# AILab-CVC/SEED-X

Measured on AMD Instinct MI355X. Metric: end-to-end generations/sec (img-in -> txt + 1024px-img-out), higher is better.
Workload: dtype fp16

## Files before the change

include/seedx_hip.h:

```cpp
#ifndef SEEDX_HIP_H
#define SEEDX_HIP_H
#include <stdint.h>
#ifdef __cplusplus
extern "C" {
#endif

#define SX_OK 0
#define SX_ERR_INVALID 1
#define SX_ERR_HIP 2

#define SX_F16 0
#define SX_BF16 1
#define SX_F32 2
#define SX_BF16X3 3
#define SX_F16X2 4
#define SX_FP8_E4M3 5
#define SX_TILED16 0x100

#define SX_ACT_NONE 0
#define SX_ACT_GELU 1
#define SX_ACT_SILU 2

#define SX_A_LINEAR 0
#define SX_A_CONV3X3 1

const char* sx_last_error(void);
int sx_version(void);

typedef struct sx_gemm_args {
  const void* A;
  const void* W;
  void* C;
  const float* bias;
  const float* bias2d;
  const float* residual;
  int32_t M, N, K;
  int32_t ldc, ldr;
  int32_t n_valid;
  int32_t res_mod;
  int32_t bias2d_rows;
  int32_t dtype;
  int32_t out_dtype;
  int32_t act;
  int32_t glu;
  int32_t a_mode;
  int32_t B, Hin, Win, Cin, Hout, Wout;
  int32_t stride;
  int32_t upsample;
  int32_t ld_bias2d;
  int32_t pad_mode;
  int32_t a_planes;
} sx_gemm_args;
int sx_gemm(const sx_gemm_args* args, void* stream);
int sx_gemm_gn(const sx_gemm_args* args, double* stats, int groups, int rows_per_sample, int* fused_host, void* stream);
typedef struct sx_gemm_ln_args {
  void* x16_out;
  double* row_stats_out;
  const double* row_stats_in;
  const float* colsum;
  int32_t ld_x16;
  int32_t dim;
  float eps;
  int32_t reserved;
} sx_gemm_ln_args;
int sx_gemm_ln(const sx_gemm_args* args, const sx_gemm_ln_args* ln, void* stream);
int sx_gemm_force_tile(int cfg);
int sx_gemm_debug_stamps(void* buf);
int sx_gemm_pick_tile(int M, int N, int K, int glu, int conv);

typedef struct sx_gemv_args {
  const void* x;
  const void* W;
  void* y;
  const float* residual;
  int32_t M, N, K;
  int32_t dtype, out_dtype, act, glu;
  int32_t w_layout;
  int32_t x_layout;
  void* workspace;
  uint64_t workspace_bytes;
  void* x16_out;
  float* row_ssq_out;
  const float* row_ssq_in;
  int32_t ssq_in_parts, ssq_dim;
  float ssq_eps;
  int32_t x_planes;
  int32_t out_planes;
  const float* x16_gamma;
  int32_t w_dtype;
  const float* w_scale;
} sx_gemv_args;
int sx_gemv_ssq_parts(int N, int glu, int w_layout);
int sx_gemv(const sx_gemv_args* args, void* stream);
int sx_gemv_force_valu(int on);
int sx_gemv_tune(int key, int value);

int sx_layernorm(const void* x, int in_dtype, void* y, int out_dtype, const float* gamma, const float* beta,
                 int rows, int cols, float eps, int rms, void* stream);

int sx_softmax_rows(const float* x, int64_t ldx, void* y, int64_t ldy, int rows, int cols, float scale, int out_dtype,
                    void* stream);

int sx_groupnorm(const float* x, void* y, void* raw16, int out_dtype, const float* gamma, const float* beta,
                 double* stats, int B, int HW, int C, int groups, float eps, int silu, void* stream);
int sx_groupnorm2(const float* x, const float* x2, int C1, void* y, void* raw16, int out_dtype, const float* gamma,
                  const float* beta, double* stats, int B, int HW, int C, int groups, float eps, int silu, void* stream);
int sx_norm_tune(int key, int value);
int sx_groupnorm_sp(const float* x, const float* x2, int C1, void* y, void* raw16, int out_dtype, const float* gamma,
                    const float* beta, double* stats, int B, int HW, int hw_total, int C, int groups, float eps, int silu,
                    int phase, void* stream);

typedef struct sx_attn_args {
  const void* Q;
  const void* K;
  const void* V;
  void* O;
  int32_t B, H, Sq, Skv, D, reserved;
  int64_t q_batch_stride, q_row_stride, q_head_stride;
  int64_t k_batch_stride, k_row_stride, k_head_stride;
  int64_t v_batch_stride, v_row_stride, v_head_stride;
  int64_t o_batch_stride, o_row_stride;
  float scale;
  int32_t causal;
  int32_t dtype;
} sx_attn_args;
int sx_attention(const sx_attn_args* args, void* stream);

typedef struct sx_attn_small_args {
  const void* Q;
  const void* K;
  const void* V;
  void* O;
  int32_t B, H, Sq, Skv, D;
  int64_t q_batch_stride, q_row_stride, q_head_stride;
  int64_t k_batch_stride, k_row_stride, k_head_stride;
  int64_t v_batch_stride, v_row_stride, v_head_stride;
  int64_t o_batch_stride, o_row_stride;
  float scale;
  int32_t dtype;
} sx_attn_small_args;
int sx_attention_small(const sx_attn_small_args* args, void* stream);

int sx_attn_decode(const void* q, const void* kcache, const void* vcache, void* out, float* scratch,
                   const int32_t* ctx_len_dev, int H, int D, int Tmax, int nsplit, float scale, int dtype,
                   void* stream);

int sx_rope_kv_append(void* qkv, void* kcache, void* vcache, const float* cos_tab, const float* sin_tab,
                      const int32_t* pos0_dev, int T, int H, int D, int Tmax, int dtype, void* stream);
int sx_embedding(const int32_t* ids, const void* table, float* out, int T, int dim, int dtype, void* stream);
int sx_scatter_rows(const float* src, const int32_t* rows, float* dst, int n, int dim, void* stream);
int sx_greedy_next(float* logits, int vocab, const int32_t* img_ids_dev, int n_img, const int32_t* prev_id_dev,
                   int32_t* next_id_dev, int32_t* out_ids, const int32_t* step_dev, void* stream);

int sx_rope_kv_append_b(void* qkv, void* kcache, void* vcache, const float* cos_tab, const float* sin_tab,
                        const int32_t* pos0_dev, int G, int T, int H, int D, int Tmax, int64_t cache_seq_stride, int dtype,
                        void* stream);
int sx_attn_decode_b(const void* q, const void* kcache, const void* vcache, void* out, float* scratch,
                     const int32_t* ctx_len_dev, int G, int H, int D, int Tmax, int64_t cache_seq_stride, int nsplit,
                     float scale, int dtype, int64_t q_seq_stride, void* stream);
typedef struct sx_attn_decode_args {
  const void* qkv;
  void* kcache;
  void* vcache;
  void* out;
  float* scratch;
  void* counters;
  const float* cos_tab;
  const float* sin_tab;
  const int32_t* pos_dev;
  int32_t G, H, D, Tmax, nsplit, dtype;
  int64_t cache_seq_stride;
  float scale;
  int32_t reserved;
} sx_attn_decode_args;
int sx_attn_decode_fused(const sx_attn_decode_args* args, void* stream);
int sx_greedy_next_b(float* logits, int ld_logits, int vocab, const int32_t* img_ids_dev, int n_img,
                     const int32_t* prev_id_dev, int32_t* next_id_dev, int32_t* out_ids, int ld_out,
                     const int32_t* step_dev, int G, void* stream);
int sx_scatter_rows_step(const float* src, const int32_t* step_dev, float* dst, int G, int dim, int seq_rows, void* stream);
int sx_add_i32_n(int32_t* p, int delta, int n, void* stream);
typedef struct sx_slot_step_args {
  float* logits;
  const int32_t* img_ids_dev;
  int32_t* cur;
  int32_t* live;
  int32_t* n_new;
  const int32_t* max_new;
  const int32_t* force_at;
  int32_t* pos;
  int32_t* ctx;
  int32_t* step;
  int32_t* out_ids;
  int32_t* status;
  int32_t ld_logits, vocab, n_img, ld_out, force_id, eos_id, G, reserved;
} sx_slot_step_args;
int sx_greedy_next_slots(const sx_slot_step_args* args, void* stream);
typedef struct sx_sample_args {
  const int32_t* do_sample;
  const float* temperature;
  const int32_t* top_k;
  const float* top_p;
  const uint32_t* seed;
  const int32_t* token_index;
  int32_t* n_kept;
  float* p_chosen;
} sx_sample_args;
int sx_sample_next_b(float* logits, int ld_logits, int vocab, const int32_t* img_ids_dev, int n_img,
                     const int32_t* prev_id_dev, int32_t* next_id_dev, int32_t* out_ids, int ld_out,
                     const int32_t* step_dev, int G, const sx_sample_args* sample, void* stream);
int sx_sample_next_slots(const sx_slot_step_args* args, const sx_sample_args* sample, void* stream);

int sx_cast(const void* src, int src_dtype, void* dst, int dst_dtype, int64_t n, void* stream);
int sx_split_bf16(const float* x, void* out, int64_t rows, int cols, int role, void* stream);

int sx_split16(const float* x, int64_t ldx, void* out, int rows, int cols, int dtype, void* stream);
int sx_rmsnorm_planes(const float* x, const float* gamma, float* y32, void* out16, int rows, int cols, float eps, int dtype,
                      void* stream);
int sx_rope_kv_append_f32(float* qkv, float* kcache, float* vcache, const float* cos_tab, const float* sin_tab,
                          const int32_t* pos0_dev, int G, int T, int H, int D, int Tmax, int64_t cache_seq_stride,
                          int table_dtype, void* stream);
int sx_rope_kv_append_f32_v16(float* qkv, float* kcache, void* vcache16, const float* cos_tab, const float* sin_tab,
                              const int32_t* pos0_dev, int G, int T, int H, int D, int Tmax, int64_t cache_seq_stride,
                              int table_dtype, void* stream);
int sx_rope_kv_append_f32_q8(float* qkv, void* kcodes, void* vcodes, float* kscale, float* vscale, const float* cos_tab,
                             const float* sin_tab, const int32_t* pos0_dev, int G, int T, int H, int D, int Tmax,
                             int64_t cache_seq_stride, int64_t scale_seq_stride, int table_dtype, int emulate, void* stream);
typedef struct sx_attn_f32_args {
  const float* q;
  const float* kcache;
  const void* vcache;
  void* out;
  const int32_t* pos0_dev;
  int64_t q_row_stride, cache_seq_stride;
  int64_t kv_row_stride;
  int64_t kv_head_stride;
  int32_t G, T, H, D, Tmax, dtype;
  float scale;
  int32_t causal;
  int32_t v16;
  int32_t nsplit;
  float* scratch;
  const float* rope_cos;
  const float* rope_sin;
  const float* k_new;
  const float* v_new;
  int32_t kv_fp8;
  const float* k_scale;
  const float* v_scale;
  int64_t scale_seq_stride;
} sx_attn_f32_args;
int sx_attention_f32(const sx_attn_f32_args* args, void* stream);
int sx_attention_f32_variant(int v);
int sx_copy2d_f32(const float* src, int64_t src_ld, float* dst, int64_t dst_ld, int64_t rows, int cols,
                  void* stream);
int sx_add_f32(const float* a, const float* b, float* y, int64_t n, void* stream);
int sx_patchify(const float* img, void* patches, int B, int S, int P, int Kpad, int dtype, void* stream);
int sx_im2col3x3_small(const float* x, void* out, int B, int H, int W, int Cin, int Kpad, int dtype,
                       void* stream);
int sx_avgpool_tokens(const float* x, float* y, int B, int L, int D, int k, void* stream);
int sx_timestep_embedding(const float* t, const int32_t* idx_dev, void* out, int n, int dim, int dtype, void* stream);
int sx_nchw_to_nhwc(const float* src, float* dst, int ld, int B, int C, int HW, void* stream);
int sx_nhwc_to_nchw(const float* src, int ld, float* dst, int B, int C, int HW, void* stream);
int sx_add_i32(int32_t* p, int delta, void* stream);
int sx_profile_marker(int tag, void* stream);
int sx_silu_cast(const float* x, void* y, int dtype, int64_t n, void* stream);

int sx_cfg_euler_step(const float* eps, float* latents, float* scaled_next, const float* sigmas_dev,
                      const int32_t* step_dev, int nb, int64_t n, int C, int ld_scaled, float gs, float igs, int mode,
                      void* stream);

int sx_resample_u8(const void* src, int Hin, int Win, int C, int64_t src_stride, void* dst, int Hout, int Wout,
                   const int32_t* kk_h, const int32_t* bounds_h, int ksize_h, const int32_t* kk_v,
                   const int32_t* bounds_v, int ksize_v, int y_first, int y_rows, void* tmp, void* stream);
int sx_u8_to_chw_lut(const void* src, int H, int W, int64_t src_stride, int x0, int y0, int Hc, int Wc,
                     const float* lut3x256, float* dst, void* stream);
int sx_chw_to_u8_image(const float* src, int H, int W, void* dst, void* stream);
int sx_marker_mask(const int64_t* ids, int T, int64_t boi, int64_t bop, int64_t eoi, int64_t eop, void* mask,
                   void* stream);
int sx_l2norm_dim1(const float* x, float* y, int B, int T, int D, float eps, void* stream);

int sx_comm_alloc(void** ptr, uint64_t bytes);
int sx_comm_free(void* ptr);
int sx_ipc_export(void* ptr, unsigned char* handle64);
int sx_ipc_open(const unsigned char* handle64, void** ptr);
int sx_ipc_close(void* ptr);
#define SX_ONESHOT_CHUNK 4096
typedef struct sx_oneshot_args {
  void* data;
  void* gather_out;
  const void* stage;
  const void* flags;
  void* epoch;
  void* status;
  int32_t n, cap, rank, world;
  uint32_t max_spin;
  int32_t chunk;
  int32_t mode;
  int32_t reserved;
} sx_oneshot_args;
int sx_allreduce_oneshot(const sx_oneshot_args* args, void* stream);

int sx_halo_pack(const void* x, const void* prev_row, const void* next_row, void* out, int B, int Hl, int W, int C, int left_col,
                 int bottom, void* stream);

#ifdef __cplusplus
}
#endif
#endif
```

seed-x_amd/_lib.py:

```python
import ctypes as C
import os

_HERE = os.path.dirname(os.path.abspath(__file__))
LIB_PATH = os.path.join(_HERE, "lib", "libseedx_hip.so")

SX_F16, SX_BF16, SX_F32 = 0, 1, 2
SX_BF16X3 = 3
SX_F16X2 = 4
SX_FP8_E4M3 = 5
SX_TILED16 = 0x100
SX_ACT_NONE, SX_ACT_GELU, SX_ACT_SILU = 0, 1, 2
SX_A_LINEAR, SX_A_CONV3X3 = 0, 1

c_i32, c_i64, c_f32, c_vp = C.c_int32, C.c_int64, C.c_float, C.c_void_p


class GemmArgs(C.Structure):
    _fields_ = [("A", c_vp), ("W", c_vp), ("C", c_vp), ("bias", c_vp), ("bias2d", c_vp), ("residual", c_vp),
                ("M", c_i32), ("N", c_i32), ("K", c_i32), ("ldc", c_i32), ("ldr", c_i32), ("n_valid", c_i32),
                ("res_mod", c_i32), ("bias2d_rows", c_i32), ("dtype", c_i32), ("out_dtype", c_i32),
                ("act", c_i32), ("glu", c_i32), ("a_mode", c_i32),
                ("B", c_i32), ("Hin", c_i32), ("Win", c_i32), ("Cin", c_i32), ("Hout", c_i32), ("Wout", c_i32),
                ("stride", c_i32), ("upsample", c_i32), ("ld_bias2d", c_i32), ("pad_mode", c_i32), ("a_planes", c_i32)]


class GemmLnArgs(C.Structure):
    _fields_ = [("x16_out", c_vp), ("row_stats_out", c_vp), ("row_stats_in", c_vp), ("colsum", c_vp),
                ("ld_x16", c_i32), ("dim", c_i32), ("eps", c_f32), ("reserved", c_i32)]


class GemvArgs(C.Structure):
    _fields_ = [("x", c_vp), ("W", c_vp), ("y", c_vp), ("residual", c_vp),
                ("M", c_i32), ("N", c_i32), ("K", c_i32),
                ("dtype", c_i32), ("out_dtype", c_i32), ("act", c_i32), ("glu", c_i32),
                ("w_layout", c_i32), ("x_layout", c_i32), ("workspace", c_vp), ("workspace_bytes", C.c_uint64),
                ("x16_out", c_vp), ("row_ssq_out", c_vp), ("row_ssq_in", c_vp), ("ssq_in_parts", c_i32), ("ssq_dim", c_i32),
                ("ssq_eps", c_f32), ("x_planes", c_i32), ("out_planes", c_i32), ("x16_gamma", c_vp),
                ("w_dtype", c_i32), ("w_scale", c_vp)]


class AttnF32Args(C.Structure):
    _fields_ = [("q", c_vp), ("kcache", c_vp), ("vcache", c_vp), ("out", c_vp), ("pos0_dev", c_vp),
                ("q_row_stride", c_i64), ("cache_seq_stride", c_i64), ("kv_row_stride", c_i64), ("kv_head_stride", c_i64),
                ("G", c_i32), ("T", c_i32), ("H", c_i32), ("D", c_i32), ("Tmax", c_i32), ("dtype", c_i32),
                ("scale", c_f32), ("causal", c_i32), ("v16", c_i32), ("nsplit", c_i32), ("scratch", c_vp),
                ("rope_cos", c_vp), ("rope_sin", c_vp), ("k_new", c_vp), ("v_new", c_vp),
                ("kv_fp8", c_i32), ("k_scale", c_vp), ("v_scale", c_vp), ("scale_seq_stride", c_i64)]


class OneshotArgs(C.Structure):
    _fields_ = [("data", c_vp), ("gather_out", c_vp), ("stage", c_vp), ("flags", c_vp), ("epoch", c_vp), ("status", c_vp),
                ("n", c_i32), ("cap", c_i32), ("rank", c_i32), ("world", c_i32), ("max_spin", C.c_uint32), ("chunk", c_i32),
                ("mode", c_i32), ("reserved", c_i32)]


class AttnDecodeArgs(C.Structure):
    _fields_ = [("qkv", c_vp), ("kcache", c_vp), ("vcache", c_vp), ("out", c_vp), ("scratch", c_vp), ("counters", c_vp),
                ("cos_tab", c_vp), ("sin_tab", c_vp), ("pos_dev", c_vp),
                ("G", c_i32), ("H", c_i32), ("D", c_i32), ("Tmax", c_i32), ("nsplit", c_i32), ("dtype", c_i32),
                ("cache_seq_stride", c_i64), ("scale", c_f32), ("reserved", c_i32)]


class SlotStepArgs(C.Structure):
    _fields_ = [("logits", c_vp), ("img_ids_dev", c_vp), ("cur", c_vp), ("live", c_vp), ("n_new", c_vp), ("max_new", c_vp),
                ("force_at", c_vp), ("pos", c_vp), ("ctx", c_vp), ("step", c_vp), ("out_ids", c_vp), ("status", c_vp),
                ("ld_logits", c_i32), ("vocab", c_i32), ("n_img", c_i32), ("ld_out", c_i32), ("force_id", c_i32),
                ("eos_id", c_i32), ("G", c_i32), ("reserved", c_i32)]


class SampleArgs(C.Structure):
    _fields_ = [("do_sample", c_vp), ("temperature", c_vp), ("top_k", c_vp), ("top_p", c_vp), ("seed", c_vp),
                ("token_index", c_vp), ("n_kept", c_vp), ("p_chosen", c_vp)]


class AttnArgs(C.Structure):
    _fields_ = [("Q", c_vp), ("K", c_vp), ("V", c_vp), ("O", c_vp),
                ("B", c_i32), ("H", c_i32), ("Sq", c_i32), ("Skv", c_i32), ("D", c_i32), ("reserved", c_i32),
                ("q_batch_stride", c_i64), ("q_row_stride", c_i64), ("q_head_stride", c_i64),
                ("k_batch_stride", c_i64), ("k_row_stride", c_i64), ("k_head_stride", c_i64),
                ("v_batch_stride", c_i64), ("v_row_stride", c_i64), ("v_head_stride", c_i64),
                ("o_batch_stride", c_i64), ("o_row_stride", c_i64),
                ("scale", c_f32), ("causal", c_i32), ("dtype", c_i32)]


class AttnSmallArgs(C.Structure):
    _fields_ = [("Q", c_vp), ("K", c_vp), ("V", c_vp), ("O", c_vp),
                ("B", c_i32), ("H", c_i32), ("Sq", c_i32), ("Skv", c_i32), ("D", c_i32),
                ("q_batch_stride", c_i64), ("q_row_stride", c_i64), ("q_head_stride", c_i64),
                ("k_batch_stride", c_i64), ("k_row_stride", c_i64), ("k_head_stride", c_i64),
                ("v_batch_stride", c_i64), ("v_row_stride", c_i64), ("v_head_stride", c_i64),
                ("o_batch_stride", c_i64), ("o_row_stride", c_i64),
                ("scale", c_f32), ("dtype", c_i32)]


SIGNATURES = {
    "sx_version": [],
    "sx_gemm": [C.POINTER(GemmArgs), c_vp],
    "sx_gemm_gn": [C.POINTER(GemmArgs), c_vp, c_i32, c_i32, C.POINTER(c_i32), c_vp],
    "sx_gemm_ln": [C.POINTER(GemmArgs), C.POINTER(GemmLnArgs), c_vp],
    "sx_gemm_force_tile": [c_i32],
    "sx_gemm_debug_stamps": [c_vp],
    "sx_gemm_pick_tile": [c_i32, c_i32, c_i32, c_i32, c_i32],
    "sx_gemv": [C.POINTER(GemvArgs), c_vp],
    "sx_gemv_ssq_parts": [c_i32, c_i32, c_i32],
    "sx_gemv_force_valu": [c_i32],
    "sx_layernorm": [c_vp, c_i32, c_vp, c_i32, c_vp, c_vp, c_i32, c_i32, c_f32, c_i32, c_vp],
    "sx_softmax_rows": [c_vp, c_i64, c_vp, c_i64, c_i32, c_i32, c_f32, c_i32, c_vp],
    "sx_groupnorm": [c_vp, c_vp, c_vp, c_i32, c_vp, c_vp, c_vp, c_i32, c_i32, c_i32, c_i32, c_f32, c_i32, c_vp],
    "sx_groupnorm2": [c_vp, c_vp, c_i32, c_vp, c_vp, c_i32, c_vp, c_vp, c_vp, c_i32, c_i32, c_i32, c_i32, c_f32, c_i32, c_vp],
    "sx_groupnorm_sp": [c_vp, c_vp, c_i32, c_vp, c_vp, c_i32, c_vp, c_vp, c_vp, c_i32, c_i32, c_i32, c_i32, c_i32, c_f32, c_i32,
                        c_i32, c_vp],
    "sx_attention": [C.POINTER(AttnArgs), c_vp],
    "sx_norm_tune": [c_i32, c_i32],
    "sx_gemv_tune": [c_i32, c_i32],
    "sx_comm_alloc": [C.POINTER(c_vp), C.c_uint64],
    "sx_comm_free": [c_vp],
    "sx_ipc_export": [c_vp, C.c_char_p],
    "sx_ipc_open": [C.c_char_p, C.POINTER(c_vp)],
    "sx_ipc_close": [c_vp],
    "sx_allreduce_oneshot": [C.POINTER(OneshotArgs), c_vp],
    "sx_halo_pack": [c_vp, c_vp, c_vp, c_vp, c_i32, c_i32, c_i32, c_i32, c_i32, c_i32, c_vp],
    "sx_attention_small": [C.POINTER(AttnSmallArgs), c_vp],
    "sx_attn_decode": [c_vp, c_vp, c_vp, c_vp, c_vp, c_vp, c_i32, c_i32, c_i32, c_i32, c_f32, c_i32, c_vp],
    "sx_rope_kv_append": [c_vp, c_vp, c_vp, c_vp, c_vp, c_vp, c_i32, c_i32, c_i32, c_i32, c_i32, c_vp],
    "sx_rope_kv_append_b": [c_vp, c_vp, c_vp, c_vp, c_vp, c_vp, c_i32, c_i32, c_i32, c_i32, c_i32, c_i64, c_i32, c_vp],
    "sx_attn_decode_fused": [C.POINTER(AttnDecodeArgs), c_vp],
    "sx_attn_decode_b": [c_vp, c_vp, c_vp, c_vp, c_vp, c_vp, c_i32, c_i32, c_i32, c_i32, c_i64, c_i32, c_f32, c_i32, c_i64, c_vp],
    "sx_greedy_next_b": [c_vp, c_i32, c_i32, c_vp, c_i32, c_vp, c_vp, c_vp, c_i32, c_vp, c_i32, c_vp],
    "sx_greedy_next_slots": [C.POINTER(SlotStepArgs), c_vp],
    "sx_sample_next_b": [c_vp, c_i32, c_i32, c_vp, c_i32, c_vp, c_vp, c_vp, c_i32, c_vp, c_i32, C.POINTER(SampleArgs), c_vp],
    "sx_sample_next_slots": [C.POINTER(SlotStepArgs), C.POINTER(SampleArgs), c_vp],
    "sx_scatter_rows_step": [c_vp, c_vp, c_vp, c_i32, c_i32, c_i32, c_vp],
    "sx_add_i32_n": [c_vp, c_i32, c_i32, c_vp],
    "sx_embedding": [c_vp, c_vp, c_vp, c_i32, c_i32, c_i32, c_vp],
    "sx_scatter_rows": [c_vp, c_vp, c_vp, c_i32, c_i32, c_vp],
    "sx_greedy_next": [c_vp, c_i32, c_vp, c_i32, c_vp, c_vp, c_vp, c_vp, c_vp],
    "sx_cast": [c_vp, c_i32, c_vp, c_i32, c_i64, c_vp],
    "sx_split_bf16": [c_vp, c_vp, c_i64, c_i32, c_i32, c_vp],
    "sx_split16": [c_vp, c_i64, c_vp, c_i32, c_i32, c_i32, c_vp],
    "sx_rmsnorm_planes": [c_vp, c_vp, c_vp, c_vp, c_i32, c_i32, c_f32, c_i32, c_vp],
    "sx_rope_kv_append_f32": [c_vp, c_vp, c_vp, c_vp, c_vp, c_vp, c_i32, c_i32, c_i32, c_i32, c_i32, c_i64, c_i32, c_vp],
    "sx_rope_kv_append_f32_v16": [c_vp, c_vp, c_vp, c_vp, c_vp, c_vp, c_i32, c_i32, c_i32, c_i32, c_i32, c_i64, c_i32, c_vp],
    "sx_rope_kv_append_f32_q8": [c_vp, c_vp, c_vp, c_vp, c_vp, c_vp, c_vp, c_vp, c_i32, c_i32, c_i32, c_i32, c_i32, c_i64, c_i64, c_i32,
                                 c_i32, c_vp],
    "sx_attention_f32": [C.POINTER(AttnF32Args), c_vp],
    "sx_attention_f32_variant": [c_i32],
    "sx_copy2d_f32": [c_vp, c_i64, c_vp, c_i64, c_i64, c_i32, c_vp],
    "sx_add_f32": [c_vp, c_vp, c_vp, c_i64, c_vp],
    "sx_patchify": [c_vp, c_vp, c_i32, c_i32, c_i32, c_i32, c_i32, c_vp],
    "sx_im2col3x3_small": [c_vp, c_vp, c_i32, c_i32, c_i32, c_i32, c_i32, c_i32, c_vp],
    "sx_avgpool_tokens": [c_vp, c_vp, c_i32, c_i32, c_i32, c_i32, c_vp],
    "sx_timestep_embedding": [c_vp, c_vp, c_vp, c_i32, c_i32, c_i32, c_vp],
    "sx_nchw_to_nhwc": [c_vp, c_vp, c_i32, c_i32, c_i32, c_i32, c_vp],
    "sx_nhwc_to_nchw": [c_vp, c_i32, c_vp, c_i32, c_i32, c_i32, c_vp],
    "sx_add_i32": [c_vp, c_i32, c_vp],
    "sx_profile_marker": [c_i32, c_vp],
    "sx_silu_cast": [c_vp, c_vp, c_i32, c_i64, c_vp],
    "sx_resample_u8": [c_vp, c_i32, c_i32, c_i32, c_i64, c_vp, c_i32, c_i32, c_vp, c_vp, c_i32, c_vp, c_vp, c_i32, c_i32, c_i32,
                       c_vp, c_vp],
    "sx_u8_to_chw_lut": [c_vp, c_i32, c_i32, c_i64, c_i32, c_i32, c_i32, c_i32, c_vp, c_vp, c_vp],
    "sx_chw_to_u8_image": [c_vp, c_i32, c_i32, c_vp, c_vp],
    "sx_marker_mask": [c_vp, c_i32, c_i64, c_i64, c_i64, c_i64, c_vp, c_vp],
    "sx_l2norm_dim1": [c_vp, c_vp, c_i32, c_i32, c_i32, c_f32, c_vp],
    "sx_cfg_euler_step": [c_vp, c_vp, c_vp, c_vp, c_vp, c_i32, c_i64, c_i32, c_i32, c_f32, c_f32, c_i32, c_vp],
}

_lib = None


def load():
    global _lib
    if _lib is not None:
        return _lib
    if not os.path.exists(LIB_PATH):
        raise RuntimeError(
            f"seedx_amd: {LIB_PATH} not found — build it with `python -c 'import __graft_entry__ as g; g.build()'` "
            "(hipcc --offload-arch=gfx950). There is no CPU fallback for the product path.")
    lib = C.CDLL(LIB_PATH)
    for name, argtypes in SIGNATURES.items():
        fn = getattr(lib, name)
        fn.argtypes = argtypes
        fn.restype = C.c_int
    lib.sx_last_error.argtypes = []
    lib.sx_last_error.restype = C.c_char_p
    _lib = lib
    return lib


def check(status, what):
    if status != 0:
        msg = load().sx_last_error().decode("utf-8", "replace")
        raise RuntimeError(f"{what} failed (status {status}): {msg}")
```

seed-x_amd/csrc/gemm.hip:

```cpp
#include "gemm_common.h"

namespace sxk_gemm {

template <typename TT, int BM, int BN, int WM, int WN, int NSTAGE, int AMODE>
__global__ __launch_bounds__(WM * WN * 64) void gemm_kernel(const GemmP p) {
#if defined(__HIP_DEVICE_COMPILE__)
  typedef typename TT::vec8 vec8;
  constexpr int NW = WM * WN;
  static_assert(NW == 4 || NW == 8, "4 or 8 waves per block");
  constexpr int TM = BM / WM, TN = BN / WN;
  constexpr int FM = TM / 16, FN = TN / 16;
  constexpr bool kGlu = (FN % 2 == 0);
  constexpr int BNP = (BN + 8 * NW - 1) / (8 * NW) * (8 * NW);
  constexpr int A_PER_WAVE = BM / (8 * NW);
  constexpr int B_PER_WAVE = BNP / (8 * NW);
  constexpr int LOADS = A_PER_WAVE + B_PER_WAVE;
  constexpr int A_BYTES = BM * 128, B_BYTES = BNP * 128, STAGE = A_BYTES + B_BYTES;
  static_assert(LOADS * (NSTAGE - 1) <= 63, "vmcnt range");
  extern __shared__ __attribute__((aligned(16))) unsigned char smem[];

  const int tid = threadIdx.x, lane = tid & 63;
  const int wave = __builtin_amdgcn_readfirstlane(tid >> 6);
  const int wm = wave / WN, wn = wave % WN;
  unsigned long long t_start = 0, t_first = 0, t_main = 0;
// ... 43 lines not shown
    int dy = 0, dx = 0, cc = 0;
    if (AMODE == SX_A_CONV3X3) {
      const int tap = kt / cpt;
      cc = kt - tap * cpt;
      dy = tap / 3;
      dx = tap - dy * 3;
    }
#pragma unroll
    for (int i = 0; i < A_PER_WAVE; ++i) {
      unsigned voff;
      if (AMODE == SX_A_LINEAR) {
        voff = a_off[i] + (unsigned)kt * 128u;
      } else {
        int iy = a_y[i] + dy, ix = a_x[i] + dx;
        const bool ok = (a_b[i] >= 0) && iy >= 0 && iy < Hv && ix >= 0 && ix < Wv;
        if (p.upsample) { iy >>= 1; ix >>= 1; }
        voff = ok ? (unsigned)(((a_b[i] + iy) * p.Win + ix) * p.Cin) * 2u + (unsigned)cc * 128u + gchunk
                  : 0x80000000u;
      }
      __builtin_amdgcn_raw_ptr_buffer_load_lds(rA, SX_LDS_PTR(sA + (wave * A_PER_WAVE + i) * 1024), 16, voff, 0, 0,
                                               0);
    }
#pragma unroll
    for (int i = 0; i < B_PER_WAVE; ++i) {
      __builtin_amdgcn_raw_ptr_buffer_load_lds(rW, SX_LDS_PTR(sB + (wave * B_PER_WAVE + i) * 1024), 16,
                                               w_off[i] + (unsigned)(kt >= nkw ? kt - nkw : kt) * 128u, 0, 0, 0);
    }
  };

  f32x4_t acc[FN][FM];
  if (p.res_init) {
#pragma unroll
    for (int j = 0; j < FM; ++j) {
      const int m = m0 + wm * TM + j * 16 + (lane & 15);
      const int mc = m < p.M ? m : p.M - 1;
      const float* rr = p.residual + (size_t)(p.res_mod ? (mc % p.res_mod) : mc) * p.ldr;
#pragma unroll
      for (int i = 0; i < FN; ++i) {
        int c = n0 + wn * TN + i * 16 + (lane >> 4) * 4;
        if (c + 4 > p.ldr) c = 0;
        acc[i][j] = *(const f32x4_t*)(rr + c);
      }
    }
  } else {
#pragma unroll
    for (int i = 0; i < FN; ++i)
#pragma unroll
      for (int j = 0; j < FM; ++j) acc[i][j] = (f32x4_t){0.f, 0.f, 0.f, 0.f};
  }

  const unsigned frag_row = (unsigned)(lane & 15) * 128u;
  unsigned frag_sw[2];
  frag_sw[0] = (unsigned)(((lane >> 4)) ^ (lane & 7)) << 4;
  frag_sw[1] = (unsigned)((4 + (lane >> 4)) ^ (lane & 7)) << 4;

  const int nkt = p.K / 64;
  constexpr int D = NSTAGE - 1;
#pragma unroll
  for (int s = 0; s < D; ++s)
    if (s < nkt) stage(s, s);
  int cur = 0, nxt = D % NSTAGE;
  for (int kt = 0; kt < nkt; ++kt) {
    if (D >= 2 && kt + 1 < nkt) wait_vmcnt<LOADS*(D - 1)>();
    else wait_vmcnt<0>();
    __builtin_amdgcn_s_barrier();
    if (p.dbg && kt == 0) t_first = __builtin_amdgcn_s_memtime();
    if (kt + D < nkt) stage(nxt, kt + D);
    const unsigned char* sA = smem + cur * STAGE + (wm * TM) * 128;
    const unsigned char* sB = smem + cur * STAGE + A_BYTES + (wn * TN) * 128;
#pragma unroll
    for (int ks = 0; ks < 2; ++ks) {
      vec8 af[FM], wf[FN];
#pragma unroll
      for (int j = 0; j < FM; ++j) af[j] = *(const vec8*)(sA + j * 2048 + frag_row + frag_sw[ks]);
#pragma unroll
      for (int i = 0; i < FN; ++i) wf[i] = *(const vec8*)(sB + i * 2048 + frag_row + frag_sw[ks]);
#pragma unroll
      for (int i = 0; i < FN; ++i)
#pragma unroll
        for (int j = 0; j < FM; ++j) acc[i][j] = TT::mfma16(wf[i], af[j], acc[i][j]);
    }
    cur = (cur + 1 == NSTAGE) ? 0 : cur + 1;
    nxt = (nxt + 1 == NSTAGE) ? 0 : nxt + 1;
  }

  if (p.dbg) t_main = __builtin_amdgcn_s_memtime();
  const int lq = (lane >> 4) * 4;
  int ncol[FN], nout[FN];
  bool nok[FN];
  f32x4_t bv[FN];
#pragma unroll
  for (int i = 0; i < FN; ++i) {
    const int nb = n0 + wn * TN + i * 16;
    ncol[i] = nb + lq;
    nout[i] = (kGlu && p.glu) ? (nb >> 1) + lq : ncol[i];
    nok[i] = ncol[i] < p.N && nout[i] < p.n_valid && !((kGlu && p.glu) && (i & 1));
    if (ncol[i] >= p.N) ncol[i] = p.N - 4;
    if (nout[i] + 4 > p.ldc) nout[i] = 0;
    bv[i] = (f32x4_t){0.f, 0.f, 0.f, 0.f};
  }
  if (p.bias) {
#pragma unroll
    for (int i = 0; i < FN; ++i) bv[i] = *(const f32x4_t*)(p.bias + ncol[i]);
  }
  const bool wide = p.out_dtype != SX_F32 && !(kGlu && p.glu) && (p.ldc & 7) == 0 && (((size_t)p.C) & 15) == 0;
  bool pair_ok[(FN + 1) / 2];
#pragma unroll
  for (int i = 0; i < (FN + 1) / 2; ++i) {
    const int lim = p.n_valid < p.N ? p.n_valid : p.N;
    pair_ok[i] = (2 * i + 1 < FN) && (n0 + wn * TN + i * 32 + 32 <= lim);
  }
#pragma unroll
  for (int j = 0; j < FM; ++j) {
    const int m = m0 + wm * TM + j * 16 + (lane & 15);
    const bool mok = m < p.M;
    const int mc = mok ? m : p.M - 1;
    f32x4_t v[FN], rv[FN];
#pragma unroll
    for (int i = 0; i < FN; ++i) {
      v[i] = acc[i][j] + bv[i];
      rv[i] = (f32x4_t){0.f, 0.f, 0.f, 0.f};
    }
    if (p.bias2d) {
      const float* b2 = p.bias2d + (size_t)(mc / p.bias2d_rows) * p.ldb2;
#pragma unroll
      for (int i = 0; i < FN; ++i) v[i] += *(const f32x4_t*)(b2 + ncol[i]);
    }
    if (p.residual && !p.res_init) {
      const float* rr = p.residual + (size_t)(p.res_mod ? (mc % p.res_mod) : mc) * p.ldr;
#pragma unroll
      for (int i = 0; i < FN; ++i) {
        const int c = (nout[i] + 4 <= p.ldr) ? nout[i] : 0;
        rv[i] = *(const f32x4_t*)(rr + c);
      }
    }
    if (wide) {
#pragma unroll
      for (int i = 0; i + 1 < FN; i += 2) {
        if (!pair_ok[i >> 1]) continue;
        u32x2_t o[2];
#pragma unroll
        for (int h = 0; h < 2; ++h) {
          f32x4_t x = v[i + h];
          if (p.act == SX_ACT_GELU) {
            const f32x2_t g0 = gelu_erf2((f32x2_t){x[0], x[1]}), g1 = gelu_erf2((f32x2_t){x[2], x[3]});
            x = (f32x4_t){g0[0], g0[1], g1[0], g1[1]};
          } else if (p.act != SX_ACT_NONE) {
#pragma unroll
            for (int r = 0; r < 4; ++r) x[r] = apply_act(x[r], p.act);
          }
          x += rv[i + h];
          if (p.out_dtype == SX_BF16) {
            o[h][0] = pack2<BF16>(x[0], x[1]);
            o[h][1] = pack2<BF16>(x[2], x[3]);
          } else {
            o[h][0] = pack2<F16>(x[0], x[1]);
            o[h][1] = pack2<F16>(x[2], x[3]);
          }
        }
        const auto s0 = __builtin_amdgcn_permlane16_swap(o[0][0], o[1][0], false, false);
        const auto s1 = __builtin_amdgcn_permlane16_swap(o[0][1], o[1][1], false, false);
        if (!mok) continue;
        const u32x4_t w4 = {s0[0], s1[0], s0[1], s1[1]};
        const int q = lane >> 4;
        const int col = n0 + wn * TN + i * 16 + (q & 1) * 16 + (q >> 1) * 8;
        *(u32x4_t*)((unsigned short*)p.C + (size_t)m * p.ldc + col) = w4;
      }
    }
#pragma unroll
    for (int i = 0; i < FN; ++i) {
      if (wide && pair_ok[i >> 1]) continue;
      if ((kGlu && p.glu)) {
        if (i & 1) continue;
        const f32x4_t g = v[(i + 1) < FN ? (i + 1) : i];
        if (p.act == SX_ACT_GELU) {
          const f32x2_t g0 = gelu_erf2((f32x2_t){g[0], g[1]}), g1 = gelu_erf2((f32x2_t){g[2], g[3]});
          v[i][0] *= g0[0]; v[i][1] *= g0[1]; v[i][2] *= g1[0]; v[i][3] *= g1[1];
        } else {
#pragma unroll
          for (int r = 0; r < 4; ++r) v[i][r] = v[i][r] * apply_act(g[r], p.act);
        }
      } else if (p.act == SX_ACT_GELU) {
        const f32x2_t g0 = gelu_erf2((f32x2_t){v[i][0], v[i][1]}), g1 = gelu_erf2((f32x2_t){v[i][2], v[i][3]});
        v[i] = (f32x4_t){g0[0], g0[1], g1[0], g1[1]};
      } else if (p.act != SX_ACT_NONE) {
#pragma unroll
        for (int r = 0; r < 4; ++r) v[i][r] = apply_act(v[i][r], p.act);
      }
      const f32x4_t o4 = v[i] + rv[i];
      if (!(mok && nok[i])) continue;
      if (p.out_dtype == SX_F32) {
        *(f32x4_t*)((float*)p.C + (size_t)m * p.ldc + nout[i]) = o4;
      } else {
        u32x2_t o;
        if (p.out_dtype == SX_BF16) {
          o[0] = pack2<BF16>(o4[0], o4[1]);
          o[1] = pack2<BF16>(o4[2], o4[3]);
        } else {
          o[0] = pack2<F16>(o4[0], o4[1]);
          o[1] = pack2<F16>(o4[2], o4[3]);
        }
        *(u32x2_t*)((unsigned short*)p.C + (size_t)m * p.ldc + nout[i]) = o;
      }
    }
  }
  if (p.dbg) {
    asm volatile("s_waitcnt vmcnt(0)" ::: "memory");
    const unsigned long long t_end = __builtin_amdgcn_s_memtime();
    if (tid == 0) {
      unsigned long long* d = p.dbg + (size_t)blockIdx.x * 4;
      d[0] = t_start; d[1] = t_first; d[2] = t_main; d[3] = t_end;
    }
  }
#endif
}

unsigned long long* g_dbg = nullptr;
int g_gm = 0;
int g_xcd_2d = 1;

template <typename TT, int BM, int BN, int WM, int WN, int NSTAGE>
int launch_cfg(const GemmP& p0, int a_mode, hipStream_t st) {
  GemmP p = p0;
  p.dbg = g_dbg;
  const int grid = plan_grid(p, BM, BN, g_xcd_2d, g_gm);
  constexpr int NW = WM * WN;
  const size_t lds = (size_t)NSTAGE * (BM + (BN + 8 * NW - 1) / (8 * NW) * (8 * NW)) * 128;
  auto reserve = [&](const void* k, hipError_t* attr, bool* done) -> hipError_t {
    int dev = 0;
    (void)hipGetDevice(&dev);
    dev &= 15;
    if (!done[dev]) {
      attr[dev] = lds > 65536 ? hipFuncSetAttribute(k, hipFuncAttributeMaxDynamicSharedMemorySize, (int)lds) : hipSuccess;
      done[dev] = true;
    }
    return attr[dev];
  };
  if (a_mode == SX_A_LINEAR) {
    auto k = gemm_kernel<TT, BM, BN, WM, WN, NSTAGE, SX_A_LINEAR>;
    static hipError_t attr[16];
    static bool done[16];
    const hipError_t e = reserve((const void*)k, attr, done);
    SX_CHECK(e == hipSuccess, "sx_gemm: cannot reserve %zu B of LDS for the %dx%d tile: %s", lds, BM, BN, hipGetErrorString(e));
    hipLaunchKernelGGL(k, dim3(grid), dim3(NW * 64), lds, st, p);
  } else {
    auto k = gemm_kernel<TT, BM, BN, WM, WN, NSTAGE, SX_A_CONV3X3>;
    static hipError_t attr[16];
    static bool done[16];
    const hipError_t e = reserve((const void*)k, attr, done);
    SX_CHECK(e == hipSuccess, "sx_gemm: cannot reserve %zu B of LDS for the %dx%d tile: %s", lds, BM, BN, hipGetErrorString(e));
    hipLaunchKernelGGL(k, dim3(grid), dim3(NW * 64), lds, st, p);
  }
  SX_HIP_LAUNCH_CHECK();
  return SX_OK;
}

struct TileCfg { int bm, bn; bool glu_ok; int slots; float a_lin, b_lin, a_conv, b_conv; };
static const int kNumTiles = 9;
static const TileCfg kTiles[kNumTiles] = {
    {128, 128, true, 512, 7.85f, 0.01202f, 15.26f, 0.01513f},  {128, 80, false, 256, 3.45f, 0.00766f, 3.59f, 0.01135f},
    {64, 128, true, 256, 1.37f, 0.00479f, 1.63f, 0.00546f},    {64, 64, true, 256, 0.33f, 0.00301f, 0.82f, 0.00313f},
    {256, 256, true, 256, 11.34f, 0.02161f, 13.19f, 0.02365f}, {256, 320, false, 256, 17.95f, 0.02566f, 18.01f, 0.02985f},
    {256, 160, false, 256, 8.13f, 0.01579f, 9.06f, 0.01897f},  {256, 256, true, 256, 10.56f, 0.01592f, 12.81f, 0.01840f},
    {256, 320, false, 256, 13.32f, 0.01928f, 15.12f, 0.02173f}};

inline int pick_tile(int M, int N, int K, bool glu, bool conv, int force, unsigned allow = 0x7f) {
  if (force >= 0 && force < kNumTiles && (!glu || kTiles[force].glu_ok)) return force;
  int best = 2;
  float best_t = 1e30f;
  for (int c = 0; c < kNumTiles; ++c) {
    const TileCfg& t = kTiles[c];
    if (!((allow >> c) & 1u)) continue;
    if (glu && !t.glu_ok) continue;
    const long tiles = (long)((M + t.bm - 1) / t.bm) * ((N + t.bn - 1) / t.bn);
    const long rounds = (tiles + t.slots - 1) / t.slots;
    const float us = (float)rounds * (conv ? t.a_conv + t.b_conv * (float)K : t.a_lin + t.b_lin * (float)K);
    if (us < best_t) { best_t = us; best = c; }
  }
  return best;
}

}
using namespace sxk_gemm;

static int g_force_tile = -1;
extern "C" int sx_gemm_pick_tile(int M, int N, int K, int glu, int conv) {
  return sxk_gemm::pick_tile(M, N, K, glu != 0, conv != 0, -1, 0x1ff);
}

extern "C" int sx_gemm_debug_stamps(void* buf) {
  sxk_gemm::g_dbg = (unsigned long long*)buf;
  return SX_OK;
}

extern "C" int sx_gemm_force_tile(int cfg) {
  if (cfg == 100 || cfg == 101) { sxk_gemm::g_xcd_2d = cfg - 100; return SX_OK; }
  if (cfg >= 300 && cfg <= 364) { sxk_gemm::g_gm = cfg - 300; return SX_OK; }
  SX_CHECK(cfg >= -1 && cfg < kNumTiles, "sx_gemm_force_tile: %d is not -1, a tile config 0..%d, 100/101 or 300..364", cfg,
           kNumTiles - 1);
  g_force_tile = cfg;
  return SX_OK;
}

static int gemm_impl(const sx_gemm_args* a, double* gn_stats, int gn_groups, int gn_rows, int* gn_fused, const sx_gemm_ln_args* ln,
                     void* stream);

extern "C" int sx_gemm(const sx_gemm_args* a, void* stream) { return gemm_impl(a, nullptr, 0, 0, nullptr, nullptr, stream); }

extern "C" int sx_gemm_ln(const sx_gemm_args* a, const sx_gemm_ln_args* ln, void* stream) {
  SX_CHECK(ln && (ln->row_stats_in || ln->row_stats_out), "sx_gemm_ln: neither a producer nor a consumer role");
  return gemm_impl(a, nullptr, 0, 0, nullptr, ln, stream);
}

extern "C" int sx_gemm_gn(const sx_gemm_args* a, double* stats, int groups, int rows_per_sample, int* fused, void* stream) {
  SX_CHECK(stats && fused && groups > 0 && rows_per_sample > 0, "sx_gemm_gn: bad statistics arguments");
  return gemm_impl(a, stats, groups, rows_per_sample, fused, nullptr, stream);
}

static int gemm_impl(const sx_gemm_args* a, double* gn_stats, int gn_groups, int gn_rows, int* gn_fused, const sx_gemm_ln_args* ln,
                     void* stream) {
  SX_CHECK(a && a->A && a->W && a->C, "sx_gemm: null pointer");
  if (gn_fused) *gn_fused = 0;
  SX_CHECK(a->dtype == SX_F16 || a->dtype == SX_BF16, "sx_gemm: dtype must be f16/bf16");
  SX_CHECK(a->out_dtype >= SX_F16 && a->out_dtype <= SX_F32, "sx_gemm: bad out_dtype");
  SX_CHECK(a->M > 0 && a->N > 0 && a->K > 0, "sx_gemm: empty problem M=%d N=%d K=%d", a->M, a->N, a->K);
  SX_CHECK(a->K % 64 == 0, "sx_gemm: K=%d must be a multiple of 64 (pad the operand)", a->K);
  SX_CHECK(a->N % 16 == 0, "sx_gemm: N=%d must be a multiple of 16 (pad the weight)", a->N);
  SX_CHECK(!a->glu || a->N % 32 == 0, "sx_gemm: glu needs N %% 32 == 0");
  const int n_out = a->glu ? a->N / 2 : a->N;
  SX_CHECK(a->n_valid >= 0 && a->n_valid % 4 == 0 && a->n_valid <= n_out, "sx_gemm: n_valid=%d", a->n_valid);
  SX_CHECK(a->ldc >= (a->n_valid > 0 ? a->n_valid : n_out) && a->ldc % 4 == 0, "sx_gemm: ldc=%d invalid for n_out=%d",
           a->ldc, n_out);
  SX_CHECK(!a->residual || (a->ldr >= (a->n_valid > 0 ? a->n_valid : n_out) && a->ldr % 4 == 0), "sx_gemm: ldr=%d invalid", a->ldr);
  SX_CHECK(!a->bias2d || a->bias2d_rows > 0, "sx_gemm: bias2d_rows must be > 0");
  GemmP p;
  memset(&p, 0, sizeof(p));
  p.A = a->A; p.W = a->W; p.C = a->C; p.bias = a->bias; p.bias2d = a->bias2d; p.residual = a->residual;
  SX_CHECK(a->a_planes >= 0 && a->a_planes <= 2, "sx_gemm: a_planes=%d", a->a_planes);
  const int planes = a->a_planes == 2 ? 2 : 1;
  SX_CHECK(planes == 1 || (a->a_mode == SX_A_LINEAR && !ln), "sx_gemm: a_planes = 2 is for plain linear GEMMs");
  const int Kk = a->K * planes;
  p.M = a->M; p.N = a->N; p.K = Kk; p.Kw = a->K; p.ldc = a->ldc; p.ldr = a->ldr; p.res_mod = a->res_mod;
  p.n_valid = a->n_valid > 0 ? a->n_valid : n_out;
  p.bias2d_rows = a->bias2d_rows; p.out_dtype = a->out_dtype; p.act = a->act; p.glu = a->glu;
  p.ldb2 = a->ld_bias2d > 0 ? a->ld_bias2d : a->N;
  p.pad = 1;
  uint64_t a_bytes;
  if (a->a_mode == SX_A_CONV3X3) {
    SX_CHECK(a->Cin % 64 == 0 && a->K == 9 * a->Cin, "sx_gemm conv: Cin=%d K=%d", a->Cin, a->K);
    SX_CHECK(a->stride == 1 || a->stride == 2, "sx_gemm conv: stride");
    SX_CHECK(a->M == a->B * a->Hout * a->Wout, "sx_gemm conv: M != B*Hout*Wout");
    const int hv = a->upsample ? 2 * a->Hin : a->Hin, wv = a->upsample ? 2 * a->Win : a->Win;
    SX_CHECK(a->pad_mode == 0 || a->pad_mode == 1, "sx_gemm conv: pad_mode");
    const int padsum = a->pad_mode ? 1 : 2;
    SX_CHECK(a->Hout == (hv + padsum - 3) / a->stride + 1 && a->Wout == (wv + padsum - 3) / a->stride + 1,
             "sx_gemm conv: output geometry mismatch");
    p.pad = a->pad_mode ? 0 : 1;
    p.Hin = a->Hin; p.Win = a->Win; p.Cin = a->Cin; p.Hout = a->Hout; p.Wout = a->Wout;
    p.stride = a->stride; p.upsample = a->upsample;
    a_bytes = (uint64_t)a->B * a->Hin * a->Win * a->Cin * 2;
  } else {
    SX_CHECK(a->a_mode == SX_A_LINEAR, "sx_gemm: bad a_mode");
    a_bytes = (uint64_t)a->M * Kk * 2;
  }
  const uint64_t w_bytes = (uint64_t)a->N * a->K * 2;
  SX_CHECK(a_bytes < 0x7fffffffull && w_bytes < 0x7fffffffull, "sx_gemm: operand exceeds 2 GiB descriptor range");
  p.a_bytes = (unsigned)a_bytes;
  p.w_bytes = (unsigned)w_bytes;
  hipStream_t st = (hipStream_t)stream;
  p.res_init = (p.residual && p.act == SX_ACT_NONE && !p.glu) ? 1 : 0;
  if (ln) {
    SX_CHECK(a->a_mode == SX_A_LINEAR && !gn_stats, "sx_gemm_ln: linear GEMMs only");
    SX_CHECK(!(ln->row_stats_in && ln->row_stats_out), "sx_gemm_ln: a launch is a producer or a consumer, not both");
    if (ln->row_stats_out) {
      SX_CHECK(ln->x16_out && a->out_dtype == SX_F32 && !a->glu && a->act == SX_ACT_NONE && p.n_valid == a->N,
               "sx_gemm_ln producer: needs x16_out and a plain fp32 output of all N columns");
      SX_CHECK(ln->ld_x16 >= a->N && ln->ld_x16 % 4 == 0 && (((size_t)ln->x16_out) & 7) == 0, "sx_gemm_ln producer: ld_x16=%d", ln->ld_x16);
      p.ln_x16 = ln->x16_out; p.ln_ldx = ln->ld_x16; p.ln_out = ln->row_stats_out;
    } else {
      SX_CHECK(ln->colsum && ln->dim == a->K && ln->eps > 0.f, "sx_gemm_ln consumer: colsum / dim (= K) / eps");
      SX_CHECK(a->out_dtype == a->dtype && !a->residual && !a->bias2d, "sx_gemm_ln consumer: 16-bit output, no residual / bias2d");
      p.ln_in = ln->row_stats_in; p.ln_cs = ln->colsum; p.ln_eps = ln->eps; p.ln_inv_dim = 1.0f / (float)ln->dim;
    }
  }
  unsigned allow = 0x7f;
  if (ln) allow = 0;
  allow |= pp_supported(p, a->dtype, 256, a->a_mode) ? 0x80u : 0u;
  allow |= pp_supported(p, a->dtype, 320, a->a_mode) ? 0x100u : 0u;
  SX_CHECK(!(g_force_tile == 7 || g_force_tile == 8) || ((allow >> g_force_tile) & 1u),
           "sx_gemm: forced ping-pong tile has no kernel for this epilogue");
  if (ln) {
    const int plain = pick_tile(a->M, a->N, Kk, a->glu != 0, false, g_force_tile, 0x1ff);
    SX_CHECK((plain == 7 || plain == 8) && ((allow >> plain) & 1u),
             "sx_gemm_ln: M=%d N=%d K=%d does not run on a ping-pong tile with this epilogue (tile %d): keep sx_layernorm for it", a->M,
             a->N, a->K, plain);
    allow = 1u << plain;
  }
  const int cfg = pick_tile(a->M, a->N, Kk, a->glu != 0, a->a_mode == SX_A_CONV3X3, g_force_tile, allow);
  if (cfg == 7 || cfg == 8) {
    if (gn_stats && a->out_dtype == SX_F32 && !a->glu && a->act == SX_ACT_NONE && p.n_valid == a->N && a->N % gn_groups == 0 &&
        (a->N / gn_groups) % 2 == 0 && gn_rows % 256 == 0 && a->M % gn_rows == 0) {
      p.gn_stats = gn_stats; p.gn_groups = gn_groups; p.gn_cpg = a->N / gn_groups; p.gn_rows = gn_rows;
      *gn_fused = 1;
    }
    return launch_pp(p, a->dtype, cfg == 7 ? 256 : 320, a->a_mode, st);
  }
#define SX_GEMM_DISPATCH(TT)                                                  \
  switch (cfg) {                                                              \
    case 0: return launch_cfg<TT, 128, 128, 2, 2, 2>(p, a->a_mode, st);       \
    case 1: return launch_cfg<TT, 128, 80, 4, 1, 3>(p, a->a_mode, st);        \
    case 2: return launch_cfg<TT, 64, 128, 2, 2, 3>(p, a->a_mode, st);        \
    case 3: return launch_cfg<TT, 64, 64, 2, 2, 3>(p, a->a_mode, st);         \
    case 4: return launch_cfg<TT, 256, 256, 2, 4, 2>(p, a->a_mode, st);       \
    case 5: return launch_cfg<TT, 256, 320, 2, 4, 2>(p, a->a_mode, st);       \
    default: return launch_cfg<TT, 256, 160, 4, 2, 2>(p, a->a_mode, st);      \
  }
  if (a->dtype == SX_BF16) { SX_GEMM_DISPATCH(BF16) } else { SX_GEMM_DISPATCH(F16) }
#undef SX_GEMM_DISPATCH
}
```

seed-x_amd/csrc/gemm_common.h:

```cpp
#pragma once
#include "sx_common.h"

namespace sxk_gemm {

struct GemmP {
  const void* A;
  const void* W;
  void* C;
  const float* bias;
  const float* bias2d;
  const float* residual;
  int M, N, K, ldc, ldr, n_valid, res_mod, bias2d_rows, out_dtype, act, glu;
  int Kw;
  int Hin, Win, Cin, Hout, Wout, stride, upsample, ldb2, pad;
  int tiles_m, tiles_n, xm, xn;
  int gm;
  int res_init;
  unsigned a_bytes, w_bytes;
  unsigned long long* dbg;
  double* gn_stats;
  int gn_cpg, gn_groups, gn_rows;
  void* ln_x16;
  double* ln_out;
  const double* ln_in;
  const float* ln_cs;
  int ln_ldx;
  float ln_eps, ln_inv_dim;
};

template <int N>
__device__ __forceinline__ void wait_vmcnt() {
  asm volatile("s_waitcnt vmcnt(%0)" ::"n"(N) : "memory");
}

__device__ __forceinline__ bool tile_coords(const GemmP& p, int bid, int nblk, int& tile_m, int& tile_n) {
  if (p.xm == 0) {
    const int t = xcd_remap(bid, nblk);
    tile_m = t % p.tiles_m;
    tile_n = t / p.tiles_m;
    return true;
  }
  const int xcd = bid & 7, idx = bid >> 3;
  const int xr = xcd / p.xn, xc = xcd - xr * p.xn;
  const int ms = xr * p.tiles_m / p.xm, me = (xr + 1) * p.tiles_m / p.xm;
  const int ns = xc * p.tiles_n / p.xn, ne = (xc + 1) * p.tiles_n / p.xn;
  const int rm = me - ms, rn = ne - ns;
  if (idx >= rm * rn) return false;
  const int per_group = p.gm * rn;
  const int g = idx / per_group, first = g * p.gm;
  const int gsz = (rm - first) < p.gm ? (rm - first) : p.gm;
  const int r = idx - g * per_group;
  tile_m = ms + first + r % gsz;
  tile_n = ns + r / gsz;
  return true;
}

inline int plan_grid(GemmP& p, int BM, int BN, int xcd_2d, int gm_force) {
  p.tiles_m = (p.M + BM - 1) / BM;
  p.tiles_n = (p.N + BN - 1) / BN;
  int grid = p.tiles_m * p.tiles_n;
  p.xm = p.xn = 0;
  p.gm = 1;
  if (grid >= 16 && xcd_2d) {
    const double ab = (double)p.M * p.K, wb = (double)p.N * p.K;
    double best = 1e300;
    for (int xm = 1; xm <= 8; xm *= 2) {
      const int xn = 8 / xm;
      if (xm > p.tiles_m || xn > p.tiles_n) continue;
      const long padded = 8L * ((p.tiles_m + xm - 1) / xm) * ((p.tiles_n + xn - 1) / xn);
      const double cost = (ab * xn + wb * xm) * (1.0 + 4.0 * (double)(padded - grid) / grid);
      if (cost < best) { best = cost; p.xm = xm; p.xn = xn; }
    }
    if (p.xm) grid = 8 * ((p.tiles_m + p.xm - 1) / p.xm) * ((p.tiles_n + p.xn - 1) / p.xn);
    p.gm = gm_force > 0 ? gm_force : 8;
  }
  return grid;
}

int launch_pp(const GemmP& p, int dtype, int bn, int a_mode, hipStream_t st);
bool pp_supported(const GemmP& p, int dtype, int bn, int a_mode);

extern unsigned long long* g_dbg;
extern int g_gm;
extern int g_xcd_2d;

}
```

seed-x_amd/csrc/gemm_pp.hip:

```cpp
#include "gemm_common.h"
#include <type_traits>

namespace sxk_gemm {

#define SX_A_CONV3X3_UP 2

#define PP_SYNC()                            \
  do {                                       \
    __builtin_amdgcn_sched_barrier(0);       \
    __builtin_amdgcn_s_barrier();            \
    __builtin_amdgcn_sched_barrier(0);       \
  } while (0)

template <typename TT, int BN, int AMODE, bool OUT32, int ACT, bool GLU, int LN = 0>
__global__ __launch_bounds__(512) void gemm_pp_kernel(const GemmP p) {
#if defined(__HIP_DEVICE_COMPILE__)
  typedef typename TT::vec8 vec8;
  static_assert(LN != 2 || (OUT32 && !GLU && ACT == SX_ACT_NONE), "the LayerNorm producer is the plain fp32-output epilogue");
  constexpr int BM = 256, TN = BN / 4, FN = TN / 16, FM = 8, FH = 4;
  constexpr int NB = BN / 64;
  constexpr int C1 = NB - 3, C2 = 3;
  constexpr int WAITN = 4 + NB;
  constexpr int A_BYTES = BM * 128, STAGE = A_BYTES + BN * 128;
  static_assert(!GLU || FN % 2 == 0, "GLU pairs n-fragments");
  static_assert(BN == 256 || BN == 320, "ping-pong tiles are 256x256 and 256x320");
  extern __shared__ __attribute__((aligned(16))) unsigned char smem[];

  const int tid = threadIdx.x, lane = tid & 63;
  const int wave = __builtin_amdgcn_readfirstlane(tid >> 6);
  const int g = wave >> 2, wc = wave & 3;
  unsigned long long t_start = 0, t_first = 0, t_main = 0;
  if (p.dbg) t_start = __builtin_amdgcn_s_memtime();

  int tile_m, tile_n;
  if (!tile_coords(p, blockIdx.x, gridDim.x, tile_m, tile_n)) return;
  const int m0 = tile_m * BM, n0 = tile_n * BN;

  double ln_s1 = 0.0, ln_s2 = 0.0;
  if constexpr (LN == 1) {
    if (tid < BM) {
      const int m = m0 + tid < p.M ? m0 + tid : p.M - 1;
      ln_s1 = p.ln_in[2 * (size_t)m];
      ln_s2 = p.ln_in[2 * (size_t)m + 1];
    }
  }
  __amdgpu_buffer_rsrc_t rA = __builtin_amdgcn_make_buffer_rsrc((void*)p.A, 0, (int)p.a_bytes, 0x00020000);
  __amdgpu_buffer_rsrc_t rW = __builtin_amdgcn_make_buffer_rsrc((void*)p.W, 0, (int)p.w_bytes, 0x00020000);

  const int rl = lane >> 3;
  const unsigned gchunk = ((lane & 7) ^ rl) << 4;
  unsigned a_off[4], a_msk[4];
  int a_lrow[4];
#pragma unroll
  for (int s = 0; s < 4; ++s) {
    a_lrow[s] = g * 128 + (s >> 1) * 64 + ((2 * wave + (s & 1)) & 7) * 8;
    const int row = m0 + a_lrow[s] + rl;
    if (AMODE == SX_A_LINEAR) {
      a_off[s] = (row < p.M) ? (unsigned)row * (unsigned)p.K * 2u + gchunk : 0xC0000000u;
      a_msk[s] = 0;
    } else {
      const int hw = p.Hout * p.Wout;
      const int b = row / hw, rem = row - b * hw;
      const int oy = rem / p.Wout, ox = rem - oy * p.Wout;
      const int Hv = p.upsample ? 2 * p.Hin : p.Hin, Wv = p.upsample ? 2 * p.Win : p.Win;
      const int vy = oy * p.stride - p.pad, vx = ox * p.stride - p.pad;
      unsigned msk = 0;
#pragma unroll
      for (int t = 0; t < 9; ++t) {
        const int iy = vy + t / 3, ix = vx + t % 3;
        if (row < p.M && iy >= 0 && iy < Hv && ix >= 0 && ix < Wv) msk |= 1u << t;
      }
      int sy = vy, sx = vx;
      if (AMODE == SX_A_CONV3X3_UP) {
        sy = oy >> 1; sx = ox >> 1;
        msk |= (unsigned)(oy & 1) << 9 | (unsigned)(ox & 1) << 10;
      }
      a_off[s] = (unsigned)(((b * p.Hin + sy) * p.Win + sx) * p.Cin) * 2u + gchunk;
      a_msk[s] = msk;
    }
  }
  unsigned w_off[NB];
#pragma unroll
  for (int i = 0; i < NB; ++i) {
    const int row = n0 + (wave * NB + i) * 8 + rl;
    w_off[i] = (row < p.N) ? (unsigned)row * (unsigned)p.Kw * 2u + gchunk : 0xC0000000u;
  }
  const int cpt = (AMODE != SX_A_LINEAR) ? p.Cin / 64 : 1;
  const int nkt = p.K / 64;
  const int nkw = p.Kw / 64;

  struct Tap { int cc, dy, dx; };
  auto tap_next = [&](Tap& t) {
    if (++t.cc == cpt) { t.cc = 0; if (++t.dx == 3) { t.dx = 0; ++t.dy; } }
  };

  auto koff_of = [&](int kt) -> unsigned { return (kt < nkt) ? (unsigned)kt * 128u : 0x80000000u; };
  auto koff_w = [&](int kt) -> unsigned { return (kt < nkt) ? (unsigned)(kt >= nkw ? kt - nkw : kt) * 128u : 0x80000000u; };
  auto dma_a = [&](int s, int buf, int kt, const Tap& t) {
    unsigned voff;
    if (AMODE == SX_A_LINEAR) {
      voff = a_off[s] + koff_of(kt);
    } else {
      const int tap = t.dy * 3 + t.dx;
      const bool ok = ((a_msk[s] >> tap) & 1u) != 0 && kt < nkt;
      unsigned o;
      if (AMODE == SX_A_CONV3X3_UP) {
        const int ry = ((int)((a_msk[s] >> 9) & 1u) + t.dy - 1) >> 1, rx = ((int)((a_msk[s] >> 10) & 1u) + t.dx - 1) >> 1;
        o = a_off[s] + (unsigned)((ry * p.Win + rx) * p.Cin) * 2u + (unsigned)t.cc * 128u;
      } else {
        o = a_off[s] + (unsigned)(((t.dy * p.Win + t.dx) * p.Cin + t.cc * 64) * 2);
      }
      voff = ok ? o : 0x80000000u;
    }
    __builtin_amdgcn_raw_ptr_buffer_load_lds(rA, SX_LDS_PTR(smem + buf * STAGE + a_lrow[s] * 128), 16, voff, 0, 0, 0);
  };
  auto dma_w = [&](int i, int buf, int kt) {
    __builtin_amdgcn_raw_ptr_buffer_load_lds(rW, SX_LDS_PTR(smem + buf * STAGE + A_BYTES + (wave * NB + i) * 1024), 16,
                                             w_off[i] + koff_w(kt), 0, 0, 0);
  };
  auto issue_x = [&](int buf, int kt, const Tap& t) {
    dma_a(0, buf, kt, t);
    dma_a(1, buf, kt, t);
#pragma unroll
    for (int i = 0; i < C1; ++i) dma_w(i, buf, kt);
  };
  auto issue_y = [&](int buf, int kt) {
#pragma unroll
    for (int i = C1; i < NB; ++i) dma_w(i, buf, kt);
  };

  f32x4_t acc[FN][FM];
  const int lq = (lane >> 4) * 4;
  if (p.res_init) {
#pragma unroll
    for (int j = 0; j < FM; ++j) {
      const int m = m0 + g * 128 + j * 16 + (lane & 15);
      const int mc = m < p.M ? m : p.M - 1;
      const float* rr = p.residual + (size_t)(p.res_mod ? (mc % p.res_mod) : mc) * p.ldr;
#pragma unroll
      for (int i = 0; i < FN; ++i) {
        int c = n0 + wc * TN + i * 16 + lq;
        if (c + 4 > p.ldr) c = 0;
        acc[i][j] = *(const f32x4_t*)(rr + c);
      }
    }
  } else {
#pragma unroll
    for (int i = 0; i < FN; ++i)
#pragma unroll
      for (int j = 0; j < FM; ++j) acc[i][j] = (f32x4_t){0.f, 0.f, 0.f, 0.f};
  }

  const unsigned frag_row = (unsigned)(lane & 15) * 128u;
  unsigned frag_sw[2];
  frag_sw[0] = (unsigned)(((lane >> 4)) ^ (lane & 7)) << 4;
  frag_sw[1] = (unsigned)((4 + (lane >> 4)) ^ (lane & 7)) << 4;
  const unsigned a_frag = (unsigned)(g * 128) * 128u + frag_row;
  const unsigned w_frag = (unsigned)A_BYTES + (unsigned)(wc * TN) * 128u + frag_row;

  Tap kx = {0, 0, 0}, kz = {0, 0, 0};
  issue_x(0, 0, kx);
  issue_y(0, 0);
  dma_a(2, 0, 0, kz);
  dma_a(3, 0, 0, kz);
  tap_next(kz);
  tap_next(kx);
  issue_x(1, 1, kx);
  issue_y(1, 1);
  tap_next(kx);
  float* ln_lds = (float*)(smem + 2 * STAGE);
  if constexpr (LN == 1) {
    if (tid < BM) {
      const double mu = ln_s1 * (double)p.ln_inv_dim;
      const double var = ln_s2 * (double)p.ln_inv_dim - mu * mu;
      const float rstd = __builtin_amdgcn_rsqf((float)(var > 0.0 ? var : 0.0) + p.ln_eps);
      *(f32x2_t*)(ln_lds + 2 * tid) = (f32x2_t){rstd, -rstd * (float)mu};
    }
  }
  wait_vmcnt<WAITN>();
  PP_SYNC();
  if (p.dbg) t_first = __builtin_amdgcn_s_memtime();
  if (g == 1) PP_SYNC();

  vec8 af[FH], wf0[FN], wf1[FN];

  auto mma = [&](const vec8* wf, int h) {
    __builtin_amdgcn_s_setprio(1);
#pragma unroll
    for (int i = 0; i < FN; ++i)
#pragma unroll
      for (int j = 0; j < FH; ++j) acc[i][h * FH + j] = TT::mfma16(wf[i], af[j], acc[i][h * FH + j]);
    __builtin_amdgcn_s_setprio(0);
  };
  auto lgkm0 = [&]() { asm volatile("s_waitcnt lgkmcnt(0)" ::: "memory"); };

  auto ktile = [&](auto BUFC, int u) {
    constexpr int BUF = decltype(BUFC)::value;
    const unsigned char* sbuf = smem + BUF * STAGE;
#pragma unroll
    for (int j = 0; j < FH; ++j) af[j] = *(const vec8*)(sbuf + a_frag + j * 2048 + frag_sw[0]);
#pragma unroll
    for (int i = 0; i < FN; ++i) wf0[i] = *(const vec8*)(sbuf + w_frag + i * 2048 + frag_sw[0]);
    dma_a(2, BUF ^ 1, u + 1, kz);
    lgkm0();
    PP_SYNC();
    mma(wf0, 0);
    PP_SYNC();
#pragma unroll
    for (int j = 0; j < FH; ++j) af[j] = *(const vec8*)(sbuf + a_frag + j * 2048 + frag_sw[1]);
#pragma unroll
    for (int i = 0; i < FN; ++i) wf1[i] = *(const vec8*)(sbuf + w_frag + i * 2048 + frag_sw[1]);
    dma_a(3, BUF ^ 1, u + 1, kz);
    tap_next(kz);
    wait_vmcnt<WAITN>();
    lgkm0();
    PP_SYNC();
    mma(wf1, 0);
    PP_SYNC();
#pragma unroll
    for (int j = 0; j < FH; ++j) af[j] = *(const vec8*)(sbuf + a_frag + 8192 + j * 2048 + frag_sw[0]);
    issue_x(BUF, u + 2, kx);
    lgkm0();
    PP_SYNC();
    mma(wf0, 1);
    PP_SYNC();
#pragma unroll
    for (int j = 0; j < FH; ++j) af[j] = *(const vec8*)(sbuf + a_frag + 8192 + j * 2048 + frag_sw[1]);
    issue_y(BUF, u + 2);
    tap_next(kx);
    wait_vmcnt<WAITN>();
    lgkm0();
    PP_SYNC();
    mma(wf1, 1);
    PP_SYNC();
  };

  for (int kt = 0; kt < nkt; kt += 2) {
    ktile(std::integral_constant<int, 0>{}, kt);
    if (kt + 1 < nkt) ktile(std::integral_constant<int, 1>{}, kt + 1);
  }
  if (g == 0) PP_SYNC();
  wait_vmcnt<0>();

  if (p.dbg) t_main = __builtin_amdgcn_s_memtime();
  int ncol[FN], nout[FN];
  bool nok[FN];
  f32x4_t bv[FN];
#pragma unroll
  for (int i = 0; i < FN; ++i) {
    const int nb = n0 + wc * TN + i * 16;
    ncol[i] = nb + lq;
    nout[i] = GLU ? (nb >> 1) + lq : ncol[i];
    nok[i] = ncol[i] < p.N && nout[i] < p.n_valid && !(GLU && (i & 1));
    if (ncol[i] >= p.N) ncol[i] = p.N - 4;
    if (nout[i] + 4 > p.ldc) nout[i] = 0;
    bv[i] = (f32x4_t){0.f, 0.f, 0.f, 0.f};
  }
  if (p.bias) {
#pragma unroll
    for (int i = 0; i < FN; ++i) bv[i] = *(const f32x4_t*)(p.bias + ncol[i]);
  }
  const bool b2_uniform = p.bias2d && (m0 / p.bias2d_rows) == ((m0 + BM - 1 < p.M ? m0 + BM - 1 : p.M - 1) / p.bias2d_rows);
  if (b2_uniform) {
    const float* b2 = p.bias2d + (size_t)(m0 / p.bias2d_rows) * p.ldb2;
#pragma unroll
    for (int i = 0; i < FN; ++i) bv[i] += *(const f32x4_t*)(b2 + ncol[i]);
  }
  const bool b2_rows = p.bias2d && !b2_uniform;
  const bool res_late = p.residual && !p.res_init;
  const bool wide = !OUT32 && !GLU && (p.ldc & 7) == 0 && (((size_t)p.C) & 15) == 0;
  bool pair_ok[(FN + 1) / 2];
#pragma unroll
  for (int i = 0; i < (FN + 1) / 2; ++i) {
    const int lim = p.n_valid < p.N ? p.n_valid : p.N;
    pair_ok[i] = (2 * i + 1 < FN) && (n0 + wc * TN + i * 32 + 32 <= lim);
  }
  const bool glu_wide = GLU && !OUT32 && (p.ldc & 7) == 0 && (((size_t)p.C) & 15) == 0 &&
                        ((n0 + wc * TN) >> 1) + 32 <= (p.n_valid < (p.N >> 1) ? p.n_valid : (p.N >> 1));
  auto act1 = [&](f32x4_t x) -> f32x4_t {
    if (ACT == SX_ACT_GELU) {
      const f32x2_t g0 = gelu_erf2((f32x2_t){x[0], x[1]}), g1 = gelu_erf2((f32x2_t){x[2], x[3]});
      return (f32x4_t){g0[0], g0[1], g1[0], g1[1]};
    } else if (ACT == SX_ACT_SILU) {
      return (f32x4_t){silu_f(x[0]), silu_f(x[1]), silu_f(x[2]), silu_f(x[3])};
    }
    return x;
  };
  auto pack4 = [&](f32x4_t x) -> u32x2_t {
    u32x2_t o;
    o[0] = pack2<TT>(x[0], x[1]);
    o[1] = pack2<TT>(x[2], x[3]);
    return o;
  };
  f32x4_t lcs[LN == 1 ? FN : 1];
  if constexpr (LN == 1) {
#pragma unroll
    for (int i = 0; i < FN; ++i) lcs[i] = *(const f32x4_t*)(p.ln_cs + ncol[i]);
  }
  float lsum[LN == 2 ? FM : 1], lsq[LN == 2 ? FM : 1];
  const bool gn = OUT32 && p.gn_stats != nullptr;
  float gsl[FN], gql[FN], gsh[FN], gqh[FN];
#pragma unroll
  for (int i = 0; i < FN; ++i) gsl[i] = gql[i] = gsh[i] = gqh[i] = 0.f;
#pragma unroll
  for (int j = 0; j < FM; ++j) {
    const int m = m0 + g * 128 + j * 16 + (lane & 15);
    const bool mok = m < p.M;
    const int mc = mok ? m : p.M - 1;
    f32x4_t v[FN];
    if constexpr (LN == 1) {
      const f32x2_t ab = *(const f32x2_t*)(ln_lds + 2 * (g * 128 + j * 16 + (lane & 15)));
#pragma unroll
      for (int i = 0; i < FN; ++i) v[i] = acc[i][j] * ab[0] + (lcs[i] * ab[1] + bv[i]);
    } else {
#pragma unroll
      for (int i = 0; i < FN; ++i) v[i] = acc[i][j] + bv[i];
    }
    if (b2_rows) {
      const float* b2 = p.bias2d + (size_t)(mc / p.bias2d_rows) * p.ldb2;
#pragma unroll
      for (int i = 0; i < FN; ++i) v[i] += *(const f32x4_t*)(b2 + ncol[i]);
    }
    if (GLU) {
#pragma unroll
      for (int i = 0; i + 1 < FN; i += 2) {
        const f32x4_t gt = act1(v[i + 1]);
        v[i] = v[i] * gt;
      }
    } else if (ACT != SX_ACT_NONE) {
#pragma unroll
      for (int i = 0; i < FN; ++i) v[i] = act1(v[i]);
    }
    if (res_late) {
      const float* rr = p.residual + (size_t)(p.res_mod ? (mc % p.res_mod) : mc) * p.ldr;
#pragma unroll
      for (int i = 0; i < FN; ++i) {
        if (GLU && (i & 1)) continue;
        const int c = (nout[i] + 4 <= p.ldr) ? nout[i] : 0;
        v[i] += *(const f32x4_t*)(rr + c);
      }
    }
    if (OUT32) {
#pragma unroll
      for (int i = 0; i < FN; ++i)
        if (mok && nok[i]) *(f32x4_t*)((float*)p.C + (size_t)m * p.ldc + nout[i]) = v[i];
      if constexpr (LN == 2) {
        float s1 = 0.f, s2 = 0.f;
#pragma unroll
        for (int i = 0; i < FN; ++i) {
          if (mok && nok[i]) {
            s1 += (v[i][0] + v[i][1]) + (v[i][2] + v[i][3]);
            s2 += (v[i][0] * v[i][0] + v[i][1] * v[i][1]) + (v[i][2] * v[i][2] + v[i][3] * v[i][3]);
          }
        }
        lsum[j] = s1;
        lsq[j] = s2;
        const bool xwide = (p.ln_ldx & 7) == 0 && (((size_t)p.ln_x16) & 15) == 0;
#pragma unroll
        for (int i = 0; i < FN; ++i) {
          if ((i & 1) == 0 && i + 1 < FN && xwide && pair_ok[i >> 1]) {
            const u32x2_t o0 = pack4(v[i]), o1 = pack4(v[i + 1]);
            const auto w0 = __builtin_amdgcn_permlane16_swap(o0[0], o1[0], false, false);
            const auto w1 = __builtin_amdgcn_permlane16_swap(o0[1], o1[1], false, false);
            if (mok) {
              const u32x4_t w4 = {w0[0], w1[0], w0[1], w1[1]};
              const int q = lane >> 4;
              const int col = n0 + wc * TN + i * 16 + (q & 1) * 16 + (q >> 1) * 8;
              *(u32x4_t*)((unsigned short*)p.ln_x16 + (size_t)m * p.ln_ldx + col) = w4;
            }
            continue;
          }
          if ((i & 1) && xwide && pair_ok[i >> 1]) continue;
          if (mok && nok[i]) *(u32x2_t*)((unsigned short*)p.ln_x16 + (size_t)m * p.ln_ldx + nout[i]) = pack4(v[i]);
        }
      }
      if (gn && mok) {
#pragma unroll
        for (int i = 0; i < FN; ++i) {
          gsl[i] += v[i][0] + v[i][1];
          gql[i] += v[i][0] * v[i][0] + v[i][1] * v[i][1];
          gsh[i] += v[i][2] + v[i][3];
          gqh[i] += v[i][2] * v[i][2] + v[i][3] * v[i][3];
        }
      }
    } else {
      if constexpr (GLU && FN == 4) {
        if (glu_wide) {
          const u32x2_t o0 = pack4(v[0]), o1 = pack4(v[2]);
          const auto s0 = __builtin_amdgcn_permlane16_swap(o0[0], o1[0], false, false);
          const auto s1 = __builtin_amdgcn_permlane16_swap(o0[1], o1[1], false, false);
          if (mok) {
            const u32x4_t w4 = {s0[0], s1[0], s0[1], s1[1]};
            const int q = lane >> 4;
            const int col = ((n0 + wc * TN) >> 1) + (q & 1) * 16 + (q >> 1) * 8;
            *(u32x4_t*)((unsigned short*)p.C + (size_t)m * p.ldc + col) = w4;
          }
          continue;
        }
      }
#pragma unroll
      for (int i = 0; i < FN; ++i) {
        if (GLU && (i & 1)) continue;
        if (!GLU && wide && (i & 1) == 0 && i + 1 < FN && pair_ok[i >> 1]) {
          const u32x2_t o0 = pack4(v[i]), o1 = pack4(v[i + 1]);
          const auto s0 = __builtin_amdgcn_permlane16_swap(o0[0], o1[0], false, false);
          const auto s1 = __builtin_amdgcn_permlane16_swap(o0[1], o1[1], false, false);
          if (mok) {
            const u32x4_t w4 = {s0[0], s1[0], s0[1], s1[1]};
            const int q = lane >> 4;
            const int col = n0 + wc * TN + i * 16 + (q & 1) * 16 + (q >> 1) * 8;
            *(u32x4_t*)((unsigned short*)p.C + (size_t)m * p.ldc + col) = w4;
          }
          continue;
        }
        if (!GLU && wide && (i & 1) && pair_ok[i >> 1]) continue;
        if (mok && nok[i]) *(u32x2_t*)((unsigned short*)p.C + (size_t)m * p.ldc + nout[i]) = pack4(v[i]);
      }
    }
  }
  if constexpr (LN == 2) {
    float* racc = (float*)smem;
    __syncthreads();
#pragma unroll
    for (int j = 0; j < FM; ++j) {
      float s1 = lsum[j], s2 = lsq[j];
      s1 += __shfl_xor(s1, 16, 64); s2 += __shfl_xor(s2, 16, 64);
      s1 += __shfl_xor(s1, 32, 64); s2 += __shfl_xor(s2, 32, 64);
      if (lane < 16) *(f32x2_t*)(racc + ((size_t)(wc * BM + g * 128 + j * 16 + lane)) * 2) = (f32x2_t){s1, s2};
    }
    __syncthreads();
    if (tid < BM && m0 + tid < p.M) {
      float s1 = 0.f, s2 = 0.f;
#pragma unroll
      for (int w = 0; w < 4; ++w) { s1 += racc[(w * BM + tid) * 2]; s2 += racc[(w * BM + tid) * 2 + 1]; }
      atomicAdd(&p.ln_out[2 * (size_t)(m0 + tid)], (double)s1);
      atomicAdd(&p.ln_out[2 * (size_t)(m0 + tid) + 1], (double)s2);
    }
  }
  if (OUT32 && gn) {
    auto row16_sum = [](float x) -> float {
      x += __builtin_bit_cast(float, __builtin_amdgcn_update_dpp(0, __builtin_bit_cast(int, x), 0xB1, 0xF, 0xF, true));
      x += __builtin_bit_cast(float, __builtin_amdgcn_update_dpp(0, __builtin_bit_cast(int, x), 0x4E, 0xF, 0xF, true));
      x += __builtin_bit_cast(float, __builtin_amdgcn_update_dpp(0, __builtin_bit_cast(int, x), 0x141, 0xF, 0xF, true));
      x += __builtin_bit_cast(float, __builtin_amdgcn_update_dpp(0, __builtin_bit_cast(int, x), 0x140, 0xF, 0xF, true));
      return x;
    };
#pragma unroll
    for (int i = 0; i < FN; ++i) {
      gsl[i] = row16_sum(gsl[i]);
      gql[i] = row16_sum(gql[i]);
      gsh[i] = row16_sum(gsh[i]);
      gqh[i] = row16_sum(gqh[i]);
    }
    float* gslot = (float*)smem;
    const int gbase = n0 / p.gn_cpg;
    const int nlast = (n0 + BN < p.N ? n0 + BN : p.N) - 1;
    const int ngr = nlast / p.gn_cpg - gbase + 1;
    __syncthreads();
    if ((lane & 15) == 0) {
#pragma unroll
      for (int i = 0; i < FN; ++i) {
        const int cp = (wc * TN + i * 16 + lq) >> 1;
        *(f32x4_t*)(gslot + ((size_t)g * (BN / 2) + cp) * 2) = (f32x4_t){gsl[i], gql[i], gsh[i], gqh[i]};
      }
    }
    __syncthreads();
    const int smp = m0 / p.gn_rows;
    for (int t = tid; t < 2 * ngr; t += 512) {
      const int G = gbase + (t >> 1), which = t & 1;
      int c_lo = G * p.gn_cpg - n0, c_hi = (G + 1) * p.gn_cpg - n0;
      c_lo = c_lo < 0 ? 0 : c_lo;
      const int c_end = (p.N - n0 < BN ? p.N - n0 : BN);
      c_hi = c_hi > c_end ? c_end : c_hi;
      float acc = 0.f;
      for (int cp = c_lo >> 1; cp < (c_hi >> 1); ++cp) acc += gslot[(size_t)cp * 2 + which];
      for (int cp = c_lo >> 1; cp < (c_hi >> 1); ++cp) acc += gslot[((size_t)(BN / 2) + cp) * 2 + which];
      atomicAdd(&p.gn_stats[((size_t)smp * p.gn_groups + G) * 2 + which], (double)acc);
    }
  }
  if (p.dbg) {
    asm volatile("s_waitcnt vmcnt(0)" ::: "memory");
    const unsigned long long t_end = __builtin_amdgcn_s_memtime();
    if (tid == 0) {
      unsigned long long* d = p.dbg + (size_t)blockIdx.x * 4;
      d[0] = t_start; d[1] = t_first; d[2] = t_main; d[3] = t_end;
    }
  }
#endif
}

template <typename TT, int BN, int AMODE, bool OUT32, int ACT, bool GLU, int LN = 0>
static int launch_one(const GemmP& p0, hipStream_t st) {
  GemmP p = p0;
  p.dbg = g_dbg;
  const int grid = plan_grid(p, 256, BN, g_xcd_2d, g_gm);
  constexpr size_t lds = 2 * (size_t)(256 + BN) * 128 + (LN == 1 ? 2048 : 0);
  auto k = gemm_pp_kernel<TT, BN, AMODE, OUT32, ACT, GLU, LN>;
  static hipError_t attr[16];
  static bool done[16];
  int dev = 0;
  (void)hipGetDevice(&dev);
  dev &= 15;
  if (!done[dev]) {
    attr[dev] = hipFuncSetAttribute((const void*)k, hipFuncAttributeMaxDynamicSharedMemorySize, (int)lds);
    done[dev] = true;
  }
  SX_CHECK(attr[dev] == hipSuccess, "sx_gemm: cannot reserve %zu B of LDS for the 256x%d ping-pong tile: %s", lds, BN,
           hipGetErrorString(attr[dev]));
  hipLaunchKernelGGL(k, dim3(grid), dim3(512), lds, st, p);
  SX_HIP_LAUNCH_CHECK();
  return SX_OK;
}

static int epi_code(const GemmP& p, int dtype) {
  const bool out32 = p.out_dtype == SX_F32;
  if (!out32 && p.out_dtype != dtype) return -1;
  if (p.glu) {
    if (out32) return -1;
    if (p.act == SX_ACT_GELU) return 2;
    if (p.act == SX_ACT_SILU) return 3;
    return -1;
  }
  if (p.act == SX_ACT_NONE) return out32 ? 4 : 0;
  if (p.act == SX_ACT_GELU && !out32) return 1;
  return -1;
}

bool pp_supported(const GemmP& p, int dtype, int bn, int a_mode) {
  const int e = epi_code(p, dtype);
  if (e < 0) return false;
  if (p.ln_in && !(a_mode == SX_A_LINEAR && (e == 0 || e == 2) && !p.ln_out)) return false;
  if (p.ln_out && !(a_mode == SX_A_LINEAR && e == 4 && !p.gn_stats)) return false;
  if (bn == 320 && (e == 2 || e == 3)) return false;
  if (a_mode == SX_A_CONV3X3 && !(e == 0 || e == 4)) return false;
  if (a_mode == SX_A_CONV3X3 && p.upsample && !(p.stride == 1 && p.pad == 1)) return false;
  return bn == 256 || bn == 320;
}

template <typename TT>
static int launch_t(const GemmP& p, int dtype, int bn, int a_mode, hipStream_t st) {
  const int e = epi_code(p, dtype);
#define PP_CASE(BNV, AM, O32, ACTV, GLUV) return launch_one<TT, BNV, AM, O32, ACTV, GLUV>(p, st)
  if (p.ln_in) {
    if (e == 2) return launch_one<TT, 256, SX_A_LINEAR, false, SX_ACT_GELU, true, 1>(p, st);
    if (bn == 256) return launch_one<TT, 256, SX_A_LINEAR, false, SX_ACT_NONE, false, 1>(p, st);
    return launch_one<TT, 320, SX_A_LINEAR, false, SX_ACT_NONE, false, 1>(p, st);
  }
  if (p.ln_out) {
    if (bn == 256) return launch_one<TT, 256, SX_A_LINEAR, true, SX_ACT_NONE, false, 2>(p, st);
    return launch_one<TT, 320, SX_A_LINEAR, true, SX_ACT_NONE, false, 2>(p, st);
  }
  if (a_mode == SX_A_LINEAR) {
    if (bn == 256) {
      switch (e) {
        case 0: PP_CASE(256, SX_A_LINEAR, false, SX_ACT_NONE, false);
        case 1: PP_CASE(256, SX_A_LINEAR, false, SX_ACT_GELU, false);
        case 2: PP_CASE(256, SX_A_LINEAR, false, SX_ACT_GELU, true);
        case 3: PP_CASE(256, SX_A_LINEAR, false, SX_ACT_SILU, true);
        case 4: PP_CASE(256, SX_A_LINEAR, true, SX_ACT_NONE, false);
      }
    } else {
      switch (e) {
        case 0: PP_CASE(320, SX_A_LINEAR, false, SX_ACT_NONE, false);
        case 1: PP_CASE(320, SX_A_LINEAR, false, SX_ACT_GELU, false);
        case 4: PP_CASE(320, SX_A_LINEAR, true, SX_ACT_NONE, false);
      }
    }
  } else if (!p.upsample) {
    if (bn == 256) {
      switch (e) {
        case 0: PP_CASE(256, SX_A_CONV3X3, false, SX_ACT_NONE, false);
        case 4: PP_CASE(256, SX_A_CONV3X3, true, SX_ACT_NONE, false);
      }
    } else {
      switch (e) {
        case 0: PP_CASE(320, SX_A_CONV3X3, false, SX_ACT_NONE, false);
        case 4: PP_CASE(320, SX_A_CONV3X3, true, SX_ACT_NONE, false);
      }
    }
  } else {
    if (bn == 256) {
      switch (e) {
        case 0: PP_CASE(256, SX_A_CONV3X3_UP, false, SX_ACT_NONE, false);
        case 4: PP_CASE(256, SX_A_CONV3X3_UP, true, SX_ACT_NONE, false);
      }
    } else {
      switch (e) {
        case 0: PP_CASE(320, SX_A_CONV3X3_UP, false, SX_ACT_NONE, false);
        case 4: PP_CASE(320, SX_A_CONV3X3_UP, true, SX_ACT_NONE, false);
      }
    }
  }
#undef PP_CASE
  return -1;
}

int launch_pp(const GemmP& p, int dtype, int bn, int a_mode, hipStream_t st) {
  if (!pp_supported(p, dtype, bn, a_mode)) return -1;
  return dtype == SX_BF16 ? launch_t<BF16>(p, dtype, bn, a_mode, st) : launch_t<F16>(p, dtype, bn, a_mode, st);
}

}
```

seed-x_amd/csrc/norm.hip:

```cpp
#include "sx_common.h"

namespace sxk_norm {

template <int IN_DT>
__device__ __forceinline__ f32x4_t load4(const void* base, size_t idx4) {
  if (IN_DT == SX_F32) {
    return ((const f32x4_t*)base)[idx4];
  } else {
    const u32x2_t u = ((const u32x2_t*)base)[idx4];
    f32x4_t v;
    if (IN_DT == SX_BF16) {
      v[0] = BF16::to_f32(u[0] & 0xffff); v[1] = BF16::to_f32(u[0] >> 16);
      v[2] = BF16::to_f32(u[1] & 0xffff); v[3] = BF16::to_f32(u[1] >> 16);
    } else {
      v[0] = F16::to_f32(u[0] & 0xffff); v[1] = F16::to_f32(u[0] >> 16);
      v[2] = F16::to_f32(u[1] & 0xffff); v[3] = F16::to_f32(u[1] >> 16);
    }
    return v;
  }
}
__device__ __forceinline__ void store4(void* base, int dt, size_t idx4, f32x4_t v) {
  if (dt == SX_F32) {
    ((f32x4_t*)base)[idx4] = v;
  } else {
    u32x2_t o;
    if (dt == SX_BF16) { o[0] = pack2<BF16>(v[0], v[1]); o[1] = pack2<BF16>(v[2], v[3]); }
    else { o[0] = pack2<F16>(v[0], v[1]); o[1] = pack2<F16>(v[2], v[3]); }
    ((u32x2_t*)base)[idx4] = o;
  }
}

template <int IN_DT, int NV>
__global__ __launch_bounds__(256) void layernorm_kernel(const void* x, void* y, int out_dt, const float* gamma,
                                                        const float* beta, int rows, int cols, float eps, int rms) {
  const int lane = threadIdx.x & 63;
  const int row = blockIdx.x * 4 + (threadIdx.x >> 6);
  if (row >= rows) return;
  const int n4 = cols >> 2;
  const size_t base4 = (size_t)row * n4;
  f32x4_t v[NV];
#pragma unroll
  for (int k = 0; k < NV; ++k) {
    const int i = lane + 64 * k;
    v[k] = (i < n4) ? load4<IN_DT>(x, base4 + i) : (f32x4_t){0.f, 0.f, 0.f, 0.f};
  }
  float mean = 0.f;
  if (!rms) {
    float s = 0.f;
#pragma unroll
    for (int k = 0; k < NV; ++k) s += (v[k][0] + v[k][1]) + (v[k][2] + v[k][3]);
    mean = wave_sum(s) / (float)cols;
  }
  float q = 0.f;
#pragma unroll
  for (int k = 0; k < NV; ++k) {
    const int i = lane + 64 * k;
    if (i < n4) {
      const f32x4_t d = v[k] - mean;
      q += (d[0] * d[0] + d[1] * d[1]) + (d[2] * d[2] + d[3] * d[3]);
    }
  }
  const float rstd = rsqrtf(wave_sum(q) / (float)cols + eps);
#pragma unroll
  for (int k = 0; k < NV; ++k) {
    const int i = lane + 64 * k;
    if (i < n4) {
      f32x4_t o = (v[k] - mean) * rstd * ((const f32x4_t*)gamma)[i];
      if (beta) o += ((const f32x4_t*)beta)[i];
      store4(y, out_dt, base4 + i, o);
    }
  }
}

template <int IN_DT>
__global__ __launch_bounds__(256) void layernorm_block_kernel(const void* x, void* y, int out_dt, const float* gamma,
                                                              const float* beta, int rows, int cols, float eps, int rms) {
  __shared__ float red[8];
  const int row = blockIdx.x, tid = threadIdx.x, lane = tid & 63, w = tid >> 6;
  const int n4 = cols >> 2;
  const size_t base4 = (size_t)row * n4;
  constexpr int NV = 6;
  f32x4_t v[NV], g[NV], b[NV];
#pragma unroll
  for (int k = 0; k < NV; ++k) {
    const int i = tid + 256 * k;
    const bool ok = i < n4;
    v[k] = ok ? load4<IN_DT>(x, base4 + i) : (f32x4_t){0.f, 0.f, 0.f, 0.f};
    g[k] = ok ? ((const f32x4_t*)gamma)[i] : (f32x4_t){0.f, 0.f, 0.f, 0.f};
    b[k] = (ok && beta) ? ((const f32x4_t*)beta)[i] : (f32x4_t){0.f, 0.f, 0.f, 0.f};
  }
  float mean = 0.f;
  if (!rms) {
    float s = 0.f;
#pragma unroll
    for (int k = 0; k < NV; ++k) s += (v[k][0] + v[k][1]) + (v[k][2] + v[k][3]);
    s = wave_sum(s);
    if (lane == 0) red[w] = s;
    __syncthreads();
    mean = (red[0] + red[1] + red[2] + red[3]) / (float)cols;
  }
  float q = 0.f;
#pragma unroll
  for (int k = 0; k < NV; ++k) {
    if (tid + 256 * k < n4) {
      const f32x4_t d = v[k] - mean;
      q += (d[0] * d[0] + d[1] * d[1]) + (d[2] * d[2] + d[3] * d[3]);
    }
  }
  q = wave_sum(q);
  if (lane == 0) red[4 + w] = q;
  __syncthreads();
  const float rstd = rsqrtf((red[4] + red[5] + red[6] + red[7]) / (float)cols + eps);
#pragma unroll
  for (int k = 0; k < NV; ++k) {
    const int i = tid + 256 * k;
    if (i < n4) {
      const size_t o4 = (out_dt & SX_TILED16) ? ((size_t)(row >> 4) * (size_t)cols * 16 + (size_t)(i >> 3) * 512 + (size_t)(row & 15) * 32 + (size_t)(i & 7) * 4) >> 2 : base4 + i;
      store4(y, out_dt & 0xff, o4, (v[k] - mean) * rstd * g[k] + b[k]);
    }
  }
}

static int g_gn_stat_blocks = 0;

constexpr int GN_MAX_SLOTS2 = 6;
constexpr int GN_MAX_SLOTS4 = 3;

__global__ void gn_zero_kernel(double* p, int n) {
  const int i = blockIdx.x * blockDim.x + threadIdx.x;
  if (i < n) p[i] = 0.0;
}

template <bool TWO>
__global__ __launch_bounds__(320) void gn_stats_kernel(const float* x, const float* x2, int C1, double* stats, int HW, int C,
                                                       int groups, int rows_per_block) {
  __shared__ __attribute__((aligned(16))) float part[GN_MAX_SLOTS4 * 320 * 4];
  const int T = blockDim.x;
  const int b = blockIdx.y;
  const int r0 = blockIdx.x * rows_per_block;
  const int r1 = min(HW, r0 + rows_per_block);
  const int nq = C >> 2, cpg = C / groups;
  float sl[GN_MAX_SLOTS4], ql[GN_MAX_SLOTS4], sh[GN_MAX_SLOTS4], qh[GN_MAX_SLOTS4];
  const f32x4_t* src[GN_MAX_SLOTS4];
  int ld[GN_MAX_SLOTS4];
  const int nq1 = TWO ? (C1 >> 2) : nq, nq2 = nq - nq1;
  const f32x4_t* xb = (const f32x4_t*)(x + (size_t)b * HW * (TWO ? C1 : C));
  const f32x4_t* xb2 = TWO ? (const f32x4_t*)(x2 + (size_t)b * HW * (C - C1)) : nullptr;
#pragma unroll
  for (int k = 0; k < GN_MAX_SLOTS4; ++k) {
    sl[k] = ql[k] = sh[k] = qh[k] = 0.f;
    const int qd = threadIdx.x + k * T;
    const bool second = TWO && qd >= nq1;
    src[k] = second ? xb2 + (qd - nq1) : xb + qd;
    ld[k] = second ? nq2 : nq1;
  }
  auto add = [&](int k, const f32x4_t v) {
    sl[k] += v[0] + v[1];
    ql[k] += v[0] * v[0] + v[1] * v[1];
    sh[k] += v[2] + v[3];
    qh[k] += v[2] * v[2] + v[3] * v[3];
  };
  int r = r0;
  for (; r + 3 < r1; r += 4) {
#pragma unroll
    for (int k = 0; k < GN_MAX_SLOTS4; ++k) {
      if (threadIdx.x + k * T < nq) {
        const f32x4_t v0 = src[k][(size_t)r * ld[k]], v1 = src[k][(size_t)(r + 1) * ld[k]];
        const f32x4_t v2 = src[k][(size_t)(r + 2) * ld[k]], v3 = src[k][(size_t)(r + 3) * ld[k]];
        add(k, v0); add(k, v1); add(k, v2); add(k, v3);
      }
    }
  }
  for (; r < r1; ++r) {
#pragma unroll
    for (int k = 0; k < GN_MAX_SLOTS4; ++k)
      if (threadIdx.x + k * T < nq) add(k, src[k][(size_t)r * ld[k]]);
  }
#pragma unroll
  for (int k = 0; k < GN_MAX_SLOTS4; ++k) {
    const int qd = threadIdx.x + k * T;
    if (qd < nq) *(f32x4_t*)(part + 4 * qd) = (f32x4_t){sl[k], ql[k], sh[k], qh[k]};
  }
  __syncthreads();
  for (int i = threadIdx.x; i < 2 * groups; i += T) {
    const int gi = i >> 1, which = i & 1;
    const int p0 = gi * (cpg >> 1), p1 = p0 + (cpg >> 1);
    float a = 0.f;
    for (int pr = p0; pr < p1; ++pr) a += part[2 * pr + which];
    atomicAdd(&stats[(size_t)b * groups * 2 + i], (double)a);
  }
}

constexpr int GN_MAX_C = 3072;
template <bool TWO>
__global__ __launch_bounds__(256) void gn_apply_kernel(const float* x, const float* x2, int C1, void* y, void* raw16, int out_dt,
                                                       const float* gamma, const float* beta, const double* stats,
                                                       int HW, int C, int groups, float eps, int silu,
                                                       int rows_per_block, int hw_total) {
  __shared__ __attribute__((aligned(16))) float s_sc[GN_MAX_C], s_sh[GN_MAX_C];
  const int b = blockIdx.y;
  const int r0 = blockIdx.x * rows_per_block;
  const int r1 = min(HW, r0 + rows_per_block);
  const int n4 = C >> 2, cpg = C / groups;
  const double cnt = (double)hw_total * cpg;
  for (int c = threadIdx.x; c < C; c += 256) {
    const int g = c / cpg;
    const double su = stats[((size_t)b * groups + g) * 2], sq = stats[((size_t)b * groups + g) * 2 + 1];
    const double mean = su / cnt;
    double var = sq / cnt - mean * mean;
    if (var < 0) var = 0;
    const float rstd = (float)(1.0 / sqrt(var + (double)eps));
    const float ga = gamma[c] * rstd;
    s_sc[c] = ga;
    s_sh[c] = beta[c] - (float)mean * ga;
  }
  __syncthreads();
  const size_t base4 = ((size_t)b * HW + r0) * n4;
  const int total = (r1 - r0) * n4;
  const f32x4_t* x4 = (const f32x4_t*)x + (TWO ? 0 : base4);
  const f32x4_t* x4b = (const f32x4_t*)x2;
  const int n4a = C1 >> 2, n4b = n4 - n4a;
  const size_t row_base = (size_t)b * HW + r0;
  auto fetch = [&](int i, int row, int q) -> f32x4_t {
    if (!TWO) return x4[i];
    return q < n4a ? x4[(row_base + row) * n4a + q] : x4b[(row_base + row) * n4b + (q - n4a)];
  };
  auto store_planes = [&](void* dst, int row, int qi, const f32x4_t v) {
    unsigned short h[4], l[4];
#pragma unroll
    for (int e = 0; e < 4; ++e) {
      h[e] = BF16::from_f32(v[e]);
      l[e] = BF16::from_f32(v[e] - BF16::to_f32(h[e]));
    }
    u32x2_t oh, ol;
    oh[0] = h[0] | ((unsigned)h[1] << 16); oh[1] = h[2] | ((unsigned)h[3] << 16);
    ol[0] = l[0] | ((unsigned)l[1] << 16); ol[1] = l[2] | ((unsigned)l[3] << 16);
    u32x2_t* o = (u32x2_t*)dst + (row_base + row) * 3 * n4 + qi;
    o[0] = oh;
    o[n4] = oh;
    o[2 * n4] = ol;
  };
  auto store_planes2 = [&](void* dst, int row, int qi, const f32x4_t v) {
    unsigned short h[4], l[4];
#pragma unroll
    for (int e = 0; e < 4; ++e) {
      h[e] = F16::from_f32(__builtin_amdgcn_fmed3f(v[e], -65504.f, 65504.f));
      l[e] = F16::from_f32(v[e] - F16::to_f32(h[e]));
    }
    u32x2_t oh, ol;
    oh[0] = h[0] | ((unsigned)h[1] << 16); oh[1] = h[2] | ((unsigned)h[3] << 16);
    ol[0] = l[0] | ((unsigned)l[1] << 16); ol[1] = l[2] | ((unsigned)l[3] << 16);
    u32x2_t* o = (u32x2_t*)dst + (row_base + row) * 2 * n4 + qi;
    o[0] = oh;
    o[n4] = ol;
  };
  auto one = [&](int i, int row, int qi, const f32x4_t v) {
    f32x4_t o = v * *(const f32x4_t*)(s_sc + 4 * qi) + *(const f32x4_t*)(s_sh + 4 * qi);
    if (silu) {
#pragma unroll
      for (int e = 0; e < 4; ++e) o[e] = silu_f(o[e]);
    }
    if (out_dt == SX_BF16X3) {
      store_planes(y, row, qi, o);
      if (raw16) store_planes(raw16, row, qi, v);
      return;
    }
    if (out_dt == SX_F16X2) {
      store_planes2(y, row, qi, o);
      if (raw16) store_planes2(raw16, row, qi, v);
      return;
    }
    store4(y, out_dt, base4 + i, o);
    if (raw16) store4(raw16, out_dt, base4 + i, v);
  };
  const int step = 256 % n4, dstep = 256 / n4;
  int qi = threadIdx.x % n4, ri = threadIdx.x / n4;
  int i = threadIdx.x;
  auto adv = [&](int& r_, int& q_) { q_ += step; r_ += dstep; if (q_ >= n4) { q_ -= n4; ++r_; } };
  for (; i + 768 < total; i += 1024) {
    int q1 = qi, r1_ = ri; adv(r1_, q1);
    int q2 = q1, r2_ = r1_; adv(r2_, q2);
    int q3 = q2, r3_ = r2_; adv(r3_, q3);
    const f32x4_t v0 = fetch(i, ri, qi), v1 = fetch(i + 256, r1_, q1), v2 = fetch(i + 512, r2_, q2), v3 = fetch(i + 768, r3_, q3);
    one(i, ri, qi, v0);
    one(i + 256, r1_, q1, v1);
    one(i + 512, r2_, q2, v2);
    one(i + 768, r3_, q3, v3);
    qi = q3; ri = r3_; adv(ri, qi);
  }
  for (; i < total; i += 256) {
    one(i, ri, qi, fetch(i, ri, qi));
    adv(ri, qi);
  }
}

template <typename TT, bool F32OUT = false>
__global__ __launch_bounds__(256) void softmax_rows_kernel(const float* x, long ldx, unsigned short* y, long ldy, int C,
                                                           float scale) {
  __shared__ float red[4];
  const int tid = threadIdx.x, lane = tid & 63, wave = tid >> 6;
  const float4* xr = (const float4*)(x + (size_t)blockIdx.x * ldx);
  unsigned short* yr = y + (size_t)blockIdx.x * ldy;
  const int n4 = C >> 2;
  const float sl2 = scale * 1.4426950408889634f;
  float m = -INFINITY;
  for (int i = tid; i < n4; i += 256) {
    const float4 v = xr[i];
    m = fmaxf(fmaxf(m, fmaxf(v.x, v.y)), fmaxf(v.z, v.w));
  }
  m = wave_max(m);
  if (lane == 0) red[wave] = m;
  __syncthreads();
  m = fmaxf(fmaxf(red[0], red[1]), fmaxf(red[2], red[3])) * sl2;
  __syncthreads();
  float sum = 0.f;
  for (int i = tid; i < n4; i += 256) {
    const float4 v = xr[i];
    sum += exp2f(v.x * sl2 - m) + exp2f(v.y * sl2 - m) + exp2f(v.z * sl2 - m) + exp2f(v.w * sl2 - m);
  }
  sum = wave_sum(sum);
  if (lane == 0) red[wave] = sum;
  __syncthreads();
  const float inv = 1.f / (red[0] + red[1] + red[2] + red[3]);
  for (int i = tid; i < n4; i += 256) {
    const float4 v = xr[i];
    if (F32OUT) {
      ((float4*)((float*)y + (size_t)blockIdx.x * ldy))[i] =
          make_float4(exp2f(v.x * sl2 - m) * inv, exp2f(v.y * sl2 - m) * inv, exp2f(v.z * sl2 - m) * inv, exp2f(v.w * sl2 - m) * inv);
      continue;
    }
    u32x2_t o;
    o[0] = pack2<TT>(exp2f(v.x * sl2 - m) * inv, exp2f(v.y * sl2 - m) * inv);
    o[1] = pack2<TT>(exp2f(v.z * sl2 - m) * inv, exp2f(v.w * sl2 - m) * inv);
    *(u32x2_t*)(yr + 4 * i) = o;
  }
}

}
using namespace sxk_norm;

extern "C" int sx_layernorm(const void* x, int in_dtype, void* y, int out_dtype, const float* gamma,
                            const float* beta, int rows, int cols, float eps, int rms, void* stream) {
  SX_CHECK(x && y && gamma, "sx_layernorm: null pointer");
  SX_CHECK(rows > 0 && cols > 0 && cols % 4 == 0, "sx_layernorm: rows=%d cols=%d (cols %% 4 must be 0)", rows, cols);
  const bool tiled = (out_dtype & SX_TILED16) != 0;
  SX_CHECK(!tiled || (rows <= 32 && cols % 32 == 0 && ((out_dtype & 0xff) == SX_F16 || (out_dtype & 0xff) == SX_BF16)),
           "sx_layernorm: SX_TILED16 needs rows <= 32, cols %% 32 == 0 and a 16-bit output (rows=%d cols=%d)", rows, cols);
  SX_CHECK((out_dtype & 0xff) >= SX_F16 && (out_dtype & 0xff) <= SX_F32 && (out_dtype & ~0x1ff) == 0, "sx_layernorm: bad out dtype");
  hipStream_t st = (hipStream_t)stream;
  const dim3 grid((rows + 3) / 4), block(256);
  const int n4 = cols / 4;
  SX_CHECK(n4 <= 64 * 24, "sx_layernorm: cols=%d exceeds the register-resident limit (6144)", cols);
#define SX_LN_GO(DT, NV) \
  hipLaunchKernelGGL((layernorm_kernel<DT, NV>), grid, block, 0, st, x, y, out_dtype, gamma, beta, rows, cols, eps, rms)
#define SX_LN_NV(DT)                        \
  if (n4 <= 64 * 3) { SX_LN_GO(DT, 3); }    \
  else if (n4 <= 64 * 5) { SX_LN_GO(DT, 5); }  \
  else if (n4 <= 64 * 8) { SX_LN_GO(DT, 8); }  \
  else if (n4 <= 64 * 16) { SX_LN_GO(DT, 16); } \
  else { SX_LN_GO(DT, 24); }
  if (rows <= 32) {
    const dim3 g1(rows);
    switch (in_dtype) {
      case SX_F32: hipLaunchKernelGGL(layernorm_block_kernel<SX_F32>, g1, block, 0, st, x, y, out_dtype, gamma, beta, rows, cols, eps, rms); break;
      case SX_F16: hipLaunchKernelGGL(layernorm_block_kernel<SX_F16>, g1, block, 0, st, x, y, out_dtype, gamma, beta, rows, cols, eps, rms); break;
      case SX_BF16: hipLaunchKernelGGL(layernorm_block_kernel<SX_BF16>, g1, block, 0, st, x, y, out_dtype, gamma, beta, rows, cols, eps, rms); break;
      default: SX_FAIL("sx_layernorm: bad in dtype %d", in_dtype);
    }
    SX_HIP_LAUNCH_CHECK();
    return SX_OK;
  }
  switch (in_dtype) {
    case SX_F32: SX_LN_NV(SX_F32) break;
    case SX_F16: SX_LN_NV(SX_F16) break;
    case SX_BF16: SX_LN_NV(SX_BF16) break;
    default:
      SX_FAIL("sx_layernorm: bad in dtype %d", in_dtype);
  }
#undef SX_LN_NV
#undef SX_LN_GO
  SX_HIP_LAUNCH_CHECK();
  return SX_OK;
}

static int groupnorm_impl(const float* x, const float* x2, int C1, void* y, void* raw16, int out_dtype, const float* gamma,
                          const float* beta, double* stats, int B, int HW, int hw_total, int C, int groups, float eps,
                          int silu, int phase, void* stream) {
  SX_CHECK(x && stats, "sx_groupnorm: null pointer");
  SX_CHECK(phase == 1 || (y && gamma && beta), "sx_groupnorm: null pointer");
  SX_CHECK(!x2 || (C1 > 0 && C1 < C && C1 % 4 == 0 && (C - C1) % 4 == 0), "sx_groupnorm2: C1=%d of C=%d", C1, C);
  SX_CHECK(phase == 1 || out_dtype == SX_F16 || out_dtype == SX_BF16 || out_dtype == SX_BF16X3 || out_dtype == SX_F16X2 ||
               (out_dtype == SX_F32 && !raw16),
           "sx_groupnorm: output must be 16-bit, SX_BF16X3, SX_F16X2, or fp32 without a raw copy");
  SX_CHECK(groups > 0 && groups <= 64 && C % groups == 0, "sx_groupnorm: C=%d groups=%d", C, groups);
  SX_CHECK(C % 4 == 0 && (C / groups) % 2 == 0, "sx_groupnorm: C %% 4 and (C/groups) %% 2 must be 0 (C=%d)", C);
  SX_CHECK(C / 2 <= 256 * GN_MAX_SLOTS2 && C <= GN_MAX_C, "sx_groupnorm: C=%d too large", C);
  SX_CHECK(hw_total >= HW && HW > 0, "sx_groupnorm: hw_total=%d < HW=%d", hw_total, HW);
  hipStream_t st = (hipStream_t)stream;
  int rows_per_block = (HW * B + 2047) / 2048;
  if (rows_per_block < 4) rows_per_block = 4;
  const dim3 grid((HW + rows_per_block - 1) / rows_per_block, B), block(256);
  const int nq = C / 4;
  const int T = (nq % 320 == 0) ? 320 : ((nq % 160 == 0) ? 160 : ((nq <= 128) ? 128 : 256));
  SX_CHECK((nq + T - 1) / T <= GN_MAX_SLOTS4, "sx_groupnorm: C=%d too large", C);
  if (phase != 2) {
    hipLaunchKernelGGL(gn_zero_kernel, dim3((2 * B * groups + 255) / 256), dim3(256), 0, st, stats, 2 * B * groups);
    SX_HIP_LAUNCH_CHECK();
    long nblk = g_gn_stat_blocks;
    if (nblk <= 0) {
      nblk = ((long)B * HW * C * 4) >> 18;
      nblk = nblk < 512 ? 512 : (nblk > 2048 ? 2048 : nblk);
    }
    int rows_stats = (int)(((long)HW * B + nblk - 1) / nblk);
    if (rows_stats < 8) rows_stats = 8;
    const dim3 grid_s((HW + rows_stats - 1) / rows_stats, B);
    if (x2)
      hipLaunchKernelGGL(gn_stats_kernel<true>, grid_s, dim3(T), 0, st, x, x2, C1, stats, HW, C, groups, rows_stats);
    else
      hipLaunchKernelGGL(gn_stats_kernel<false>, grid_s, dim3(T), 0, st, x, x2, C, stats, HW, C, groups, rows_stats);
    SX_HIP_LAUNCH_CHECK();
  }
  if (phase != 1) {
    if (x2)
      hipLaunchKernelGGL(gn_apply_kernel<true>, grid, block, 0, st, x, x2, C1, y, raw16, out_dtype, gamma, beta, stats, HW, C,
                         groups, eps, silu, rows_per_block, hw_total);
    else
      hipLaunchKernelGGL(gn_apply_kernel<false>, grid, block, 0, st, x, x2, C, y, raw16, out_dtype, gamma, beta, stats, HW, C,
                         groups, eps, silu, rows_per_block, hw_total);
    SX_HIP_LAUNCH_CHECK();
  }
  return SX_OK;
}

extern "C" int sx_norm_tune(int key, int value) {
  if (key == 0 && (value == 0 || (value >= 64 && value <= 65536))) { g_gn_stat_blocks = value; return SX_OK; }
  SX_FAIL("sx_norm_tune: unknown key %d / value %d", key, value);
}

extern "C" int sx_groupnorm2(const float* x, const float* x2, int C1, void* y, void* raw16, int out_dtype, const float* gamma,
                             const float* beta, double* stats, int B, int HW, int C, int groups, float eps, int silu,
                             void* stream) {
  return groupnorm_impl(x, x2, C1, y, raw16, out_dtype, gamma, beta, stats, B, HW, HW, C, groups, eps, silu, 0, stream);
}

extern "C" int sx_groupnorm_sp(const float* x, const float* x2, int C1, void* y, void* raw16, int out_dtype, const float* gamma,
                               const float* beta, double* stats, int B, int HW, int hw_total, int C, int groups, float eps,
                               int silu, int phase, void* stream) {
  SX_CHECK(phase == 1 || phase == 2, "sx_groupnorm_sp: phase must be 1 (statistics) or 2 (apply)");
  return groupnorm_impl(x, x2, C1, y, raw16, out_dtype, gamma, beta, stats, B, HW, hw_total, C, groups, eps, silu, phase, stream);
}

extern "C" int sx_groupnorm(const float* x, void* y, void* raw16, int out_dtype, const float* gamma,
                            const float* beta, double* stats, int B, int HW, int C, int groups, float eps, int silu,
                            void* stream) {
  return sx_groupnorm2(x, nullptr, 0, y, raw16, out_dtype, gamma, beta, stats, B, HW, C, groups, eps, silu, stream);
}

extern "C" int sx_softmax_rows(const float* x, int64_t ldx, void* y, int64_t ldy, int rows, int cols, float scale,
                               int out_dtype, void* stream) {
  SX_CHECK(x && y, "sx_softmax_rows: null pointer");
  SX_CHECK(rows > 0 && cols > 0 && cols % 4 == 0 && ldx % 4 == 0 && ldy % 4 == 0, "sx_softmax_rows: rows=%d cols=%d", rows, cols);
  SX_CHECK(scale > 0.f, "sx_softmax_rows: scale must be positive");
  SX_CHECK(out_dtype >= SX_F16 && out_dtype <= SX_F32, "sx_softmax_rows: bad output dtype");
  hipStream_t st = (hipStream_t)stream;
  if (out_dtype == SX_F32)
    hipLaunchKernelGGL((softmax_rows_kernel<BF16, true>), dim3(rows), dim3(256), 0, st, x, (long)ldx, (unsigned short*)y, (long)ldy, cols, scale);
  else if (out_dtype == SX_BF16)
    hipLaunchKernelGGL(softmax_rows_kernel<BF16>, dim3(rows), dim3(256), 0, st, x, (long)ldx, (unsigned short*)y, (long)ldy, cols, scale);
  else
    hipLaunchKernelGGL(softmax_rows_kernel<F16>, dim3(rows), dim3(256), 0, st, x, (long)ldx, (unsigned short*)y, (long)ldy, cols, scale);
  SX_HIP_LAUNCH_CHECK();
  return SX_OK;
}
```

seed-x_amd/ops.py:

```python
import ctypes as C
import math

import os

import torch

from . import _lib
from ._lib import (SX_A_CONV3X3, SX_A_LINEAR, SX_ACT_GELU, SX_ACT_NONE, SX_ACT_SILU, SX_BF16, SX_F16, SX_F32,
                   AttnArgs, AttnSmallArgs, GemmArgs, GemvArgs, check)

_DT = {torch.float16: SX_F16, torch.bfloat16: SX_BF16, torch.float32: SX_F32}
_TD = {v: k for k, v in _DT.items()}
ACT = {None: SX_ACT_NONE, "none": SX_ACT_NONE, "gelu": SX_ACT_GELU, "silu": SX_ACT_SILU}


def dt_code(dtype):
    return _DT[dtype]


def _stream():
    return C.c_void_p(torch.cuda.current_stream().cuda_stream)


def _p(t):
    if t is None:
        return None
    if not t.is_cuda:
        raise RuntimeError("seedx_amd.ops: tensors must live on the GPU (no CPU fallback)")
    return C.c_void_p(t.data_ptr())


def _f32c(t):
    if t is None:
        return None
    assert t.dtype == torch.float32 and t.is_contiguous(), "expected contiguous fp32 tensor"
    return t


class GnStats:
    __slots__ = ("buf", "groups", "rows", "ready")

    def __init__(self, buf, groups, rows):
        self.buf, self.groups, self.rows, self.ready = buf, int(groups), int(rows), False

    @staticmethod
    def arena(n, B, groups, device):
        return torch.zeros((n, B, groups, 2), dtype=torch.float64, device=device)


class LnRows:
    __slots__ = ("x16", "stats")

    def __init__(self, M, C, dtype, device, stats=None):
        self.x16 = torch.empty((M, C), dtype=dtype, device=device)
        self.stats = stats if stats is not None else torch.zeros((M, 2), dtype=torch.float64, device=device)
        assert self.stats.shape == (M, 2) and self.stats.dtype == torch.float64 and self.stats.is_contiguous()


def gemm_tile(M, N, K, glu=False, conv=False):
    return int(_lib.load().sx_gemm_pick_tile(int(M), int(N), int(K), 1 if glu else 0, 1 if conv else 0))


def ln_fold_ok(M, C, consumers, producers):
    return all(gemm_tile(M, n, C, glu) >= 7 for n, glu in consumers) and all(gemm_tile(M, C, k) >= 7 for k in producers)


def fold_layernorm(w, bias, gamma, beta):
    wf = (w.float() * gamma.float()[None, :]).to(w.dtype).contiguous()
    cs = wf.float().sum(dim=1).contiguous()
    b = w.float() @ beta.float()
    if bias is not None:
        b = b + bias.float()
    return wf, cs, b.contiguous()


GN_FUSE = os.environ.get("SX_GN_FUSE", "1") != "0"


def _launch_gemm(lib, args, gn, what):
    if gn is None or not GN_FUSE:
        check(lib.sx_gemm(C.byref(args), _stream()), what)
        return
    assert gn.buf.dtype == torch.float64 and gn.buf.is_contiguous() and args.M % gn.rows == 0 \
        and gn.buf.numel() == (args.M // gn.rows) * gn.groups * 2, "GnStats does not describe this output"
    fused = C.c_int32(0)
    check(lib.sx_gemm_gn(C.byref(args), gn.buf.data_ptr(), gn.groups, gn.rows, C.byref(fused), _stream()), what)
    gn.ready = bool(fused.value)


def gemm(a, w, bias=None, bias2d=None, bias2d_rows=0, residual=None, res_mod=0, act=None, glu=False,
         out_dtype=None, out=None, n_valid=0, ld_bias2d=0, gn=None, ln_emit=None, ln_apply=None, a_planes=1):
    lib = _lib.load()
    assert a.dim() == 2 and w.dim() == 2 and a.is_contiguous() and w.is_contiguous()
    assert a.dtype == w.dtype and a.dtype in (torch.float16, torch.bfloat16)
    M, K = a.shape
    N = w.shape[0]
    assert a_planes in (1, 2) and K % a_planes == 0
    K //= a_planes
    assert w.shape[1] == K, f"K mismatch {a.shape} vs {w.shape} (a_planes {a_planes})"
    n_out = N // 2 if glu else N
    n_store = n_valid if n_valid else n_out
    out_dtype = out_dtype or a.dtype
    if out is None:
        out = torch.empty((M, n_store), dtype=out_dtype, device=a.device)
    assert out.dtype == out_dtype and out.stride(-1) == 1 and out.shape[0] == M
    args = GemmArgs()
    args.A, args.W, args.C = a.data_ptr(), w.data_ptr(), out.data_ptr()
    args.bias = _f32c(bias).data_ptr() if bias is not None else None
    if bias2d is not None:
        assert bias2d.dtype == torch.float32 and bias2d.stride(-1) == 1
        args.bias2d = bias2d.data_ptr()
        args.ld_bias2d = ld_bias2d or bias2d.stride(0)
    if residual is not None:
        assert residual.dtype == torch.float32 and residual.stride(-1) == 1
        args.residual = residual.data_ptr()
        args.ldr = residual.stride(0)
    args.M, args.N, args.K = M, N, K
    args.ldc = out.stride(0)
    args.n_valid = n_valid
    args.res_mod = res_mod
    args.bias2d_rows = bias2d_rows
    args.dtype = _DT[a.dtype]
    args.out_dtype = _DT[out_dtype]
    args.act = ACT[act]
    args.glu = 1 if glu else 0
    args.a_mode = SX_A_LINEAR
    args.a_planes = a_planes
    if ln_emit is not None or ln_apply is not None:
        assert gn is None and not (ln_emit is not None and ln_apply is not None)
        la = _lib.GemmLnArgs()
        if ln_emit is not None:
            assert ln_emit.x16.shape == (M, N) and ln_emit.x16.dtype == a.dtype and ln_emit.stats.shape[0] == M
            la.x16_out, la.ld_x16, la.row_stats_out = ln_emit.x16.data_ptr(), ln_emit.x16.stride(0), ln_emit.stats.data_ptr()
        else:
            rows, colsum, eps = ln_apply
            assert rows.stats.shape[0] == M and colsum.dtype == torch.float32 and colsum.numel() == N and colsum.is_contiguous()
            la.row_stats_in, la.colsum, la.dim, la.eps = rows.stats.data_ptr(), colsum.data_ptr(), K, float(eps)
        check(lib.sx_gemm_ln(C.byref(args), C.byref(la), _stream()), "sx_gemm_ln")
        return out
    _launch_gemm(lib, args, gn, "sx_gemm")
    return out


def conv3x3(x, w, bias=None, bias2d=None, residual=None, stride=1, upsample=False, out_dtype=None, act=None,
            n_valid=0, pad_mode=0, gn=None):
    lib = _lib.load()
    assert x.dim() == 4 and x.is_contiguous() and w.is_contiguous()
    B, H, W, Cin = x.shape
    Cout, K = w.shape
    assert K == 9 * Cin
    hv, wv = (2 * H, 2 * W) if upsample else (H, W)
    padsum = 1 if pad_mode else 2
    Hout, Wout = (hv + padsum - 3) // stride + 1, (wv + padsum - 3) // stride + 1
    M = B * Hout * Wout
    out_dtype = out_dtype or x.dtype
    n_store = n_valid if n_valid else Cout
    out = torch.empty((M, n_store), dtype=out_dtype, device=x.device)
    args = GemmArgs()
    args.A, args.W, args.C = x.data_ptr(), w.data_ptr(), out.data_ptr()
    args.bias = _f32c(bias).data_ptr() if bias is not None else None
    args.n_valid = n_valid
    if bias2d is not None:
        assert bias2d.dtype == torch.float32 and bias2d.stride(-1) == 1 and bias2d.shape == (B, Cout)
        args.bias2d = bias2d.data_ptr()
        args.bias2d_rows = Hout * Wout
        args.ld_bias2d = bias2d.stride(0)
    if residual is not None:
        assert residual.dtype == torch.float32 and residual.stride(-1) == 1
        args.residual = residual.data_ptr()
        args.ldr = residual.stride(0)
    args.M, args.N, args.K = M, Cout, K
    args.ldc = n_store
    args.dtype = _DT[x.dtype]
    args.out_dtype = _DT[out_dtype]
    args.act = ACT[act]
    args.a_mode = SX_A_CONV3X3
    args.B, args.Hin, args.Win, args.Cin, args.Hout, args.Wout = B, H, W, Cin, Hout, Wout
    args.stride = stride
    args.upsample = 1 if upsample else 0
    args.pad_mode = pad_mode
    _launch_gemm(lib, args, gn, "sx_gemm(conv3x3)")
    return out.view(B, Hout * Wout, n_store)


def pack_decode_tiles(w):
    N, K = w.shape
    assert N % 16 == 0 and K % 32 == 0
    return w.view(N // 16, 16, K // 32, 32).permute(0, 2, 1, 3).contiguous().view(N, K)


def pack_decode_tiles20(w):
    N, K = w.shape
    assert N % 20 == 0 and K % 32 == 0
    return w.view(N // 20, 20, K // 32, 32).permute(0, 2, 1, 3).contiguous().view(N, K)


def _fp8_row_order(codes):
    K = codes.shape[-1]
    return codes.reshape(*codes.shape[:-1], K // 64, 2, 4, 8).transpose(-3, -2).reshape(*codes.shape[:-1], K // 64, 64)


def pack_decode_tiles_fp8(codes):
    N, K = codes.shape
    assert codes.dtype == torch.uint8 and N % 16 == 0 and K % 64 == 0
    return _fp8_row_order(codes).view(N // 16, 16, K // 64, 64).permute(0, 2, 1, 3).contiguous()


def pack_decode_tiles20_fp8(codes):
    N, K = codes.shape
    assert codes.dtype == torch.uint8 and N % 20 == 0 and K % 64 == 0
    return _fp8_row_order(codes).view(N // 20, 20, K // 64, 64).permute(0, 2, 1, 3).contiguous()


class Tiled16:
    __slots__ = ("t", "rows", "cols", "planes")

    def __init__(self, rows, cols, dtype, device, planes=1):
        assert rows <= 32 and cols % 32 == 0 and planes in (1, 2)
        nb = planes * ((rows + 15) // 16)
        self.t, self.rows, self.cols, self.planes = torch.empty((nb, cols // 32, 16, 32), dtype=dtype, device=device), rows, cols, planes

    @property
    def dtype(self):
        return self.t.dtype

    def dense(self):
        nb = self.t.shape[0]
        d = self.t.permute(0, 2, 1, 3).reshape(nb * 16, self.cols)
        if self.planes == 2:
            half = (nb // 2) * 16
            return d[:self.rows].float() + d[half:half + self.rows].float()
        return d[:self.rows].contiguous()


def gemv(x, w, residual=None, act=None, glu=False, out_dtype=None, w_tiles=None, y_tiled=False, workspace=None,
         emit_norm=False, ssq_in=None, w_tiles20=None, planes_out=False, norm_gamma=None, w_fp8=None):
    lib = _lib.load()
    xt = isinstance(x, Tiled16)
    if xt:
        M, K = x.rows, x.cols
        assert x.dtype == w.dtype and (x.planes == 2 or w_tiles is not None or w_tiles20 is not None or w_fp8 is not None)
    else:
        assert x.dim() == 2 and x.is_contiguous() and w.is_contiguous() and x.dtype == w.dtype
        M, K = x.shape
    N = w.shape[0]
    n_out = N // 2 if glu else N
    out_dtype = out_dtype or x.dtype
    dev = x.t.device if xt else x.device
    if y_tiled:
        yt = Tiled16(M, n_out, out_dtype, dev, planes=2 if planes_out else 1)
        y = yt.t
    else:
        y = torch.empty((M, n_out), dtype=out_dtype, device=dev)
    args = GemvArgs()
    args.x, args.W, args.y = (x.t if xt else x).data_ptr(), w.data_ptr(), y.data_ptr()
    args.x_layout = 1 if xt else 0
    args.x_planes = x.planes if xt else 1
    if workspace is not None:
        args.workspace, args.workspace_bytes = workspace.data_ptr(), workspace.numel() * workspace.element_size()
    if residual is not None:
        assert residual.dtype == torch.float32 and residual.is_contiguous() and residual.shape == (M, n_out)
        args.residual = residual.data_ptr()
    args.M, args.N, args.K = M, N, K
    args.dtype, args.out_dtype, args.act, args.glu = _DT[x.dtype], _DT[out_dtype], ACT[act], 1 if glu else 0
    if y_tiled:
        args.out_dtype |= _lib.SX_TILED16
    if planes_out:
        assert y_tiled or emit_norm
        args.out_planes = 1
    if w_tiles is not None and (xt or y_tiled or M >= 5) and K % 64 == 0 and K >= 256 and N % 32 == 0:
        assert w_tiles.shape == w.shape and w_tiles.dtype == w.dtype and w_tiles.is_contiguous()
        args.W, args.w_layout = w_tiles.data_ptr(), 1
    if w_tiles20 is not None and not glu and (xt or y_tiled or M >= 5) and K % 64 == 0 and K >= 256 and N % 32 == 0 and N % 20 == 0:
        assert w_tiles20.shape == w.shape and w_tiles20.dtype == w.dtype and w_tiles20.is_contiguous()
        args.W, args.w_layout = w_tiles20.data_ptr(), 2
    if w_fp8 is not None:
        t8, sc = w_fp8
        assert t8.dtype == torch.uint8 and t8.is_contiguous() and t8.dim() == 4 and t8.shape[2] in (16, 20) and t8.shape[3] == 64
        assert t8.shape[0] * t8.shape[2] == N and t8.shape[1] * 64 == K and t8.device == dev, "FP8 tiles do not match the weight's shape"
        assert sc.dtype == torch.float32 and sc.is_contiguous() and sc.shape == (N,) and sc.device == dev
        args.W, args.w_layout = t8.data_ptr(), 1 if t8.shape[2] == 16 else 2
        args.w_dtype, args.w_scale = _lib.SX_FP8_E4M3, sc.data_ptr()
    x16 = ssq = None
    if emit_norm:
        assert args.w_layout in (1, 2) and out_dtype == torch.float32 and not glu and not y_tiled
        x16 = Tiled16(M, n_out, w.dtype, dev, planes=2 if planes_out else 1)
        if norm_gamma is not None:
            assert norm_gamma.dtype == torch.float32 and norm_gamma.is_contiguous() and norm_gamma.numel() == n_out
            args.x16_gamma = norm_gamma.data_ptr()
        ssq = torch.empty((16 * ((M + 15) // 16), lib.sx_gemv_ssq_parts(N, 0, args.w_layout)), dtype=torch.float32, device=dev)
        args.x16_out, args.row_ssq_out = x16.t.data_ptr(), ssq.data_ptr()
    if ssq_in is not None:
        t, dim, eps = ssq_in
        assert args.w_layout == 1 and t.dtype == torch.float32 and t.is_contiguous() and t.shape[0] == 16 * ((M + 15) // 16)
        args.row_ssq_in, args.ssq_in_parts, args.ssq_dim, args.ssq_eps = t.data_ptr(), t.shape[1], int(dim), float(eps)
    check(lib.sx_gemv(C.byref(args), _stream()), "sx_gemv")
    out = yt if y_tiled else y
    return (out, x16, ssq) if emit_norm else out


def linear(x, w, **kw):
    M, K, N = x.shape[0], x.shape[1], w.shape[0]
    skinny_ok = M <= 8 or (K % 64 == 0 and K >= 256 and N % 32 == 0)
    if M <= 16 and skinny_ok and kw.get("bias") is None and kw.get("bias2d") is None and not kw.get("res_mod") \
            and kw.get("out") is None and not kw.get("n_valid"):
        res = kw.get("residual")
        if res is None or res.is_contiguous():
            return gemv(x, w, residual=res, act=kw.get("act"), glu=kw.get("glu", False), out_dtype=kw.get("out_dtype"),
                        w_tiles=kw.get("w_tiles"))
    kw.pop("w_tiles", None)
    return gemm(x, w, **kw)


def layernorm(x, gamma, beta, eps, out_dtype, rms=False, tiled=False):
    lib = _lib.load()
    assert x.is_contiguous()
    cols = x.shape[-1]
    rows = x.numel() // cols
    if tiled:
        yt = Tiled16(rows, cols, out_dtype, x.device)
        y, code = yt.t, _DT[out_dtype] | _lib.SX_TILED16
    else:
        y, code = torch.empty(x.shape, dtype=out_dtype, device=x.device), _DT[out_dtype]
    check(lib.sx_layernorm(_p(x), _DT[x.dtype], _p(y), code, _p(_f32c(gamma)), _p(_f32c(beta)), rows, cols,
                           float(eps), 1 if rms else 0, _stream()), "sx_layernorm")
    return yt if tiled else y


def rmsnorm(x, gamma, eps, out_dtype, tiled=False):
    return layernorm(x, gamma, None, eps, out_dtype, rms=True, tiled=tiled)


def groupnorm(x, gamma, beta, groups, eps, silu, out_dtype, want_raw=False, x2=None, comm=None, hw_total=None, planes=False,
              stats=None):
    lib = _lib.load()
    assert x.dtype == torch.float32 and x.is_contiguous() and x.dim() == 3
    B, HW, C1 = x.shape
    Cc = C1
    if x2 is not None:
        assert x2.dtype == torch.float32 and x2.is_contiguous() and x2.shape[:2] == (B, HW)
        Cc = C1 + x2.shape[2]
    if planes == 2:
        out_dtype, code, cols = torch.float16, _lib.SX_F16X2, 2 * Cc
    elif planes:
        out_dtype, code, cols = torch.bfloat16, _lib.SX_BF16X3, 3 * Cc
    else:
        code, cols = _DT[out_dtype], Cc
    y = torch.empty((B, HW, cols), dtype=out_dtype, device=x.device)
    raw = torch.empty((B, HW, cols), dtype=out_dtype, device=x.device) if want_raw else None
    if stats is not None and stats.ready and x2 is None and (comm is None or comm.world == 1):
        assert stats.groups == groups and stats.rows == HW and stats.buf.numel() == B * groups * 2
        check(lib.sx_groupnorm_sp(_p(x), None, C1, _p(y), _p(raw), code, _p(_f32c(gamma)), _p(_f32c(beta)), _p(stats.buf), B, HW, HW,
                                  Cc, groups, float(eps), 1 if silu else 0, 2, _stream()), "sx_groupnorm_sp(apply, fused statistics)")
        return (y, raw) if want_raw else y
    stats = torch.empty((B, groups, 2), dtype=torch.float64, device=x.device)
    if comm is None or comm.world == 1:
        check(lib.sx_groupnorm2(_p(x), _p(x2), C1, _p(y), _p(raw), code, _p(_f32c(gamma)), _p(_f32c(beta)), _p(stats),
                                B, HW, Cc, groups, float(eps), 1 if silu else 0, _stream()), "sx_groupnorm")
    else:
        args = (_p(x), _p(x2), C1, _p(y), _p(raw), code, _p(_f32c(gamma)), _p(_f32c(beta)), _p(stats), B, HW,
                int(hw_total), Cc, groups, float(eps), 1 if silu else 0)
        check(lib.sx_groupnorm_sp(*args, 1, _stream()), "sx_groupnorm_sp(stats)")
        comm.all_reduce(stats)
        check(lib.sx_groupnorm_sp(*args, 2, _stream()), "sx_groupnorm_sp(apply)")
    return (y, raw) if want_raw else y


def softmax_rows(x, scale, out_dtype):
    lib = _lib.load()
    assert x.dtype == torch.float32 and x.dim() == 2 and x.stride(1) == 1
    R, Cc = x.shape
    y = torch.empty((R, Cc), dtype=out_dtype, device=x.device)
    check(lib.sx_softmax_rows(_p(x), x.stride(0), _p(y), y.stride(0), R, Cc, float(scale), _DT[out_dtype], _stream()),
          "sx_softmax_rows")
    return y


def _bshd_strides(t):
    assert t.dim() == 4 and t.stride(3) == 1, "expected a [B, S, H, D] view with unit stride on D"
    return t.stride(0), t.stride(1), t.stride(2)


def attention(q, k, v, scale, causal=False, out=None):
    lib = _lib.load()
    B, Sq, H, D = q.shape
    Skv = k.shape[1]
    assert k.shape == (B, Skv, H, D) and v.shape == (B, Skv, H, D) and q.dtype == k.dtype == v.dtype
    if out is None:
        out = torch.empty((B, Sq, H * D), dtype=q.dtype, device=q.device)
    a = AttnArgs()
    a.Q, a.K, a.V, a.O = q.data_ptr(), k.data_ptr(), v.data_ptr(), out.data_ptr()
    a.B, a.H, a.Sq, a.Skv, a.D = B, H, Sq, Skv, D
    a.q_batch_stride, a.q_row_stride, a.q_head_stride = _bshd_strides(q)
    a.k_batch_stride, a.k_row_stride, a.k_head_stride = _bshd_strides(k)
    a.v_batch_stride, a.v_row_stride, a.v_head_stride = _bshd_strides(v)
    a.o_batch_stride, a.o_row_stride = out.stride(0), out.stride(1)
    a.scale = float(scale)
    a.causal = 1 if causal else 0
    a.dtype = _DT[q.dtype]
    check(lib.sx_attention(C.byref(a), _stream()), "sx_attention")
    return out


def attention_small(q, k, v, scale):
    lib = _lib.load()
    B, Sq, H, D = q.shape
    Skv = k.shape[1]
    out = torch.empty((B, Sq, H * D), dtype=q.dtype, device=q.device)
    a = AttnSmallArgs()
    a.Q, a.K, a.V, a.O = q.data_ptr(), k.data_ptr(), v.data_ptr(), out.data_ptr()
    a.B, a.H, a.Sq, a.Skv, a.D = B, H, Sq, Skv, D
    a.q_batch_stride, a.q_row_stride, a.q_head_stride = _bshd_strides(q)
    a.k_batch_stride, a.k_row_stride, a.k_head_stride = _bshd_strides(k)
    a.v_batch_stride, a.v_row_stride, a.v_head_stride = _bshd_strides(v)
    a.o_batch_stride, a.o_row_stride = out.stride(0), out.stride(1)
    a.scale = float(scale)
    a.dtype = _DT[q.dtype]
    check(lib.sx_attention_small(C.byref(a), _stream()), "sx_attention_small")
    return out


def attn_decode(q, kcache, vcache, ctx_len_dev, scale, nsplit=8):
    lib = _lib.load()
    H, D = q.shape
    Tmax = kcache.shape[1]
    out = torch.empty((1, H * D), dtype=q.dtype, device=q.device)
    scratch = torch.empty((H, nsplit, D + 2), dtype=torch.float32, device=q.device)
    check(lib.sx_attn_decode(_p(q), _p(kcache), _p(vcache), _p(out), _p(scratch), _p(ctx_len_dev), H, D, Tmax, nsplit,
                             float(scale), _DT[q.dtype], _stream()), "sx_attn_decode")
    return out


def _planes_out(rows, cols, dtype, device, tiled):
    if tiled:
        t = Tiled16(rows, cols, dtype, device, planes=2)
        return t, t.t, _DT[dtype] | _lib.SX_TILED16
    y = torch.empty((rows, 2 * cols), dtype=dtype, device=device)
    return y, y, _DT[dtype]


def split16(x, dtype, tiled=False):
    assert x.dtype == torch.float32 and x.dim() == 2 and x.stride(1) == 1
    rows, cols = x.shape
    ret, buf, code = _planes_out(rows, cols, dtype, x.device, tiled)
    check(_lib.load().sx_split16(_p(x), x.stride(0), _p(buf), rows, cols, code, _stream()), "sx_split16")
    return ret


def rmsnorm_planes(x, gamma, eps, dtype, tiled=False, want_f32=False, want_planes=True):
    assert x.dtype == torch.float32 and x.dim() == 2 and x.is_contiguous()
    rows, cols = x.shape
    ret = buf = None
    code = _DT[dtype]
    if want_planes:
        ret, buf, code = _planes_out(rows, cols, dtype, x.device, tiled)
    y32 = torch.empty_like(x) if want_f32 else None
    check(_lib.load().sx_rmsnorm_planes(_p(x), _p(_f32c(gamma)), _p(y32), _p(buf), rows, cols, float(eps), code, _stream()),
          "sx_rmsnorm_planes")
    return ret, y32


def _kv_scales_ok(kv_scales, kcache, vcache):
    ks, vs = kv_scales
    assert kcache.dtype == torch.uint8 and vcache.dtype == torch.uint8 and kcache.shape[3] == 128
    assert ks.dtype == torch.float32 and vs.dtype == torch.float32 and ks.shape == kcache.shape[:3] and vs.shape == ks.shape \
        and ks[0].is_contiguous() and vs.stride() == ks.stride()
    return ks, vs


def rope_kv_append_f32(qkv, kcache, vcache, cos_tab, sin_tab, pos_dev, G, T, H, D, table_dtype, kv_scales=None, kv_emulate=False):
    assert qkv.dtype == torch.float32 and qkv.is_contiguous() and qkv.shape == (G * T, 3 * H * D)
    assert kcache.dim() == 4 and kcache.shape[0] == G and kcache[0].is_contiguous() and vcache.stride() == kcache.stride()
    if kv_scales is not None or kv_emulate:
        assert not (kv_scales is not None and kv_emulate)
        if kv_emulate:
            assert kcache.dtype == torch.float32 and vcache.dtype == torch.float32
            ks = vs = None
        else:
            ks, vs = _kv_scales_ok(kv_scales, kcache, vcache)
        check(_lib.load().sx_rope_kv_append_f32_q8(_p(qkv), _p(kcache), _p(vcache), _p(ks), _p(vs), _p(cos_tab), _p(sin_tab), _p(pos_dev),
                                                   G, T, H, D, kcache.shape[2], kcache.stride(0), 0 if ks is None else ks.stride(0),
                                                   _DT[table_dtype], 1 if kv_emulate else 0, _stream()), "sx_rope_kv_append_f32_q8")
        return
    assert kcache.dtype == torch.float32 and vcache.dtype in (torch.float32, table_dtype)
    fn = "sx_rope_kv_append_f32" if vcache.dtype == torch.float32 else "sx_rope_kv_append_f32_v16"
    check(getattr(_lib.load(), fn)(_p(qkv), _p(kcache), _p(vcache), _p(cos_tab), _p(sin_tab), _p(pos_dev), G, T, H, D,
                                   kcache.shape[2], kcache.stride(0), _DT[table_dtype], _stream()), fn)


def attention_f32(qkv, kcache, vcache, pos_dev, G, T, H, D, scale, dtype, tiled=False, nsplit=1, scratch=None, rope=None, kv_scales=None,
                  kv_emulate=False):
    assert qkv.dtype == torch.float32 and qkv.is_contiguous() and qkv.shape[0] == G * T and qkv.shape[1] >= H * D
    assert kcache.shape[0] == G and kcache.shape[1] == H and kcache.shape[3] == D and vcache.stride() == kcache.stride()
    ret, buf, code = _planes_out(G * T, H * D, dtype, qkv.device, tiled)
    a = _lib.AttnF32Args()
    if kv_scales is not None:
        assert not kv_emulate
        ks, vs = _kv_scales_ok(kv_scales, kcache, vcache)
        a.kv_fp8, a.k_scale, a.v_scale, a.scale_seq_stride = 1, _p(ks), _p(vs), ks.stride(0)
    else:
        assert kcache.dtype == torch.float32 and vcache.dtype in ((torch.float32,) if kv_emulate else (torch.float32, dtype))
        a.kv_fp8 = 2 if kv_emulate else 0
    a.q, a.kcache, a.vcache, a.out, a.pos0_dev = _p(qkv), _p(kcache), _p(vcache), _p(buf), _p(pos_dev)
    a.q_row_stride, a.cache_seq_stride = qkv.stride(0), kcache.stride(0)
    a.G, a.T, a.H, a.D, a.Tmax, a.dtype, a.scale, a.causal = G, T, H, D, kcache.shape[2], code, float(scale), 1
    a.v16 = 0 if vcache.dtype in (torch.float32, torch.uint8) else 1
    if nsplit > 1 and T == 1:
        if scratch is None:
            scratch = torch.empty((G, H, nsplit, D + 2), dtype=torch.float32, device=qkv.device)
        assert scratch.dtype == torch.float32 and scratch.numel() >= G * H * nsplit * (D + 2)
        a.nsplit, a.scratch = nsplit, _p(scratch)
    if rope is not None:
        assert T == 1 and D == 128 and qkv.shape[1] == 3 * H * D
        cos, sin = rope
        a.rope_cos, a.rope_sin = _p(cos), _p(sin)
        a.k_new, a.v_new = qkv.data_ptr() + 4 * H * D, qkv.data_ptr() + 8 * H * D
    check(_lib.load().sx_attention_f32(C.byref(a), _stream()), "sx_attention_f32")
    return ret


def attention_f32_full(q, k, v, scale, dtype):
    B, Sq, H, D = q.shape
    Skv = k.shape[1]
    assert q.dtype == k.dtype == v.dtype == torch.float32 and k.shape == (B, Skv, H, D) and v.shape == k.shape
    assert q.stride(3) == 1 and q.stride(2) == D and q.stride(0) == Sq * q.stride(1), "q rows must be [B*Sq] rows of H*D heads"
    assert k.stride(3) == 1 and v.stride() == k.stride()
    ret, buf, code = _planes_out(B * Sq, H * D, dtype, q.device, False)
    a = _lib.AttnF32Args()
    a.q, a.kcache, a.vcache, a.out, a.pos0_dev = _p(q), _p(k), _p(v), _p(buf), None
    a.q_row_stride, a.cache_seq_stride, a.kv_row_stride, a.kv_head_stride = q.stride(1), k.stride(0), k.stride(1), k.stride(2)
    a.G, a.T, a.H, a.D, a.Tmax, a.dtype, a.scale, a.causal = B, Sq, H, D, Skv, code, float(scale), 0
    check(_lib.load().sx_attention_f32(C.byref(a), _stream()), "sx_attention_f32")
    return ret


def linear_planes(x32, w, w_tiles=None, **kw):
    M, K = x32.shape
    N = w.shape[0]
    if M <= 32 and K % 64 == 0 and K >= 256 and N % 32 == 0:
        return gemv(split16(x32, w.dtype, tiled=True), w, w_tiles=w_tiles, **kw)
    return gemm(split16(x32, w.dtype), w, a_planes=2, **kw)


def rope_kv_append(qkv, kcache, vcache, cos_tab, sin_tab, pos0_dev, H, D):
    lib = _lib.load()
    T = qkv.shape[0]
    assert qkv.is_contiguous() and qkv.shape[1] == 3 * H * D
    check(lib.sx_rope_kv_append(_p(qkv), _p(kcache), _p(vcache), _p(cos_tab), _p(sin_tab), _p(pos0_dev), T, H, D,
                                kcache.shape[1], _DT[qkv.dtype], _stream()), "sx_rope_kv_append")


def embedding(ids_i32, table):
    lib = _lib.load()
    T = ids_i32.numel()
    out = torch.empty((T, table.shape[1]), dtype=torch.float32, device=table.device)
    check(lib.sx_embedding(_p(ids_i32), _p(table), _p(out), T, table.shape[1], _DT[table.dtype], _stream()),
          "sx_embedding")
    return out


def scatter_rows(src, rows_i32, dst):
    lib = _lib.load()
    assert src.dtype == torch.float32 and dst.dtype == torch.float32 and src.is_contiguous() and dst.is_contiguous()
    check(lib.sx_scatter_rows(_p(src), _p(rows_i32), _p(dst), src.shape[0], src.shape[1], _stream()),
          "sx_scatter_rows")


def greedy_next(logits, vocab, img_ids_dev, prev_id_dev, next_id_dev, out_ids=None, step_dev=None):
    lib = _lib.load()
    assert logits.dtype == torch.float32
    cap = out_ids.numel() if out_ids is not None else 0
    check(lib.sx_greedy_next_b(_p(logits), 0, vocab, _p(img_ids_dev), img_ids_dev.numel(), _p(prev_id_dev),
                               _p(next_id_dev), _p(out_ids), cap, _p(step_dev), 1, _stream()), "sx_greedy_next")


def cast(x, dtype):
    lib = _lib.load()
    assert x.is_contiguous()
    y = torch.empty(x.shape, dtype=dtype, device=x.device)
    check(lib.sx_cast(_p(x), _DT[x.dtype], _p(y), _DT[dtype], x.numel(), _stream()), "sx_cast")
    return y


OPERAND_PLANES = 1


def split_bf16(x, role="a"):
    lib = _lib.load()
    assert x.dtype == torch.float32 and x.is_contiguous() and x.shape[-1] % 4 == 0
    Cc = x.shape[-1]
    out = torch.empty(x.shape[:-1] + (3 * Cc,), dtype=torch.bfloat16, device=x.device)
    check(lib.sx_split_bf16(_p(x), _p(out), x.numel() // Cc, Cc, {"a": 0, "w": 1}[role], _stream()), "sx_split_bf16")
    return out


def copy2d(src, dst, dst_col_off=0):
    lib = _lib.load()
    assert src.dtype == torch.float32 and dst.dtype == torch.float32 and src.dim() == 2 and dst.dim() == 2
    assert src.stride(1) == 1 and dst.stride(1) == 1
    d = dst[:, dst_col_off:dst_col_off + src.shape[1]]
    check(lib.sx_copy2d_f32(_p(src), src.stride(0), C.c_void_p(d.data_ptr()), dst.stride(0), src.shape[0],
                            src.shape[1], _stream()), "sx_copy2d_f32")


def add(a, b):
    lib = _lib.load()
    assert a.dtype == torch.float32 and b.dtype == torch.float32 and a.is_contiguous() and b.is_contiguous()
    y = torch.empty_like(a)
    check(lib.sx_add_f32(_p(a), _p(b), _p(y), a.numel(), _stream()), "sx_add_f32")
    return y


def patchify(img, patch, kpad, dtype):
    lib = _lib.load()
    assert img.dtype == torch.float32 and img.is_contiguous() and img.shape[1] == 3 and img.shape[2] == img.shape[3]
    B, _, S, _ = img.shape
    g = S // patch
    out = torch.empty((B * g * g, kpad), dtype=dtype, device=img.device)
    check(lib.sx_patchify(_p(img), _p(out), B, S, patch, kpad, _DT[dtype], _stream()), "sx_patchify")
    return out


def im2col3x3_small(x, kpad, dtype):
    lib = _lib.load()
    assert x.dtype == torch.float32 and x.is_contiguous() and x.dim() == 4
    B, H, W, Cin = x.shape
    out = torch.empty((B * H * W, kpad), dtype=dtype, device=x.device)
    check(lib.sx_im2col3x3_small(_p(x), _p(out), B, H, W, Cin, kpad, _DT[dtype], _stream()), "sx_im2col3x3_small")
    return out


def avgpool_tokens(x, k):
    lib = _lib.load()
    assert x.dtype == torch.float32 and x.is_contiguous()
    B, L, D = x.shape
    y = torch.empty((B, L // k, D), dtype=torch.float32, device=x.device)
    check(lib.sx_avgpool_tokens(_p(x), _p(y), B, L, D, k, _stream()), "sx_avgpool_tokens")
    return y


def timestep_embedding(t, dim, dtype, idx_dev=None, n=None):
    lib = _lib.load()
    assert t.dtype == torch.float32
    n = n if n is not None else t.numel()
    out = torch.empty((n, dim), dtype=dtype, device=t.device)
    check(lib.sx_timestep_embedding(_p(t), _p(idx_dev), _p(out), n, dim, _DT[dtype], _stream()),
          "sx_timestep_embedding")
    return out


def nchw_to_nhwc(src, ld=None, dst=None):
    lib = _lib.load()
    B, Cc, H, W = src.shape
# ... 152 lines not shown
```

seed-x_amd/unet.py:

```python
import math
import os
import types

import torch

from . import ops
from .llama import glu_pack_rows

LN_FOLD = os.environ.get("SX_LN_FOLD", "1") != "0"

SDXL_BASE_CONFIG = dict(in_channels=4, out_channels=4, block_out_channels=(320, 640, 1280), layers_per_block=2,
                        down_attn=(False, True, True), up_attn=(True, True, False), transformer_layers=(1, 2, 10),
                        heads=(5, 10, 20), cross_attention_dim=2048, addition_time_embed_dim=256, pooled_dim=1280,
                        norm_groups=32, sample_size=128)


class UNetOutput:
    def __init__(self, sample):
        self.sample = sample


class UNet2DConditionModel:
    def __init__(self, comm=None, **cfg):
        from .parallel import Comm
        self.comm = comm or Comm()
        c = dict(SDXL_BASE_CONFIG)
        c.update(cfg)
        self.cfg = c
        self.config = types.SimpleNamespace(sample_size=c.get("sample_size", 128),
                                            addition_time_embed_dim=c["addition_time_embed_dim"],
                                            in_channels=c["in_channels"], out_channels=c["out_channels"])
        ted = c["block_out_channels"][0] * 4
        self.time_embed_dim = ted
        self.add_embedding = types.SimpleNamespace(
            linear_1=types.SimpleNamespace(in_features=6 * c["addition_time_embed_dim"] + c["pooled_dim"]))
        self.device, self.dtype = None, torch.float16
        self._sd, self._P = None, None
        self._ctx_key, self._ctx = None, None
        self._gn_arena, self._gn_next, self._n_gn_slots = None, 0, 64
        self._on_mark, self._mark_i, self._trace = None, 0, None
        self._ln_ok = {}

    @classmethod
    def from_pretrained(cls, path, subfolder=None, **kw):
        import json
        import os
        d = os.path.join(path, subfolder) if subfolder else path
        j = json.load(open(os.path.join(d, "config.json")))
        cfg = dict(in_channels=j["in_channels"], out_channels=j["out_channels"],
                   block_out_channels=tuple(j["block_out_channels"]), layers_per_block=j["layers_per_block"],
                   transformer_layers=tuple(j["transformer_layers_per_block"]), heads=tuple(j["attention_head_dim"]),
                   cross_attention_dim=j["cross_attention_dim"], addition_time_embed_dim=j["addition_time_embed_dim"],
                   pooled_dim=j["projection_class_embeddings_input_dim"] - 6 * j["addition_time_embed_dim"],
                   norm_groups=j["norm_num_groups"], sample_size=j["sample_size"],
                   down_attn=tuple("CrossAttn" in t for t in j["down_block_types"]),
                   up_attn=tuple("CrossAttn" in t for t in j["up_block_types"]))
        m = cls(**cfg)
        from safetensors.torch import load_file
        f = os.path.join(d, "diffusion_pytorch_model.safetensors")
        m.load_state_dict(load_file(f))
        return m

    def expand_conv_in(self, in_channels):
        if self.cfg["in_channels"] == in_channels:
            return
        if self._sd is None and self._P is not None:
            raise RuntimeError("UNet2DConditionModel: weights already packed; expand conv_in before the first forward")
        if self._sd is not None:
            w = self._sd["conv_in.weight"]
            new = torch.zeros((w.shape[0], in_channels, w.shape[2], w.shape[3]), dtype=w.dtype)
            new[:, :w.shape[1]] = w
            self._sd = dict(self._sd)
            self._sd["conv_in.weight"] = new
        self.cfg["in_channels"] = self.config.in_channels = in_channels
        self._P = None

    def load_state_dict(self, sd, strict=True, prefix="", merge=False):
        if prefix:
            sd = {k[len(prefix):]: v for k, v in sd.items() if k.startswith(prefix)}
        if merge and self._sd is not None:
            full = dict(self._sd)
            full.update(sd)
            sd = full
        need = ["conv_in.weight", "conv_out.weight", "time_embedding.linear_1.weight", "add_embedding.linear_2.bias",
                "mid_block.resnets.1.conv2.weight", "conv_norm_out.weight"]
        missing = [k for k in need if k not in sd]
        if missing and strict:
            raise KeyError(f"UNet2DConditionModel: missing keys {missing}")
        if "conv_in.weight" in sd and sd["conv_in.weight"].shape[1] != self.cfg["in_channels"]:
            self.cfg["in_channels"] = int(sd["conv_in.weight"].shape[1])
            self.config.in_channels = self.cfg["in_channels"]
        self._sd = sd
        self._P = None
        self._ctx_key = None
        return missing, []

    def to(self, device=None, dtype=None):
        old = (self.device, self.dtype)
        if device is not None:
            self.device = torch.device(device)
        if dtype is not None:
            assert dtype in (torch.float16, torch.bfloat16)
            self.dtype = dtype
        if (self.device, self.dtype) != old:
            if self._P is not None and self._sd is None:
                raise RuntimeError("weights were already packed for %s/%s; reload the state dict to move them" % old)
            self._P = None
            self._ctx_key = None
        return self

    def eval(self):
        return self

    def requires_grad_(self, flag=False):
        return self

    def _pack(self):
        if self._P is not None:
            return self._P
        if self._sd is None:
            raise RuntimeError("UNet2DConditionModel: load_state_dict() first")
        if self.device is None or self.device.type != "cuda":
            raise RuntimeError("UNet2DConditionModel runs on the GPU only")
        sd, dev, dt, c = self._sd, self.device, self.dtype, self.cfg

        def f32(k):
            return sd[k].detach().to(dev, torch.float32).contiguous()

        def lin16(k):
            return sd[k].detach().to(dev, dt).contiguous()

        def conv16(k):
            w = sd[k].detach().to(dev, dt)
            return w.permute(0, 2, 3, 1).reshape(w.shape[0], -1).contiguous()

        def resnet(n):
            r = dict(n1=(f32(n + ".norm1.weight"), f32(n + ".norm1.bias")), w1=conv16(n + ".conv1.weight"),
                     b1=f32(n + ".conv1.bias"), n2=(f32(n + ".norm2.weight"), f32(n + ".norm2.bias")),
                     w2=conv16(n + ".conv2.weight"), b2=f32(n + ".conv2.bias"), name=n)
            if n + ".conv_shortcut.weight" in sd:
                w = sd[n + ".conv_shortcut.weight"].detach().to(dev, dt)
                r["ws"] = w.reshape(w.shape[0], w.shape[1]).contiguous()
                r["bs"] = f32(n + ".conv_shortcut.bias")
            self._temb_names.append(n)
            return r

        def transformer(n, layers, heads):
            t = dict(norm=(f32(n + ".norm.weight"), f32(n + ".norm.bias")), pin_w=lin16(n + ".proj_in.weight"),
                     pin_b=f32(n + ".proj_in.bias"), pout_w=lin16(n + ".proj_out.weight"),
                     pout_b=f32(n + ".proj_out.bias"), heads=heads, blocks=[])
            for k in range(layers):
                b = f"{n}.transformer_blocks.{k}"
                ffw = sd[b + ".ff.net.0.proj.weight"].detach().to(dev, dt)
                ffb = sd[b + ".ff.net.0.proj.bias"].detach().to(dev, torch.float32)
                half = ffw.shape[0] // 2
                t["blocks"].append(dict(
                    n1=(f32(b + ".norm1.weight"), f32(b + ".norm1.bias")),
                    wqkv=torch.cat([lin16(b + f".attn1.{q}.weight") for q in ("to_q", "to_k", "to_v")], 0).contiguous(),
                    wo1=lin16(b + ".attn1.to_out.0.weight"), bo1=f32(b + ".attn1.to_out.0.bias"),
                    n2=(f32(b + ".norm2.weight"), f32(b + ".norm2.bias")),
                    wq2=lin16(b + ".attn2.to_q.weight"),
                    wkv2=torch.cat([lin16(b + ".attn2.to_k.weight"), lin16(b + ".attn2.to_v.weight")], 0).contiguous(),
                    wo2=lin16(b + ".attn2.to_out.0.weight"), bo2=f32(b + ".attn2.to_out.0.bias"),
                    n3=(f32(b + ".norm3.weight"), f32(b + ".norm3.bias")),
                    wff1=glu_pack_rows(ffw[:half].contiguous(), ffw[half:].contiguous()),
                    bff1=glu_pack_rows(ffb[:half].reshape(-1, 1).contiguous(), ffb[half:].reshape(-1, 1).contiguous()).reshape(-1).contiguous(),
                    wff2=lin16(b + ".ff.net.2.weight"), bff2=f32(b + ".ff.net.2.bias")))
            if LN_FOLD:
                for blk in t["blocks"]:
                    blk["f1"] = ops.fold_layernorm(blk["wqkv"], None, *blk["n1"])
                    blk["f2"] = ops.fold_layernorm(blk["wq2"], None, *blk["n2"])
                    blk["f3"] = ops.fold_layernorm(blk["wff1"], blk["bff1"], *blk["n3"])
            self._xattn.append(t)
            return t

        self._temb_names, self._xattn = [], []
        boc = c["block_out_channels"]
        P = {}
        cin = c["in_channels"]
        self.cin_kpad = (9 * cin + 63) // 64 * 64
        w = sd["conv_in.weight"].detach().to(dev, dt).permute(0, 2, 3, 1).reshape(boc[0], -1)
        wp = torch.zeros(boc[0], self.cin_kpad, dtype=dt, device=dev)
        wp[:, :w.shape[1]] = w
        P["conv_in_w"], P["conv_in_b"] = wp, f32("conv_in.bias")
        P["te1"] = (lin16("time_embedding.linear_1.weight"), f32("time_embedding.linear_1.bias"))
        P["te2"] = (lin16("time_embedding.linear_2.weight"), f32("time_embedding.linear_2.bias"))
        P["ae1"] = (lin16("add_embedding.linear_1.weight"), f32("add_embedding.linear_1.bias"))
        P["ae2"] = (lin16("add_embedding.linear_2.weight"), f32("add_embedding.linear_2.bias"))
        P["down"] = []
        for i, co in enumerate(boc):
            blk = dict(res=[], attn=[], down=None)
            for j in range(c["layers_per_block"]):
                blk["res"].append(resnet(f"down_blocks.{i}.resnets.{j}"))
                if c["down_attn"][i]:
                    blk["attn"].append(transformer(f"down_blocks.{i}.attentions.{j}", c["transformer_layers"][i], c["heads"][i]))
            if i != len(boc) - 1:
                n = f"down_blocks.{i}.downsamplers.0.conv"
                blk["down"] = (conv16(n + ".weight"), f32(n + ".bias"))
            P["down"].append(blk)
        P["mid"] = dict(res=[resnet("mid_block.resnets.0")], attn=[transformer("mid_block.attentions.0", c["transformer_layers"][-1], c["heads"][-1])])
        P["mid"]["res"].append(resnet("mid_block.resnets.1"))
        P["up"] = []
        rh, rl = list(reversed(c["heads"])), list(reversed(c["transformer_layers"]))
        for i in range(len(boc)):
            blk = dict(res=[], attn=[], up=None)
            for j in range(c["layers_per_block"] + 1):
                blk["res"].append(resnet(f"up_blocks.{i}.resnets.{j}"))
                if c["up_attn"][i]:
                    blk["attn"].append(transformer(f"up_blocks.{i}.attentions.{j}", rl[i], rh[i]))
            if i != len(boc) - 1:
                n = f"up_blocks.{i}.upsamplers.0.conv"
                blk["up"] = (conv16(n + ".weight"), f32(n + ".bias"))
            P["up"].append(blk)
        P["norm_out"] = (f32("conv_norm_out.weight"), f32("conv_norm_out.bias"))
        wo = conv16("conv_out.weight")
        wop = torch.zeros(16, wo.shape[1], dtype=dt, device=dev)
        wop[:wo.shape[0]] = wo
        bo = torch.zeros(16, dtype=torch.float32, device=dev)
        bo[:wo.shape[0]] = f32("conv_out.bias")
        P["conv_out_w"], P["conv_out_b"] = wop, bo
        ws = [sd[n + ".time_emb_proj.weight"].detach().to(dev, dt) for n in self._temb_names]
        bs = [sd[n + ".time_emb_proj.bias"].detach().to(dev, torch.float32) for n in self._temb_names]
        P["temb_w"], P["temb_b"] = torch.cat(ws, 0).contiguous(), torch.cat(bs, 0).contiguous()
        off, P["temb_off"] = 0, {}
        for n, w_ in zip(self._temb_names, ws):
            P["temb_off"][n] = (off, w_.shape[0])
            off += w_.shape[0]
        self._P = P
        self._sd = None
        return P

    def _gn(self, x, gb, eps, silu, Hc, Wc, want_raw=False, x2=None, stats=None):
        G, dt = self.cfg["norm_groups"], self.dtype
        return ops.groupnorm(x, gb[0], gb[1], G, eps, silu, dt, want_raw=want_raw, x2=x2, comm=self.comm, hw_total=Hc * Wc,
                             stats=stats)

    def _gn_slot(self, B, HW):
        if self._gn_arena is None:
            return None
        i = self._gn_next
        self._gn_next += 1
        if i >= self._gn_arena.shape[0]:
            return None
        return ops.GnStats(self._gn_arena[i], self.cfg["norm_groups"], HW)

    def _conv(self, h16, B, Hc, Wc, w, bias=None, bias2d=None, residual=None, stride=1, upsample=False, n_valid=0, gn=None):
        tp = self.comm.world
        Cin = h16.shape[-1]
        if tp == 1:
            return ops.conv3x3(h16.view(B, Hc, Wc, Cin), w, bias=bias, bias2d=bias2d, residual=residual, stride=stride,
                               upsample=upsample, out_dtype=torch.float32, n_valid=n_valid, gn=gn)
        from . import seqpar
        Hl = Hc // tp
        Co = n_valid or w.shape[0]
        if stride == 2:
            xin = seqpar.with_halo(h16, self.comm, Hl, Wc, left_col=True, bottom=False)
            out = ops.conv3x3(xin, w, bias=bias, bias2d=bias2d, stride=2, pad_mode=1, out_dtype=torch.float32)
            assert residual is None
            return out.view(B, (Hl // 2) * (Wc // 2), Co)
        xin = seqpar.with_halo(h16, self.comm, Hl, Wc)
        out = ops.conv3x3(xin, w, bias=bias, bias2d=bias2d, upsample=upsample, out_dtype=torch.float32, n_valid=n_valid)
        f = 2 if upsample else 1
        out = out.view(B, f * (Hl + 2), f * Wc, Co)[:, f:f * (Hl + 1)].reshape(B, f * Hl * f * Wc, Co).contiguous()
        if residual is not None:
            out = ops.add(out, residual.reshape(out.shape).contiguous())
        return out

    def _resnet(self, r, x, B, Hc, Wc, temb_all, skip=None, st_in=None):
        Ci = x.shape[-1] + (skip.shape[-1] if skip is not None else 0)
        if "ws" in r:
            h, raw = self._gn(x, r["n1"], 1e-5, True, Hc, Wc, want_raw=True, x2=skip)
        else:
            assert skip is None
            h = self._gn(x, r["n1"], 1e-5, True, Hc, Wc, stats=st_in)
        off, Co = self._P["temb_off"][r["name"]]
        HW = x.shape[1]
        st2 = self._gn_slot(B, HW)
        h = self._conv(h, B, Hc, Wc, r["w1"], bias=r["b1"], bias2d=temb_all[:, off:off + Co], gn=st2)
        h = self._gn(h, r["n2"], 1e-5, True, Hc, Wc, stats=st2)
        if "ws" in r:
            sc = ops.gemm(raw.view(-1, Ci), r["ws"], bias=r["bs"], out_dtype=torch.float32)
        else:
            sc = x.view(-1, Ci)
        st_out = self._gn_slot(B, HW)
        out = self._conv(h, B, Hc, Wc, r["w2"], bias=r["b2"], residual=sc, gn=st_out).view(B, -1, Co)
        self._mark(out)
        return out, st_out

    def _transformer(self, t, x, B, ctx_kv, Hc, Wc, st_in=None):
        dt, heads = self.dtype, t["heads"]
        _, HW, C = x.shape
        hd = C // heads
        scale = hd ** -0.5
        sp = self.comm.world > 1
        h = self._gn(x, t["norm"], 1e-6, False, Hc, Wc, stats=st_in)
        nb = len(t["blocks"])
        M = B * HW
        if LN_FOLD and not sp and "f1" in t["blocks"][0] and self._ln_fold_ok(M, C):
            arena = torch.zeros((3 * nb, M, 2), dtype=torch.float64, device=x.device)

            def rows(i):
                return ops.LnRows(M, C, dt, x.device, stats=arena[i])
            ln = rows(0)
            hs = ops.gemm(h.view(-1, C), t["pin_w"], bias=t["pin_b"], out_dtype=torch.float32, ln_emit=ln)
            for k, b in enumerate(t["blocks"]):
                w, cs, bb = b["f1"]
                qkv = ops.gemm(ln.x16, w, bias=bb, ln_apply=(ln, cs, 1e-5)).view(B, HW, 3, heads, hd)
                att = ops.attention(qkv[:, :, 0], qkv[:, :, 1], qkv[:, :, 2], scale)
                ln = rows(3 * k + 1)
                hs = ops.gemm(att.view(-1, C), b["wo1"], bias=b["bo1"], residual=hs, out_dtype=torch.float32, ln_emit=ln)
                self._mark(hs)
                w, cs, bb = b["f2"]
                q = ops.gemm(ln.x16, w, bias=bb, ln_apply=(ln, cs, 1e-5)).view(B, HW, heads, hd)
                kv = ctx_kv[k]
                att = ops.attention(q, kv[:, :, 0], kv[:, :, 1], scale)
                ln = rows(3 * k + 2)
                hs = ops.gemm(att.view(-1, C), b["wo2"], bias=b["bo2"], residual=hs, out_dtype=torch.float32, ln_emit=ln)
                w, cs, bb = b["f3"]
                g = ops.gemm(ln.x16, w, bias=bb, act="gelu", glu=True, ln_apply=(ln, cs, 1e-5))
                if k == nb - 1:
                    hs = ops.gemm(g, b["wff2"], bias=b["bff2"], residual=hs, out_dtype=dt)
                else:
                    ln = rows(3 * k + 3)
                    hs = ops.gemm(g, b["wff2"], bias=b["bff2"], residual=hs, out_dtype=torch.float32, ln_emit=ln)
                self._mark(hs)
            st_out = self._gn_slot(B, HW)
            out = ops.gemm(hs, t["pout_w"], bias=t["pout_b"], residual=x.view(-1, C), out_dtype=torch.float32, gn=st_out)
            return out.view(B, HW, C), st_out
        hs = ops.gemm(h.view(-1, C), t["pin_w"], bias=t["pin_b"], out_dtype=torch.float32)
        for k, b in enumerate(t["blocks"]):
            n = ops.layernorm(hs, b["n1"][0], b["n1"][1], 1e-5, dt)
            if not sp:
                qkv = ops.gemm(n, b["wqkv"]).view(B, HW, 3, heads, hd)
                att = ops.attention(qkv[:, :, 0], qkv[:, :, 1], qkv[:, :, 2], scale)
            else:
                from . import seqpar
                kv_l = ops.gemm(n, b["wqkv"][C:]).view(B, HW, 2, heads, hd)
                pending = self.comm.all_gather_async(kv_l)
                q = ops.gemm(n, b["wqkv"][:C]).view(B, HW, heads, hd)
                g = pending.wait()
                kv = g.permute(1, 0, 2, 3, 4, 5).reshape(B, g.shape[0] * HW, 2, heads, hd).contiguous()
                att = ops.attention(q, kv[:, :, 0], kv[:, :, 1], scale)
            hs = ops.gemm(att.view(-1, C), b["wo1"], bias=b["bo1"], residual=hs, out_dtype=torch.float32)
            self._mark(hs)
            n = ops.layernorm(hs, b["n2"][0], b["n2"][1], 1e-5, dt)
            q = ops.gemm(n, b["wq2"]).view(B, HW, heads, hd)
            kv = ctx_kv[k]
            att = ops.attention(q, kv[:, :, 0], kv[:, :, 1], scale)
            hs = ops.gemm(att.view(-1, C), b["wo2"], bias=b["bo2"], residual=hs, out_dtype=torch.float32)
            n = ops.layernorm(hs, b["n3"][0], b["n3"][1], 1e-5, dt)
            g = ops.gemm(n, b["wff1"], bias=b["bff1"], act="gelu", glu=True)
            last = k == nb - 1
            hs = ops.gemm(g, b["wff2"], bias=b["bff2"], residual=hs, out_dtype=dt if last else torch.float32)
            self._mark(hs)
        st_out = self._gn_slot(B, HW)
        out = ops.gemm(hs, t["pout_w"], bias=t["pout_b"], residual=x.view(-1, C), out_dtype=torch.float32, gn=st_out)
        return out.view(B, HW, C), st_out

    def _ln_fold_ok(self, M, C):
        key = (M, C)
        if key not in self._ln_ok:
            self._ln_ok[key] = ops.ln_fold_ok(M, C, consumers=[(3 * C, False), (C, False), (8 * C, True)], producers=[C, 4 * C])
        return self._ln_ok[key]

    def prepare_context(self, encoder_hidden_states):
        P = self._pack()
        ehs = encoder_hidden_states
        key = (ehs.data_ptr(), ehs._version, tuple(ehs.shape))
        if self._ctx_key == key:
            return self._ctx
        B, L, ca = ehs.shape
        e16 = ops.cast(ehs.to(self.device).float().contiguous(), self.dtype).view(B * L, ca)
        ctx = []
        for t in self._xattn:
            heads = t["heads"]
            per = []
            for b in t["blocks"]:
                C = b["wq2"].shape[0]
                kv = ops.gemm(e16, b["wkv2"]).view(B, L, 2, heads, C // heads)
                per.append(kv)
            ctx.append(per)
        self._ctx_key, self._ctx = key, ctx
        return ctx

    def time_embeddings(self, t_vals, idx_dev, text_embeds, time_ids, B):
        P, dt, c = self._P, self.dtype, self.cfg
        boc0 = c["block_out_channels"][0]
        ts = ops.timestep_embedding(t_vals, boc0, dt, idx_dev=idx_dev, n=B)
        e = ops.gemm(ts, P["te1"][0], bias=P["te1"][1], act="silu")
        e = ops.gemm(e, P["te2"][0], bias=P["te2"][1], out_dtype=torch.float32)
        tid = ops.timestep_embedding(time_ids.reshape(-1).float().contiguous(), c["addition_time_embed_dim"], torch.float32)
        add = torch.empty((B, self.add_embedding.linear_1.in_features), dtype=torch.float32, device=self.device)
        ops.copy2d(text_embeds.float().contiguous(), add, 0)
        ops.copy2d(tid.view(B, -1), add, text_embeds.shape[1])
        a = ops.gemm(ops.cast(add, dt), P["ae1"][0], bias=P["ae1"][1], act="silu")
        emb = ops.gemm(a, P["ae2"][0], bias=P["ae2"][1], residual=e, out_dtype=torch.float32)
        return ops.gemm(ops.silu_cast(emb, dt), P["temb_w"], bias=P["temb_b"], out_dtype=torch.float32)

    def _mark(self, t=None):
        if self._trace is not None and t is not None:
            self._trace.append(t.detach().float().clone())
        if self._on_mark is not None:
            self._mark_i += 1
            self._on_mark(self._mark_i)

    def forward_nhwc(self, x_in, temb_all, ctx, B, H, W, on_mark=None):
        P, dt, c = self._P, self.dtype, self.cfg
        self._on_mark, self._mark_i = on_mark, 0
        cin = c["in_channels"]
        tp, rank = self.comm.world, self.comm.rank
        if tp > 1:
            from . import seqpar
            assert H % (tp * 4) == 0, f"latent rows {H} must divide by 4 x the sharding degree {tp} (two 2x down-samplings)"
        col = ops.im2col3x3_small(x_in.view(B, H, W, cin), self.cin_kpad, dt)
        x = ops.gemm(col, P["conv_in_w"], bias=P["conv_in_b"], out_dtype=torch.float32).view(B, H * W, -1)
        if tp > 1:
            x = seqpar.local_rows(x, rank, tp, H, W)
        skips = [(x, H, W)]
        ti = 0
        Hc, Wc = H, W
        self._gn_arena = ops.GnStats.arena(self._n_gn_slots, B, c["norm_groups"], x.device) if tp == 1 else None
        self._gn_next = 0
        st = None
        for blk in P["down"]:
            for j, r in enumerate(blk["res"]):
                x, st = self._resnet(r, x, B, Hc, Wc, temb_all, st_in=st)
                if blk["attn"]:
                    x, st = self._transformer(blk["attn"][j], x, B, ctx[ti], Hc, Wc, st_in=st)
                    ti += 1
                skips.append((x, Hc, Wc))
            if blk["down"] is not None:
                st = self._gn_slot(B, (Hc // 2) * (Wc // 2))
                x = self._conv(ops.cast(x, dt), B, Hc, Wc, blk["down"][0], bias=blk["down"][1], stride=2, gn=st)
                Hc, Wc = Hc // 2, Wc // 2
                skips.append((x, Hc, Wc))
        x, st = self._resnet(P["mid"]["res"][0], x, B, Hc, Wc, temb_all, st_in=st)
        x, st = self._transformer(P["mid"]["attn"][0], x, B, ctx[ti], Hc, Wc, st_in=st)
        ti += 1
        x, st = self._resnet(P["mid"]["res"][1], x, B, Hc, Wc, temb_all, st_in=st)
        for blk in P["up"]:
            for j, r in enumerate(blk["res"]):
                s, _, _ = skips.pop()
                x, st = self._resnet(r, x.contiguous(), B, Hc, Wc, temb_all, skip=s)
                if blk["attn"]:
                    x, st = self._transformer(blk["attn"][j], x, B, ctx[ti], Hc, Wc, st_in=st)
                    ti += 1
            if blk["up"] is not None:
                x = self._conv(ops.cast(x, dt), B, Hc, Wc, blk["up"][0], bias=blk["up"][1], upsample=True)
                Hc, Wc = Hc * 2, Wc * 2
                st = None
        h = self._gn(x, P["norm_out"], 1e-5, True, Hc, Wc, stats=st)
        self._gn_arena = None
        self._on_mark = None
        nv = 4 if c["out_channels"] == 4 else 0
        out = self._conv(h, B, Hc, Wc, P["conv_out_w"], bias=P["conv_out_b"], n_valid=nv)
        out = out.view(B, -1, out.shape[-1])
        if tp > 1:
            out = seqpar.gather_rows(out, self.comm)
            if not torch.cuda.is_current_stream_capturing():
                self.comm.check()
        return out

    def forward(self, sample, timestep, encoder_hidden_states, added_cond_kwargs=None, cross_attention_kwargs=None,
                return_dict=True, **_):
        self._pack()
        assert added_cond_kwargs is not None and "text_embeds" in added_cond_kwargs and "time_ids" in added_cond_kwargs
        B, Cin, H, W = sample.shape
        assert Cin == self.cfg["in_channels"]
        dev = self.device
        t = torch.as_tensor(timestep, dtype=torch.float32, device=dev).reshape(-1)
        t = t.expand(B).contiguous() if t.numel() == 1 else t
        temb = self.time_embeddings(t, None, added_cond_kwargs["text_embeds"].to(dev), added_cond_kwargs["time_ids"].to(dev), B)
        ctx = self.prepare_context(encoder_hidden_states.to(dev))
        x = ops.nchw_to_nhwc(sample.to(dev, torch.float32))
        eps = self.forward_nhwc(x, temb, ctx, B, H, W)
        out = ops.nhwc_to_nchw(eps, self.cfg["out_channels"], H, W).to(sample.dtype if sample.dtype != torch.float64 else torch.float32)
        if not return_dict:
            return (out,)
        return UNetOutput(out)

    __call__ = forward
```

Measured before the change: 1.306.

## Fuse group-norm statistics for skip-concat inputs into producing GEMM epilogues

Adds a second group-norm statistics target to the GEMM epilogue and a partial-channel stats kernel. UNet up-block resnets read a concatenation of the current activation and a skip tensor, so the producers of each half now accumulate per-group sums into a shared slot at a channel offset. The decoder's GroupNorm over the concatenated input can then skip its separate statistics pass. The cost is extra atomics in the epilogue and more complex bookkeeping of which stats are ready, with a fallback stats kernel when fusion is not possible.

Result: no change. 1.313 (median of 6 runs) (+0.5%).

```diff
diff --git a/include/seedx_hip.h b/include/seedx_hip.h
--- a/include/seedx_hip.h
+++ b/include/seedx_hip.h
@@ -53,6 +53,8 @@
 } sx_gemm_args;
 int sx_gemm(const sx_gemm_args* args, void* stream);
 int sx_gemm_gn(const sx_gemm_args* args, double* stats, int groups, int rows_per_sample, int* fused_host, void* stream);
+int sx_gemm_gn2(const sx_gemm_args* args, double* stats, int groups, int rows_per_sample, int* fused_host, double* stats2,
+                int groups2, int c0, int c_total, int* fused2_host, void* stream);
 typedef struct sx_gemm_ln_args {
   void* x16_out;
   double* row_stats_out;
@@ -105,6 +107,8 @@
                  double* stats, int B, int HW, int C, int groups, float eps, int silu, void* stream);
 int sx_groupnorm2(const float* x, const float* x2, int C1, void* y, void* raw16, int out_dtype, const float* gamma,
                   const float* beta, double* stats, int B, int HW, int C, int groups, float eps, int silu, void* stream);
+int sx_groupnorm_stats_add(const float* x, int B, int HW, int C, double* stats, int groups, double* stats2, int groups2, int c0,
+                           int c_total, void* stream);
 int sx_norm_tune(int key, int value);
 int sx_groupnorm_sp(const float* x, const float* x2, int C1, void* y, void* raw16, int out_dtype, const float* gamma,
                     const float* beta, double* stats, int B, int HW, int hw_total, int C, int groups, float eps, int silu,
diff --git a/seed-x_amd/_lib.py b/seed-x_amd/_lib.py
--- a/seed-x_amd/_lib.py
+++ b/seed-x_amd/_lib.py
@@ -97,6 +97,7 @@
     "sx_version": [],
     "sx_gemm": [C.POINTER(GemmArgs), c_vp],
     "sx_gemm_gn": [C.POINTER(GemmArgs), c_vp, c_i32, c_i32, C.POINTER(c_i32), c_vp],
+    "sx_gemm_gn2": [C.POINTER(GemmArgs), c_vp, c_i32, c_i32, C.POINTER(c_i32), c_vp, c_i32, c_i32, c_i32, C.POINTER(c_i32), c_vp],
     "sx_gemm_ln": [C.POINTER(GemmArgs), C.POINTER(GemmLnArgs), c_vp],
     "sx_gemm_force_tile": [c_i32],
     "sx_gemm_debug_stamps": [c_vp],
@@ -110,6 +111,7 @@
     "sx_groupnorm2": [c_vp, c_vp, c_i32, c_vp, c_vp, c_i32, c_vp, c_vp, c_vp, c_i32, c_i32, c_i32, c_i32, c_f32, c_i32, c_vp],
     "sx_groupnorm_sp": [c_vp, c_vp, c_i32, c_vp, c_vp, c_i32, c_vp, c_vp, c_vp, c_i32, c_i32, c_i32, c_i32, c_i32, c_f32, c_i32,
                         c_i32, c_vp],
+    "sx_groupnorm_stats_add": [c_vp, c_i32, c_i32, c_i32, c_vp, c_i32, c_vp, c_i32, c_i32, c_i32, c_vp],
     "sx_attention": [C.POINTER(AttnArgs), c_vp],
     "sx_norm_tune": [c_i32, c_i32],
     "sx_gemv_tune": [c_i32, c_i32],
diff --git a/seed-x_amd/csrc/gemm.hip b/seed-x_amd/csrc/gemm.hip
--- a/seed-x_amd/csrc/gemm.hip
+++ b/seed-x_amd/csrc/gemm.hip
@@ -369,8 +369,10 @@
   return SX_OK;
 }
 
+struct Gn2 { double* stats; int groups, c0, c_total; int* fused; };
+
 static int gemm_impl(const sx_gemm_args* a, double* gn_stats, int gn_groups, int gn_rows, int* gn_fused, const sx_gemm_ln_args* ln,
-                     void* stream);
+                     void* stream, const Gn2* gn2 = nullptr);
 
 extern "C" int sx_gemm(const sx_gemm_args* a, void* stream) { return gemm_impl(a, nullptr, 0, 0, nullptr, nullptr, stream); }
 
@@ -384,10 +386,22 @@
   return gemm_impl(a, stats, groups, rows_per_sample, fused, nullptr, stream);
 }
 
+extern "C" int sx_gemm_gn2(const sx_gemm_args* a, double* stats, int groups, int rows_per_sample, int* fused, double* stats2, int groups2,
+                           int c0, int c_total, int* fused2, void* stream) {
+  SX_CHECK((stats || stats2) && rows_per_sample > 0, "sx_gemm_gn2: no statistics target / rows_per_sample");
+  SX_CHECK(!stats || (fused && groups > 0), "sx_gemm_gn2: bad arguments of the first target");
+  SX_CHECK(!stats2 || (fused2 && groups2 > 0 && c0 >= 0 && a && c0 + a->N <= c_total),
+           "sx_gemm_gn2: bad arguments of the second target (c0=%d c_total=%d groups2=%d)", c0, c_total, groups2);
+  if (fused) *fused = 0;
+  const Gn2 g2 = {stats2, groups2, c0, c_total, fused2};
+  return gemm_impl(a, stats, stats ? groups : 0, rows_per_sample, stats ? fused : nullptr, nullptr, stream, stats2 ? &g2 : nullptr);
+}
+
 static int gemm_impl(const sx_gemm_args* a, double* gn_stats, int gn_groups, int gn_rows, int* gn_fused, const sx_gemm_ln_args* ln,
-                     void* stream) {
+                     void* stream, const Gn2* gn2) {
   SX_CHECK(a && a->A && a->W && a->C, "sx_gemm: null pointer");
   if (gn_fused) *gn_fused = 0;
+  if (gn2) *gn2->fused = 0;
   SX_CHECK(a->dtype == SX_F16 || a->dtype == SX_BF16, "sx_gemm: dtype must be f16/bf16");
   SX_CHECK(a->out_dtype >= SX_F16 && a->out_dtype <= SX_F32, "sx_gemm: bad out_dtype");
   SX_CHECK(a->M > 0 && a->N > 0 && a->K > 0, "sx_gemm: empty problem M=%d N=%d K=%d", a->M, a->N, a->K);
@@ -437,7 +451,7 @@
   hipStream_t st = (hipStream_t)stream;
   p.res_init = (p.residual && p.act == SX_ACT_NONE && !p.glu) ? 1 : 0;
   if (ln) {
-    SX_CHECK(a->a_mode == SX_A_LINEAR && !gn_stats, "sx_gemm_ln: linear GEMMs only");
+    SX_CHECK(a->a_mode == SX_A_LINEAR && !gn_stats && !gn2, "sx_gemm_ln: linear GEMMs only");
     SX_CHECK(!(ln->row_stats_in && ln->row_stats_out), "sx_gemm_ln: a launch is a producer or a consumer, not both");
     if (ln->row_stats_out) {
       SX_CHECK(ln->x16_out && a->out_dtype == SX_F32 && !a->glu && a->act == SX_ACT_NONE && p.n_valid == a->N,
@@ -465,10 +479,16 @@
   }
   const int cfg = pick_tile(a->M, a->N, Kk, a->glu != 0, a->a_mode == SX_A_CONV3X3, g_force_tile, allow);
   if (cfg == 7 || cfg == 8) {
-    if (gn_stats && a->out_dtype == SX_F32 && !a->glu && a->act == SX_ACT_NONE && p.n_valid == a->N && a->N % gn_groups == 0 &&
-        (a->N / gn_groups) % 2 == 0 && gn_rows % 256 == 0 && a->M % gn_rows == 0) {
+    const bool gn_ok = a->out_dtype == SX_F32 && !a->glu && a->act == SX_ACT_NONE && p.n_valid == a->N && gn_rows > 0 &&
+                       gn_rows % 256 == 0 && a->M % gn_rows == 0;
+    if (gn_stats && gn_ok && a->N % gn_groups == 0 && (a->N / gn_groups) % 2 == 0) {
       p.gn_stats = gn_stats; p.gn_groups = gn_groups; p.gn_cpg = a->N / gn_groups; p.gn_rows = gn_rows;
       *gn_fused = 1;
+    }
+    if (gn2 && gn_ok && gn2->c_total % gn2->groups == 0 && (gn2->c_total / gn2->groups) % 2 == 0 && gn2->c0 % 2 == 0) {
+      p.gn2_stats = gn2->stats; p.gn2_groups = gn2->groups; p.gn2_cpg = gn2->c_total / gn2->groups; p.gn2_c0 = gn2->c0;
+      p.gn_rows = gn_rows;
+      *gn2->fused = 1;
     }
     return launch_pp(p, a->dtype, cfg == 7 ? 256 : 320, a->a_mode, st);
   }
diff --git a/seed-x_amd/csrc/gemm_common.h b/seed-x_amd/csrc/gemm_common.h
--- a/seed-x_amd/csrc/gemm_common.h
+++ b/seed-x_amd/csrc/gemm_common.h
@@ -20,6 +20,8 @@
   unsigned long long* dbg;
   double* gn_stats;
   int gn_cpg, gn_groups, gn_rows;
+  double* gn2_stats;
+  int gn2_cpg, gn2_groups, gn2_c0;
   void* ln_x16;
   double* ln_out;
   const double* ln_in;
diff --git a/seed-x_amd/csrc/gemm_pp.hip b/seed-x_amd/csrc/gemm_pp.hip
--- a/seed-x_amd/csrc/gemm_pp.hip
+++ b/seed-x_amd/csrc/gemm_pp.hip
@@ -298,7 +298,7 @@
     for (int i = 0; i < FN; ++i) lcs[i] = *(const f32x4_t*)(p.ln_cs + ncol[i]);
   }
   float lsum[LN == 2 ? FM : 1], lsq[LN == 2 ? FM : 1];
-  const bool gn = OUT32 && p.gn_stats != nullptr;
+  const bool gn = OUT32 && (p.gn_stats != nullptr || p.gn2_stats != nullptr);
   float gsl[FN], gql[FN], gsh[FN], gqh[FN];
 #pragma unroll
   for (int i = 0; i < FN; ++i) gsl[i] = gql[i] = gsh[i] = gqh[i] = 0.f;
@@ -453,9 +453,6 @@
       gqh[i] = row16_sum(gqh[i]);
     }
     float* gslot = (float*)smem;
-    const int gbase = n0 / p.gn_cpg;
-    const int nlast = (n0 + BN < p.N ? n0 + BN : p.N) - 1;
-    const int ngr = nlast / p.gn_cpg - gbase + 1;
     __syncthreads();
     if ((lane & 15) == 0) {
 #pragma unroll
@@ -466,17 +463,23 @@
     }
     __syncthreads();
     const int smp = m0 / p.gn_rows;
-    for (int t = tid; t < 2 * ngr; t += 512) {
-      const int G = gbase + (t >> 1), which = t & 1;
-      int c_lo = G * p.gn_cpg - n0, c_hi = (G + 1) * p.gn_cpg - n0;
-      c_lo = c_lo < 0 ? 0 : c_lo;
-      const int c_end = (p.N - n0 < BN ? p.N - n0 : BN);
-      c_hi = c_hi > c_end ? c_end : c_hi;
-      float acc = 0.f;
-      for (int cp = c_lo >> 1; cp < (c_hi >> 1); ++cp) acc += gslot[(size_t)cp * 2 + which];
-      for (int cp = c_lo >> 1; cp < (c_hi >> 1); ++cp) acc += gslot[((size_t)(BN / 2) + cp) * 2 + which];
-      atomicAdd(&p.gn_stats[((size_t)smp * p.gn_groups + G) * 2 + which], (double)acc);
-    }
+    const int c_end = (p.N - n0 < BN ? p.N - n0 : BN);
+    auto reduce_into = [&](double* stats, int cpg, int groups, int c0) {
+      const int gbase = (c0 + n0) / cpg;
+      const int ngr = (c0 + n0 + c_end - 1) / cpg - gbase + 1;
+      for (int t = tid; t < 2 * ngr; t += 512) {
+        const int G = gbase + (t >> 1), which = t & 1;
+        int c_lo = G * cpg - c0 - n0, c_hi = c_lo + cpg;
+        c_lo = c_lo < 0 ? 0 : c_lo;
+        c_hi = c_hi > c_end ? c_end : c_hi;
+        float acc = 0.f;
+        for (int cp = c_lo >> 1; cp < (c_hi >> 1); ++cp) acc += gslot[(size_t)cp * 2 + which];
+        for (int cp = c_lo >> 1; cp < (c_hi >> 1); ++cp) acc += gslot[((size_t)(BN / 2) + cp) * 2 + which];
+        atomicAdd(&stats[((size_t)smp * groups + G) * 2 + which], (double)acc);
+      }
+    };
+    if (p.gn_stats) reduce_into(p.gn_stats, p.gn_cpg, p.gn_groups, 0);
+    if (p.gn2_stats) reduce_into(p.gn2_stats, p.gn2_cpg, p.gn2_groups, p.gn2_c0);
   }
   if (p.dbg) {
     asm volatile("s_waitcnt vmcnt(0)" ::: "memory");
@@ -530,7 +533,7 @@
   const int e = epi_code(p, dtype);
   if (e < 0) return false;
   if (p.ln_in && !(a_mode == SX_A_LINEAR && (e == 0 || e == 2) && !p.ln_out)) return false;
-  if (p.ln_out && !(a_mode == SX_A_LINEAR && e == 4 && !p.gn_stats)) return false;
+  if (p.ln_out && !(a_mode == SX_A_LINEAR && e == 4 && !p.gn_stats && !p.gn2_stats)) return false;
   if (bn == 320 && (e == 2 || e == 3)) return false;
   if (a_mode == SX_A_CONV3X3 && !(e == 0 || e == 4)) return false;
   if (a_mode == SX_A_CONV3X3 && p.upsample && !(p.stride == 1 && p.pad == 1)) return false;
diff --git a/seed-x_amd/csrc/norm.hip b/seed-x_amd/csrc/norm.hip
--- a/seed-x_amd/csrc/norm.hip
+++ b/seed-x_amd/csrc/norm.hip
@@ -131,9 +131,9 @@
   if (i < n) p[i] = 0.0;
 }
 
-template <bool TWO>
+template <bool TWO, bool PART = false>
 __global__ __launch_bounds__(320) void gn_stats_kernel(const float* x, const float* x2, int C1, double* stats, int HW, int C,
-                                                       int groups, int rows_per_block) {
+                                                       int groups, int rows_per_block, double* stats2, int groups2, int c0, int ctot) {
   __shared__ __attribute__((aligned(16))) float part[GN_MAX_SLOTS4 * 320 * 4];
   const int T = blockDim.x;
   const int b = blockIdx.y;
@@ -182,12 +182,26 @@
     if (qd < nq) *(f32x4_t*)(part + 4 * qd) = (f32x4_t){sl[k], ql[k], sh[k], qh[k]};
   }
   __syncthreads();
-  for (int i = threadIdx.x; i < 2 * groups; i += T) {
-    const int gi = i >> 1, which = i & 1;
-    const int p0 = gi * (cpg >> 1), p1 = p0 + (cpg >> 1);
-    float a = 0.f;
-    for (int pr = p0; pr < p1; ++pr) a += part[2 * pr + which];
-    atomicAdd(&stats[(size_t)b * groups * 2 + i], (double)a);
+  if (!PART || stats) {
+    for (int i = threadIdx.x; i < 2 * groups; i += T) {
+      const int gi = i >> 1, which = i & 1;
+      const int p0 = gi * (cpg >> 1), p1 = p0 + (cpg >> 1);
+      float a = 0.f;
+      for (int pr = p0; pr < p1; ++pr) a += part[2 * pr + which];
+      atomicAdd(&stats[(size_t)b * groups * 2 + i], (double)a);
+    }
+  }
+  if (PART && stats2) {
+    const int cpg2 = ctot / groups2, g0 = c0 / cpg2, ng = (c0 + C - 1) / cpg2 - g0 + 1;
+    for (int i = threadIdx.x; i < 2 * ng; i += T) {
+      const int gi = g0 + (i >> 1), which = i & 1;
+      int lo = gi * cpg2 - c0, hi = lo + cpg2;
+      lo = lo < 0 ? 0 : lo;
+      hi = hi > C ? C : hi;
+      float a = 0.f;
+      for (int pr = lo >> 1; pr < (hi >> 1); ++pr) a += part[2 * pr + which];
+      atomicAdd(&stats2[((size_t)b * groups2 + gi) * 2 + which], (double)a);
+    }
   }
 }
 
@@ -415,9 +429,9 @@
     if (rows_stats < 8) rows_stats = 8;
     const dim3 grid_s((HW + rows_stats - 1) / rows_stats, B);
     if (x2)
-      hipLaunchKernelGGL(gn_stats_kernel<true>, grid_s, dim3(T), 0, st, x, x2, C1, stats, HW, C, groups, rows_stats);
+      hipLaunchKernelGGL(gn_stats_kernel<true>, grid_s, dim3(T), 0, st, x, x2, C1, stats, HW, C, groups, rows_stats, (double*)nullptr, 1, 0, C);
     else
-      hipLaunchKernelGGL(gn_stats_kernel<false>, grid_s, dim3(T), 0, st, x, x2, C, stats, HW, C, groups, rows_stats);
+      hipLaunchKernelGGL(gn_stats_kernel<false>, grid_s, dim3(T), 0, st, x, x2, C, stats, HW, C, groups, rows_stats, (double*)nullptr, 1, 0, C);
     SX_HIP_LAUNCH_CHECK();
   }
   if (phase != 1) {
@@ -429,6 +443,32 @@
                          groups, eps, silu, rows_per_block, hw_total);
     SX_HIP_LAUNCH_CHECK();
   }
+  return SX_OK;
+}
+
+extern "C" int sx_groupnorm_stats_add(const float* x, int B, int HW, int C, double* stats, int groups, double* stats2, int groups2,
+                                      int c0, int c_total, void* stream) {
+  SX_CHECK(x && (stats || stats2) && B > 0 && HW > 0, "sx_groupnorm_stats_add: null pointer / empty input");
+  SX_CHECK(C % 4 == 0 && C / 2 <= 256 * GN_MAX_SLOTS2 && C <= GN_MAX_C, "sx_groupnorm_stats_add: C=%d", C);
+  SX_CHECK(!stats || (groups > 0 && groups <= 64 && C % groups == 0 && (C / groups) % 2 == 0), "sx_groupnorm_stats_add: C=%d groups=%d", C,
+           groups);
+  SX_CHECK(!stats2 || (groups2 > 0 && groups2 <= 64 && c_total % groups2 == 0 && (c_total / groups2) % 2 == 0 && c0 >= 0 && c0 % 2 == 0 &&
+                       c0 + C <= c_total),
+           "sx_groupnorm_stats_add: c0=%d C=%d c_total=%d groups2=%d (channels per group and c0 must be even)", c0, C, c_total, groups2);
+  const int nq = C / 4;
+  const int T = (nq % 320 == 0) ? 320 : ((nq % 160 == 0) ? 160 : ((nq <= 128) ? 128 : 256));
+  SX_CHECK((nq + T - 1) / T <= GN_MAX_SLOTS4, "sx_groupnorm_stats_add: C=%d too large", C);
+  long nblk = g_gn_stat_blocks;
+  if (nblk <= 0) {
+    nblk = ((long)B * HW * C * 4) >> 18;
+    nblk = nblk < 512 ? 512 : (nblk > 2048 ? 2048 : nblk);
+  }
+  int rows_stats = (int)(((long)HW * B + nblk - 1) / nblk);
+  if (rows_stats < 8) rows_stats = 8;
+  const dim3 grid_s((HW + rows_stats - 1) / rows_stats, B);
+  hipLaunchKernelGGL((gn_stats_kernel<false, true>), grid_s, dim3(T), 0, (hipStream_t)stream, x, (const float*)nullptr, C, stats, HW, C,
+                     stats ? groups : 1, rows_stats, stats2, stats2 ? groups2 : 1, c0, stats2 ? c_total : C);
+  SX_HIP_LAUNCH_CHECK();
   return SX_OK;
 }
 
diff --git a/seed-x_amd/ops.py b/seed-x_amd/ops.py
--- a/seed-x_amd/ops.py
+++ b/seed-x_amd/ops.py
@@ -46,6 +46,32 @@
     @staticmethod
     def arena(n, B, groups, device):
         return torch.zeros((n, B, groups, 2), dtype=torch.float64, device=device)
+
+
+class GnCat:
+    __slots__ = ("buf", "groups", "rows", "c_x", "c_total", "ready")
+
+    def __init__(self, buf, groups, rows, c_x, c_total):
+        self.buf, self.groups, self.rows, self.c_x, self.c_total = buf, int(groups), int(rows), int(c_x), int(c_total)
+        self.ready = [False, False]
+
+    def share(self, part):
+        return GnShare(self, part)
+
+
+class GnShare:
+    __slots__ = ("cat", "part")
+
+    def __init__(self, cat, part):
+        self.cat, self.part = cat, int(part)
+
+    @property
+    def c0(self):
+        return self.cat.c_x if self.part else 0
+
+    @property
+    def width(self):
+        return self.cat.c_total - self.cat.c_x if self.part else self.cat.c_x
 
 
 class LnRows:
@@ -75,21 +101,39 @@
 
 
 GN_FUSE = os.environ.get("SX_GN_FUSE", "1") != "0"
-
-
-def _launch_gemm(lib, args, gn, what):
-    if gn is None or not GN_FUSE:
+GN_CONCAT = os.environ.get("SX_GN_CONCAT", "1") != "0"
+
+
+def _launch_gemm(lib, args, gn, what, gn2=None):
+    if not GN_FUSE:
+        gn = gn2 = None
+    if not GN_CONCAT:
+        gn2 = None
+    if gn is None and gn2 is None:
         check(lib.sx_gemm(C.byref(args), _stream()), what)
         return
-    assert gn.buf.dtype == torch.float64 and gn.buf.is_contiguous() and args.M % gn.rows == 0 \
-        and gn.buf.numel() == (args.M // gn.rows) * gn.groups * 2, "GnStats does not describe this output"
+    if gn is not None:
+        assert gn.buf.dtype == torch.float64 and gn.buf.is_contiguous() and args.M % gn.rows == 0 \
+            and gn.buf.numel() == (args.M // gn.rows) * gn.groups * 2, "GnStats does not describe this output"
     fused = C.c_int32(0)
-    check(lib.sx_gemm_gn(C.byref(args), gn.buf.data_ptr(), gn.groups, gn.rows, C.byref(fused), _stream()), what)
-    gn.ready = bool(fused.value)
+    if gn2 is None:
+        check(lib.sx_gemm_gn(C.byref(args), gn.buf.data_ptr(), gn.groups, gn.rows, C.byref(fused), _stream()), what)
+        gn.ready = bool(fused.value)
+        return
+    cat = gn2.cat
+    assert cat.buf.dtype == torch.float64 and cat.buf.is_contiguous() and args.M % cat.rows == 0 and gn2.width == args.N \
+        and cat.buf.numel() == (args.M // cat.rows) * cat.groups * 2 and (gn is None or gn.rows == cat.rows), \
+        "GnCat does not describe this output"
+    fused2 = C.c_int32(0)
+    check(lib.sx_gemm_gn2(C.byref(args), gn.buf.data_ptr() if gn is not None else None, gn.groups if gn is not None else 0, cat.rows,
+                          C.byref(fused), cat.buf.data_ptr(), cat.groups, gn2.c0, cat.c_total, C.byref(fused2), _stream()), what)
+    if gn is not None:
+        gn.ready = bool(fused.value)
+    cat.ready[gn2.part] = bool(fused2.value)
 
 
 def gemm(a, w, bias=None, bias2d=None, bias2d_rows=0, residual=None, res_mod=0, act=None, glu=False,
-         out_dtype=None, out=None, n_valid=0, ld_bias2d=0, gn=None, ln_emit=None, ln_apply=None, a_planes=1):
+         out_dtype=None, out=None, n_valid=0, ld_bias2d=0, gn=None, ln_emit=None, ln_apply=None, a_planes=1, gn2=None):
     lib = _lib.load()
     assert a.dim() == 2 and w.dim() == 2 and a.is_contiguous() and w.is_contiguous()
     assert a.dtype == w.dtype and a.dtype in (torch.float16, torch.bfloat16)
@@ -127,7 +171,7 @@
     args.a_mode = SX_A_LINEAR
     args.a_planes = a_planes
     if ln_emit is not None or ln_apply is not None:
-        assert gn is None and not (ln_emit is not None and ln_apply is not None)
+        assert gn is None and gn2 is None and not (ln_emit is not None and ln_apply is not None)
         la = _lib.GemmLnArgs()
         if ln_emit is not None:
             assert ln_emit.x16.shape == (M, N) and ln_emit.x16.dtype == a.dtype and ln_emit.stats.shape[0] == M
@@ -138,12 +182,12 @@
             la.row_stats_in, la.colsum, la.dim, la.eps = rows.stats.data_ptr(), colsum.data_ptr(), K, float(eps)
         check(lib.sx_gemm_ln(C.byref(args), C.byref(la), _stream()), "sx_gemm_ln")
         return out
-    _launch_gemm(lib, args, gn, "sx_gemm")
+    _launch_gemm(lib, args, gn, "sx_gemm", gn2)
     return out
 
 
 def conv3x3(x, w, bias=None, bias2d=None, residual=None, stride=1, upsample=False, out_dtype=None, act=None,
-            n_valid=0, pad_mode=0, gn=None):
+            n_valid=0, pad_mode=0, gn=None, gn2=None):
     lib = _lib.load()
     assert x.dim() == 4 and x.is_contiguous() and w.is_contiguous()
     B, H, W, Cin = x.shape
@@ -179,7 +223,7 @@
     args.stride = stride
     args.upsample = 1 if upsample else 0
     args.pad_mode = pad_mode
-    _launch_gemm(lib, args, gn, "sx_gemm(conv3x3)")
+    _launch_gemm(lib, args, gn, "sx_gemm(conv3x3)", gn2)
     return out.view(B, Hout * Wout, n_store)
 
 
@@ -331,6 +375,23 @@
     return layernorm(x, gamma, None, eps, out_dtype, rms=True, tiled=tiled)
 
 
+def groupnorm_stats_add(x, own=None, share=None):
+    lib = _lib.load()
+    assert x.dtype == torch.float32 and x.is_contiguous() and x.dim() == 3 and (own is not None or share is not None)
+    B, HW, Cx = x.shape
+    cat = share.cat if share is not None else None
+    assert own is None or (own.rows == HW and own.buf.numel() == B * own.groups * 2)
+    assert cat is None or (cat.rows == HW and cat.buf.numel() == B * cat.groups * 2 and share.width == Cx)
+    check(lib.sx_groupnorm_stats_add(_p(x), B, HW, Cx, _p(own.buf) if own is not None else None, own.groups if own is not None else 0,
+                                     _p(cat.buf) if cat is not None else None, cat.groups if cat is not None else 0,
+                                     share.c0 if cat is not None else 0, cat.c_total if cat is not None else 0, _stream()),
+          "sx_groupnorm_stats_add")
+    if own is not None:
+        own.ready = True
+    if cat is not None:
+        cat.ready[share.part] = True
+
+
 def groupnorm(x, gamma, beta, groups, eps, silu, out_dtype, want_raw=False, x2=None, comm=None, hw_total=None, planes=False,
               stats=None):
     lib = _lib.load()
@@ -348,7 +409,18 @@
         code, cols = _DT[out_dtype], Cc
     y = torch.empty((B, HW, cols), dtype=out_dtype, device=x.device)
     raw = torch.empty((B, HW, cols), dtype=out_dtype, device=x.device) if want_raw else None
-    if stats is not None and stats.ready and x2 is None and (comm is None or comm.world == 1):
+    single = comm is None or comm.world == 1
+    if isinstance(stats, GnCat):
+        cat, stats = stats, None
+        if x2 is not None and single and GN_FUSE and GN_CONCAT and any(cat.ready):
+            assert cat.groups == groups and cat.rows == HW and cat.c_x == C1 and cat.c_total == Cc and cat.buf.numel() == B * groups * 2
+            for part, t in ((0, x), (1, x2)):
+                if not cat.ready[part]:
+                    groupnorm_stats_add(t, share=cat.share(part))
+            check(lib.sx_groupnorm_sp(_p(x), _p(x2), C1, _p(y), _p(raw), code, _p(_f32c(gamma)), _p(_f32c(beta)), _p(cat.buf), B, HW, HW,
+                                      Cc, groups, float(eps), 1 if silu else 0, 2, _stream()), "sx_groupnorm_sp(apply, concat statistics)")
+            return (y, raw) if want_raw else y
+    if stats is not None and stats.ready and x2 is None and single:
         assert stats.groups == groups and stats.rows == HW and stats.buf.numel() == B * groups * 2
         check(lib.sx_groupnorm_sp(_p(x), None, C1, _p(y), _p(raw), code, _p(_f32c(gamma)), _p(_f32c(beta)), _p(stats.buf), B, HW, HW,
                                   Cc, groups, float(eps), 1 if silu else 0, 2, _stream()), "sx_groupnorm_sp(apply, fused statistics)")
diff --git a/seed-x_amd/unet.py b/seed-x_amd/unet.py
--- a/seed-x_amd/unet.py
+++ b/seed-x_amd/unet.py
@@ -38,6 +38,7 @@
         self._sd, self._P = None, None
         self._ctx_key, self._ctx = None, None
         self._gn_arena, self._gn_next, self._n_gn_slots = None, 0, 64
+        self._cats = None
         self._on_mark, self._mark_i, self._trace = None, 0, None
         self._ln_ok = {}
 
@@ -114,6 +115,30 @@
 
     def requires_grad_(self, flag=False):
         return self
+
+    def concat_plan(self):
+        c = self.cfg
+        boc, L = c["block_out_channels"], c["layers_per_block"]
+        skips = [(boc[0], 0, "conv_in")]
+        for i, co in enumerate(boc):
+            for j in range(L):
+                skips.append((co, i, f"down_blocks.{i}.attentions.{j}.proj_out" if c["down_attn"][i] else f"down_blocks.{i}.resnets.{j}.conv2"))
+            if i != len(boc) - 1:
+                skips.append((co, i + 1, f"down_blocks.{i}.downsamplers.0.conv"))
+        plan = []
+        cx, src = boc[-1], "mid_block.resnets.1.conv2"
+        for i, co in enumerate(reversed(boc)):
+            lvl = len(boc) - 1 - i
+            for j in range(L + 1):
+                cs, slvl, sname = skips.pop()
+                assert slvl == lvl
+                plan.append(dict(name=f"up_blocks.{i}.resnets.{j}", width=cx + cs, c_x=cx, c_skip=cs, level=lvl, x_from=src, skip_from=sname))
+                cx = co
+                src = f"up_blocks.{i}.attentions.{j}.proj_out" if c["up_attn"][i] else f"up_blocks.{i}.resnets.{j}.conv2"
+            if i != len(boc) - 1:
+                src = f"up_blocks.{i}.upsamplers.0.conv"
+        assert not skips
+        return plan
 
     def _pack(self):
         if self._P is not None:
@@ -176,7 +201,7 @@
 
         self._temb_names, self._xattn = [], []
         boc = c["block_out_channels"]
-        P = {}
+        P = {"cat_plan": self.concat_plan()}
         cin = c["in_channels"]
         self.cin_kpad = (9 * cin + 63) // 64 * 64
         w = sd["conv_in.weight"].detach().to(dev, dt).permute(0, 2, 3, 1).reshape(boc[0], -1)
@@ -244,12 +269,17 @@
             return None
         return ops.GnStats(self._gn_arena[i], self.cfg["norm_groups"], HW)
 
-    def _conv(self, h16, B, Hc, Wc, w, bias=None, bias2d=None, residual=None, stride=1, upsample=False, n_valid=0, gn=None):
+    def _share(self, u, part):
+        if self._cats is None or not 0 <= u < len(self._cats) or self._cats[u] is None:
+            return None
+        return self._cats[u].share(part)
+
+    def _conv(self, h16, B, Hc, Wc, w, bias=None, bias2d=None, residual=None, stride=1, upsample=False, n_valid=0, gn=None, gn2=None):
         tp = self.comm.world
         Cin = h16.shape[-1]
         if tp == 1:
             return ops.conv3x3(h16.view(B, Hc, Wc, Cin), w, bias=bias, bias2d=bias2d, residual=residual, stride=stride,
-                               upsample=upsample, out_dtype=torch.float32, n_valid=n_valid, gn=gn)
+                               upsample=upsample, out_dtype=torch.float32, n_valid=n_valid, gn=gn, gn2=gn2)
         from . import seqpar
         Hl = Hc // tp
         Co = n_valid or w.shape[0]
@@ -266,10 +296,11 @@
             out = ops.add(out, residual.reshape(out.shape).contiguous())
         return out
 
-    def _resnet(self, r, x, B, Hc, Wc, temb_all, skip=None, st_in=None):
+    def _resnet(self, r, x, B, Hc, Wc, temb_all, skip=None, st_in=None, cat=None, gn2=None):
         Ci = x.shape[-1] + (skip.shape[-1] if skip is not None else 0)
         if "ws" in r:
-            h, raw = self._gn(x, r["n1"], 1e-5, True, Hc, Wc, want_raw=True, x2=skip)
+            h, raw = self._gn(x, r["n1"], 1e-5, True, Hc, Wc, want_raw=True, x2=skip,
+                             stats=cat if skip is not None else (st_in if ops.GN_CONCAT else None))
         else:
             assert skip is None
             h = self._gn(x, r["n1"], 1e-5, True, Hc, Wc, stats=st_in)
@@ -283,11 +314,11 @@
         else:
             sc = x.view(-1, Ci)
         st_out = self._gn_slot(B, HW)
-        out = self._conv(h, B, Hc, Wc, r["w2"], bias=r["b2"], residual=sc, gn=st_out).view(B, -1, Co)
+        out = self._conv(h, B, Hc, Wc, r["w2"], bias=r["b2"], residual=sc, gn=st_out, gn2=gn2).view(B, -1, Co)
         self._mark(out)
         return out, st_out
 
-    def _transformer(self, t, x, B, ctx_kv, Hc, Wc, st_in=None):
+    def _transformer(self, t, x, B, ctx_kv, Hc, Wc, st_in=None, gn2=None):
         dt, heads = self.dtype, t["heads"]
         _, HW, C = x.shape
         hd = C // heads
@@ -325,7 +356,7 @@
                     hs = ops.gemm(g, b["wff2"], bias=b["bff2"], residual=hs, out_dtype=torch.float32, ln_emit=ln)
                 self._mark(hs)
             st_out = self._gn_slot(B, HW)
-            out = ops.gemm(hs, t["pout_w"], bias=t["pout_b"], residual=x.view(-1, C), out_dtype=torch.float32, gn=st_out)
+            out = ops.gemm(hs, t["pout_w"], bias=t["pout_b"], residual=x.view(-1, C), out_dtype=torch.float32, gn=st_out, gn2=gn2)
             return out.view(B, HW, C), st_out
         hs = ops.gemm(h.view(-1, C), t["pin_w"], bias=t["pin_b"], out_dtype=torch.float32)
         for k, b in enumerate(t["blocks"]):
@@ -354,7 +385,7 @@
             hs = ops.gemm(g, b["wff2"], bias=b["bff2"], residual=hs, out_dtype=dt if last else torch.float32)
             self._mark(hs)
         st_out = self._gn_slot(B, HW)
-        out = ops.gemm(hs, t["pout_w"], bias=t["pout_b"], residual=x.view(-1, C), out_dtype=torch.float32, gn=st_out)
+        out = ops.gemm(hs, t["pout_w"], bias=t["pout_b"], residual=x.view(-1, C), out_dtype=torch.float32, gn=st_out, gn2=gn2)
         return out.view(B, HW, C), st_out
 
     def _ln_fold_ok(self, M, C):
@@ -413,44 +444,65 @@
             from . import seqpar
             assert H % (tp * 4) == 0, f"latent rows {H} must divide by 4 x the sharding degree {tp} (two 2x down-samplings)"
         col = ops.im2col3x3_small(x_in.view(B, H, W, cin), self.cin_kpad, dt)
-        x = ops.gemm(col, P["conv_in_w"], bias=P["conv_in_b"], out_dtype=torch.float32).view(B, H * W, -1)
+        self._gn_arena = ops.GnStats.arena(self._n_gn_slots, B, c["norm_groups"], x_in.device) if tp == 1 else None
+        self._gn_next, self._cats = 0, None
+        plan = P["cat_plan"]
+        n_up = len(plan)
+        if self._gn_arena is not None and ops.GN_FUSE and ops.GN_CONCAT and n_up < self._n_gn_slots:
+            self._cats = [ops.GnCat(self._gn_arena[u], c["norm_groups"], (H >> e["level"]) * (W >> e["level"]), e["c_x"], e["width"])
+                          for u, e in enumerate(plan)]
+            self._gn_next = n_up
+        st = None
+        sh = self._share(n_up - 1, 1)
+        if sh is not None:
+            st = self._gn_slot(B, H * W)
+        x = ops.gemm(col, P["conv_in_w"], bias=P["conv_in_b"], out_dtype=torch.float32, gn=st, gn2=sh).view(B, H * W, -1)
+        if sh is not None and not (st.ready and sh.cat.ready[1]):
+            ops.groupnorm_stats_add(x, own=None if st.ready else st, share=None if sh.cat.ready[1] else sh)
         if tp > 1:
             x = seqpar.local_rows(x, rank, tp, H, W)
         skips = [(x, H, W)]
         ti = 0
         Hc, Wc = H, W
-        self._gn_arena = ops.GnStats.arena(self._n_gn_slots, B, c["norm_groups"], x.device) if tp == 1 else None
-        self._gn_next = 0
-        st = None
         for blk in P["down"]:
             for j, r in enumerate(blk["res"]):
-                x, st = self._resnet(r, x, B, Hc, Wc, temb_all, st_in=st)
+                sh = self._share(n_up - 1 - len(skips), 1)
                 if blk["attn"]:
-                    x, st = self._transformer(blk["attn"][j], x, B, ctx[ti], Hc, Wc, st_in=st)
+                    x, st = self._resnet(r, x, B, Hc, Wc, temb_all, st_in=st)
+                    x, st = self._transformer(blk["attn"][j], x, B, ctx[ti], Hc, Wc, st_in=st, gn2=sh)
                     ti += 1
+                else:
+                    x, st = self._resnet(r, x, B, Hc, Wc, temb_all, st_in=st, gn2=sh)
                 skips.append((x, Hc, Wc))
             if blk["down"] is not None:
                 st = self._gn_slot(B, (Hc // 2) * (Wc // 2))
-                x = self._conv(ops.cast(x, dt), B, Hc, Wc, blk["down"][0], bias=blk["down"][1], stride=2, gn=st)
+                x = self._conv(ops.cast(x, dt), B, Hc, Wc, blk["down"][0], bias=blk["down"][1], stride=2, gn=st,
+                               gn2=self._share(n_up - 1 - len(skips), 1))
                 Hc, Wc = Hc // 2, Wc // 2
                 skips.append((x, Hc, Wc))
         x, st = self._resnet(P["mid"]["res"][0], x, B, Hc, Wc, temb_all, st_in=st)
         x, st = self._transformer(P["mid"]["attn"][0], x, B, ctx[ti], Hc, Wc, st_in=st)
         ti += 1
-        x, st = self._resnet(P["mid"]["res"][1], x, B, Hc, Wc, temb_all, st_in=st)
+        x, st = self._resnet(P["mid"]["res"][1], x, B, Hc, Wc, temb_all, st_in=st, gn2=self._share(0, 0))
+        u = 0
         for blk in P["up"]:
             for j, r in enumerate(blk["res"]):
                 s, _, _ = skips.pop()
-                x, st = self._resnet(r, x.contiguous(), B, Hc, Wc, temb_all, skip=s)
+                cat = self._cats[u] if self._cats is not None else None
+                nxt = self._share(u + 1, 0) if j + 1 < len(blk["res"]) else None
                 if blk["attn"]:
-                    x, st = self._transformer(blk["attn"][j], x, B, ctx[ti], Hc, Wc, st_in=st)
+                    x, st = self._resnet(r, x.contiguous(), B, Hc, Wc, temb_all, skip=s, cat=cat)
+                    x, st = self._transformer(blk["attn"][j], x, B, ctx[ti], Hc, Wc, st_in=st, gn2=nxt)
                     ti += 1
+                else:
+                    x, st = self._resnet(r, x.contiguous(), B, Hc, Wc, temb_all, skip=s, cat=cat, gn2=nxt)
+                u += 1
             if blk["up"] is not None:
-                x = self._conv(ops.cast(x, dt), B, Hc, Wc, blk["up"][0], bias=blk["up"][1], upsample=True)
+                x = self._conv(ops.cast(x, dt), B, Hc, Wc, blk["up"][0], bias=blk["up"][1], upsample=True, gn2=self._share(u, 0))
                 Hc, Wc = Hc * 2, Wc * 2
                 st = None
         h = self._gn(x, P["norm_out"], 1e-5, True, Hc, Wc, stats=st)
-        self._gn_arena = None
+        self._gn_arena, self._cats = None, None
         self._on_mark = None
         nv = 4 if c["out_channels"] == 4 else 0
         out = self._conv(h, B, Hc, Wc, P["conv_out_w"], bias=P["conv_out_b"], n_valid=nv)
```
